# JuliaMolSim/DFTK.jl

Measured on AMD Instinct MI355X. Metric: SCF iterations/sec (Hψ applies/sec) at fixed Ecut·atoms, higher is better.
Workload: dtype f64

## Files before the change

dftk.jl_amd/_lib.py:

```python
from __future__ import annotations

import ctypes as C
import os

from . import _build

c_cplx_p = C.c_void_p
_i64 = C.c_int64


class dftk_mi_cplx(C.Structure):
    _fields_ = [("re", C.c_double), ("im", C.c_double)]


class DftkMiError(RuntimeError):
    def __init__(self, status, msg):
        super().__init__(f"dftk_mi355x status {status}: {msg}")
        self.status = status


_SIGNATURES = {
    "dftk_mi_last_error": (C.c_char_p, []),
    "dftk_mi_version": (C.c_char_p, []),
    "dftk_mi_basis_create": (C.c_int, [C.c_int, C.c_int, C.c_int, C.c_double, C.c_int, C.POINTER(C.c_void_p)]),
    "dftk_mi_basis_destroy": (C.c_int, [C.c_void_p]),
    "dftk_mi_basis_sync": (C.c_int, [C.c_void_p]),
    "dftk_mi_basis_set_fft_batch": (C.c_int, [C.c_void_p, C.c_int]),
    "dftk_mi_basis_stream": (C.c_void_p, [C.c_void_p]),
    "dftk_mi_kblock_create": (C.c_int, [C.c_void_p, _i64, C.c_void_p, C.c_void_p, C.POINTER(C.c_void_p)]),
    "dftk_mi_kblock_destroy": (C.c_int, [C.c_void_p]),
    "dftk_mi_kblock_set_projectors": (C.c_int, [C.c_void_p, C.c_int, C.c_void_p, _i64, C.c_void_p]),
    "dftk_mi_kblock_set_potential": (C.c_int, [C.c_void_p, C.c_void_p]),
    "dftk_mi_apply_H": (C.c_int, [C.c_void_p, C.c_int, C.c_void_p, _i64, C.c_void_p, _i64]),
    "dftk_mi_apply_H_parts": (C.c_int, [C.c_void_p, C.c_int, C.c_int, C.c_void_p, _i64, C.c_void_p, _i64]),
    "dftk_mi_local_potential": (C.c_int, [C.c_void_p, C.c_void_p, C.c_void_p, C.c_void_p, C.c_int, C.c_void_p,
                                          C.c_void_p]),
    "dftk_mi_local_potential_collinear": (C.c_int, [C.c_void_p, C.c_void_p, C.c_void_p, C.c_void_p, C.c_int, C.c_void_p,
                                                    C.c_void_p]),
    "dftk_mi_density_accumulate_spin": (C.c_int, [C.c_void_p, C.c_int, C.c_void_p, _i64, C.c_void_p, C.c_void_p, C.c_int,
                                                  C.c_int]),
    "dftk_mi_kpoint_sphere_host": (C.c_int, [C.c_int, C.c_int, C.c_int, C.c_void_p, C.c_void_p, C.c_double, _i64,
                                             C.POINTER(_i64), C.c_void_p, C.c_void_p, C.c_void_p]),
    "dftk_mi_build_projectors_hgh": (C.c_int, [C.c_void_p, _i64, C.c_void_p, C.c_void_p, C.c_void_p, C.c_double, C.c_int,
                                               C.c_void_p, C.c_void_p, C.c_int, C.c_void_p, C.c_void_p, C.c_void_p, _i64,
                                               C.POINTER(C.c_int)]),
    "dftk_mi_atomic_superposition": (C.c_int, [C.c_void_p, C.c_int, C.c_void_p, C.c_int, C.c_void_p, C.c_int, C.c_void_p,
                                               C.c_void_p, C.c_void_p]),
    "dftk_mi_forces_local": (C.c_int, [C.c_void_p, C.c_void_p, C.c_int, C.c_void_p, C.c_int, C.c_void_p, C.c_void_p,
                                       C.c_void_p, C.c_void_p]),
    "dftk_mi_forces_nonlocal": (C.c_int, [C.c_void_p, C.c_void_p, C.c_int, C.c_void_p, _i64, C.c_void_p, C.c_int,
                                          C.c_void_p, C.c_void_p]),
    "dftk_mi_xc_gga": (C.c_int, [C.c_void_p, _i64, C.c_void_p, C.c_void_p, C.c_int, C.c_double, C.c_void_p, C.c_void_p,
                                 C.c_void_p]),
    "dftk_mi_ifft_sphere": (C.c_int, [C.c_void_p, C.c_void_p, C.c_void_p]),
    "dftk_mi_fft_sphere": (C.c_int, [C.c_void_p, C.c_void_p, C.c_void_p]),
    "dftk_mi_density_accumulate": (C.c_int, [C.c_void_p, C.c_int, C.c_void_p, _i64, C.c_void_p, C.c_void_p]),
    "dftk_mi_lobpcg": (C.c_int, [C.c_void_p, C.c_int, C.c_void_p, _i64, C.c_double, C.c_int, C.c_int, C.c_int,
                                 C.c_int, C.c_uint64, C.c_void_p, C.c_void_p, C.POINTER(C.c_int),
                                 C.POINTER(C.c_int), C.POINTER(_i64)]),
    "dftk_mi_local_potential_gga": (C.c_int, [C.c_void_p, C.c_void_p, C.c_void_p, C.c_void_p, C.c_void_p, C.c_int,
                                              C.c_double, C.c_void_p, C.c_void_p]),
    "dftk_mi_symmetrize_rho": (C.c_int, [C.c_void_p, C.c_int, C.c_void_p, C.c_void_p, C.c_int, C.c_void_p, C.c_void_p]),
    "dftk_mi_mix_kerker": (C.c_int, [C.c_void_p, C.c_void_p, C.c_double, C.c_void_p, C.c_void_p]),
    "dftk_mi_mix_dielectric": (C.c_int, [C.c_void_p, C.c_void_p, C.c_double, C.c_double, C.c_void_p, C.c_void_p]),
    "dftk_mi_chi0_dielectric_apply": (C.c_int, [C.c_void_p, C.c_void_p, C.c_double, C.c_double, C.c_void_p, C.c_void_p]),
    "dftk_mi_cube_fourier_filter": (C.c_int, [C.c_void_p, C.c_void_p, C.c_void_p, C.c_void_p]),
    "dftk_mi_kblocks_set_potential": (C.c_int, [C.c_int, C.c_void_p, C.c_void_p]),
    "dftk_mi_lobpcg_multi": (C.c_int, [C.c_int, C.c_void_p, C.c_int, C.c_void_p, C.c_void_p, C.c_double, C.c_int, C.c_int,
                                       C.c_int, C.c_int, C.c_void_p, C.c_void_p, C.c_void_p, C.c_void_p, C.c_void_p,
                                       C.c_void_p, C.c_void_p]),
    "dftk_mi_density_accumulate_multi": (C.c_int, [C.c_int, C.c_void_p, C.c_void_p, C.c_void_p, C.c_void_p, C.c_void_p,
                                                   C.c_void_p]),
    "dftk_mi_density_accumulate_multi2": (C.c_int, [C.c_int, C.c_void_p, C.c_void_p, C.c_void_p, C.c_void_p, C.c_void_p,
                                                    C.c_void_p, C.c_void_p, C.c_void_p]),
    "dftk_mi_band_kinetic_multi": (C.c_int, [C.c_int, C.c_void_p, C.c_void_p, C.c_void_p, C.c_void_p, C.c_void_p]),
    "dftk_mi_batch_stats": (C.c_int, [C.POINTER(_i64), C.POINTER(_i64), C.POINTER(_i64), C.POINTER(_i64)]),
    "dftk_mi_lobpcg_small_stats": (C.c_int, [C.POINTER(_i64), C.POINTER(_i64)]),
    "dftk_mi_ortho_small": (C.c_int, [C.c_void_p, _i64, C.c_int, C.c_void_p, _i64, C.c_int, C.c_void_p, _i64, C.c_void_p,
                                      C.c_double, C.c_void_p]),
    "dftk_mi_lobpcg_last_AX": (C.c_void_p, [C.c_void_p]),
    "dftk_mi_lobpcg_history": (C.c_int, [C.c_void_p, C.POINTER(C.c_int), C.POINTER(C.c_int), C.c_void_p, C.c_size_t,
                                         C.POINTER(C.c_int)]),
    "dftk_mi_columnwise_norms": (C.c_int, [C.c_void_p, _i64, C.c_int, C.c_void_p, _i64, C.c_void_p]),
    "dftk_mi_columnwise_dots": (C.c_int, [C.c_void_p, _i64, C.c_int, C.c_void_p, _i64, C.c_void_p, _i64, C.c_void_p]),
    "dftk_mi_ortho_qr": (C.c_int, [C.c_void_p, _i64, C.c_int, C.c_void_p, _i64, C.c_int, C.POINTER(C.c_int),
                                   C.POINTER(C.c_int)]),
    "dftk_mi_tpa_precondprep": (C.c_int, [C.c_void_p, C.c_int, C.c_void_p, _i64, C.c_void_p]),
    "dftk_mi_tpa_ldiv": (C.c_int, [C.c_void_p, C.c_int, C.c_void_p, _i64, C.c_void_p, C.c_double, C.c_void_p, _i64]),
    "dftk_mi_block_residual": (C.c_int, [C.c_void_p, C.c_int, C.c_void_p, _i64, C.c_void_p, _i64, C.c_void_p,
                                         C.c_void_p, _i64, C.c_void_p, C.c_void_p, C.c_void_p]),
    "dftk_mi_kblock_set_gamma_real": (C.c_int, [C.c_void_p, C.c_int]),
    "dftk_mi_gamma_half_size": (C.c_int, [C.c_void_p, C.POINTER(_i64)]),
    "dftk_mi_gamma_tables_host": (C.c_int, [C.c_int, C.c_int, C.c_int, _i64, C.c_void_p, C.POINTER(_i64), C.c_void_p,
                                            C.c_void_p]),
    "dftk_mi_gamma_compress": (C.c_int, [C.c_void_p, C.c_int, C.c_void_p, _i64, C.c_void_p, _i64]),
    "dftk_mi_gamma_compress_aligned": (C.c_int, [C.c_void_p, C.c_int, C.c_void_p, _i64, C.c_void_p, _i64]),
    "dftk_mi_gamma_expand": (C.c_int, [C.c_void_p, C.c_int, C.c_void_p, _i64, C.c_void_p, _i64]),
    "dftk_mi_gamma_apply_H": (C.c_int, [C.c_void_p, C.c_int, C.c_int, C.c_void_p, _i64, C.c_void_p, _i64]),
    "dftk_mi_density_accumulate_real": (C.c_int, [C.c_void_p, C.c_int, C.c_void_p, _i64, C.c_void_p, C.c_void_p]),
    "dftk_mi_shard_plan_host": (C.c_int, [C.c_int, C.c_int, C.c_int, C.c_void_p, C.c_void_p, C.c_void_p, C.c_void_p,
                                          C.c_void_p, C.c_void_p]),
    "dftk_mi_kblock_set_shard": (C.c_int, [C.c_void_p, C.c_void_p, C.c_void_p]),
    "dftk_mi_zgemm": (C.c_int, [C.c_void_p, C.c_char, _i64, _i64, _i64, dftk_mi_cplx, C.c_void_p, _i64,
                                C.c_void_p, _i64, dftk_mi_cplx, C.c_void_p, _i64]),
    "dftk_mi_zgemm_ex": (C.c_int, [C.c_void_p, C.c_char, _i64, _i64, _i64, dftk_mi_cplx, C.c_void_p, _i64,
                                   C.c_void_p, _i64, dftk_mi_cplx, C.c_void_p, _i64, C.c_int]),
    "dftk_mi_zgemm_plan_host": (C.c_int, [C.c_char, _i64, _i64, _i64, C.c_int, C.POINTER(C.c_int)]),
    "dftk_mi_heev": (C.c_int, [C.c_void_p, C.c_int, C.c_void_p, _i64, C.c_void_p, C.c_void_p, _i64]),
    "dftk_mi_prof_zgemm_shapes": (C.c_int, [C.c_void_p, C.c_int, C.c_void_p, C.c_void_p, C.POINTER(C.c_int)]),
    "dftk_mi_heev_lowest": (C.c_int, [C.c_void_p, C.c_int, C.c_int, C.c_void_p, _i64, C.c_void_p, C.c_void_p, _i64]),
    "dftk_mi_heev_sigma_host": (C.c_int, [C.c_int, C.c_void_p, C.c_int, C.POINTER(C.c_double), C.POINTER(C.c_double),
                                          C.POINTER(C.c_int), C.c_double]),
    "dftk_mi_potrf_trtri": (C.c_int, [C.c_void_p, C.c_int, C.c_void_p, _i64, C.c_void_p, _i64]),
    "dftk_mi_potrf_trtri_real": (C.c_int, [C.c_void_p, C.c_int, C.c_void_p, _i64, C.c_void_p, _i64]),
    "dftk_mi_comm_get_unique_id": (C.c_int, [C.c_char_p]),
    "dftk_mi_comm_init_rank": (C.c_int, [C.c_char_p, C.c_int, C.c_int, C.c_int, C.POINTER(C.c_void_p)]),
    "dftk_mi_comm_create_host": (C.c_int, [C.c_int, C.c_int, C.c_int, C.c_void_p, C.c_void_p, C.c_void_p,
                                           C.POINTER(C.c_void_p)]),
    "dftk_mi_comm_destroy": (C.c_int, [C.c_void_p]),
    "dftk_mi_comm_describe": (C.c_int, [C.c_void_p, C.POINTER(C.c_int), C.POINTER(C.c_int), C.POINTER(C.c_int)]),
    "dftk_mi_comm_rank": (C.c_int, [C.c_void_p]),
    "dftk_mi_comm_size": (C.c_int, [C.c_void_p]),
    "dftk_mi_allreduce_sum_f64": (C.c_int, [C.c_void_p, C.c_void_p, C.c_size_t, C.c_void_p]),
    "dftk_mi_prof_enable": (C.c_int, [C.c_void_p, C.c_int]),
    "dftk_mi_prof_get": (C.c_int, [C.c_void_p, C.c_int, C.POINTER(C.c_double), C.POINTER(C.c_double),
                                   C.POINTER(_i64)]),
    "dftk_mi_anderson_create": (C.c_int, [C.c_void_p, _i64, C.c_int, C.c_double, C.c_double, C.POINTER(C.c_void_p)]),
    "dftk_mi_anderson_destroy": (C.c_int, [C.c_void_p]),
    "dftk_mi_anderson_reset": (C.c_int, [C.c_void_p]),
    "dftk_mi_anderson_history": (C.c_int, [C.c_void_p]),
    "dftk_mi_anderson_step": (C.c_int, [C.c_void_p, C.c_void_p, C.c_double, C.c_void_p, C.c_void_p, C.POINTER(C.c_int)]),
    "dftk_mi_chi0_mix": (C.c_int, [C.c_void_p, C.c_int, C.c_void_p, C.c_void_p, C.c_void_p, C.c_double, C.c_int, C.c_double,
                                   C.c_double, C.c_void_p, C.c_double, C.c_int, C.c_int, C.c_void_p, C.POINTER(C.c_int),
                                   C.POINTER(C.c_int)]),
    "dftk_mi_launch_count": (C.c_int, [C.POINTER(_i64), C.POINTER(_i64)]),
    "dftk_mi_kblock_reuse_AX": (C.c_int, [C.c_void_p, C.c_int]),
    "dftk_mi_ax_reuse_count": (C.c_int, [C.POINTER(_i64)]),
    "dftk_mi_step_sums": (C.c_int, [C.c_void_p, _i64, C.c_void_p, C.c_void_p, C.c_void_p, C.c_void_p]),
    "dftk_mi_fermi_bisection": (C.c_int, [C.c_int, C.c_void_p, C.c_void_p, C.c_void_p, C.c_int, C.c_double, C.c_double,
                                          C.c_double, C.c_double, C.c_double, C.POINTER(C.c_double)]),
    "dftk_mi_diag_mfma_peak": (C.c_int, [C.c_void_p, C.c_int, C.c_int, C.POINTER(C.c_double)]),
    "dftk_mi_jacobi_schedule_host": (C.c_int, [C.c_int, C.c_int, C.POINTER(C.c_int), C.POINTER(C.c_int),
                                               C.POINTER(C.c_int)]),
    "dftk_mi_fft_plan_host": (C.c_int, [C.c_int, C.POINTER(C.c_int), C.POINTER(C.c_int), C.POINTER(C.c_int)]),
    "dftk_mi_sphere_tables_host": (C.c_int, [C.c_int, C.c_int, C.c_int, _i64, C.c_void_p, C.POINTER(_i64),
                                             C.POINTER(C.c_int), C.c_void_p, C.c_void_p]),
}

ALLREDUCE_FN = C.CFUNCTYPE(C.c_int, C.c_void_p, C.POINTER(C.c_double), C.c_size_t)
ALLTOALLV_FN = C.CFUNCTYPE(C.c_int, C.c_void_p, C.POINTER(C.c_double), C.POINTER(C.c_size_t), C.POINTER(C.c_size_t),
                           C.POINTER(C.c_double), C.POINTER(C.c_size_t), C.POINTER(C.c_size_t))

EXPORTED_SYMBOLS = tuple(_SIGNATURES)
_lib = None


def load(build_if_missing: bool = True):
    global _lib
    if _lib is not None:
        return _lib
    path = _build.LIBPATH
    if build_if_missing and _build.needs_build():
        _build.build()
    if not os.path.exists(path):
        raise RuntimeError(f"{path} is missing and could not be built; the MI355X hot path has no fallback")
    lib = C.CDLL(path, mode=C.RTLD_GLOBAL)
    for name, (res, args) in _SIGNATURES.items():
        fn = getattr(lib, name)
        fn.restype = res
        fn.argtypes = args
    version = lib.dftk_mi_version().decode()
    if not version.endswith("src=" + _build.source_hash()):
        raise RuntimeError(f"{path} was built from other sources ({version!r}, expected src={_build.source_hash()}): "
                           "stale binary, rebuild with python -m dftk_jl_amd._build")
    _lib = lib
    return lib


def check(status: int):
    if status != 0:
        msg = load().dftk_mi_last_error().decode(errors="replace")
# ... 7 lines not shown
```

dftk.jl_amd/csrc/api.cpp:

```cpp
#include "common.h"
#include <chrono>
#include "batch.h"
#include <algorithm>
#include <cmath>
#include <cstdarg>
#include <cstdio>
#include <cstdlib>
#include <cstring>
#include <vector>

static thread_local char g_err[1024] = "";

void dftk_set_error(const char* fmt, ...) {
    va_list ap;
    va_start(ap, fmt);
    vsnprintf(g_err, sizeof(g_err), fmt, ap);
    va_end(ap);
}

extern "C" const char* dftk_mi_last_error(void) { return g_err; }

hipError_t dftk_scratch_malloc(void** p, size_t bytes) {
    static const bool poison = getenv("DFTK_MI_POISON") != nullptr;
    hipError_t e = hipMalloc(p, bytes);
// ... 1047 lines not shown
    }
    cd *R1, *F, *Gf;
    CHK(shard_buffers(kb, n_bands, &R1, &F, &Gf));
    Transposer t(kb, n_bands);
    CHK(t.to_bands(reinterpret_cast<const cd*>(psi_d), R1, F));
    if (t.mine == 0) return 0;
    return launch_density(kb, t.mine, F, kb->n_G, weight_h + t.c0[t.me], rho_d);
}

extern "C" int dftk_mi_density_accumulate_spin(dftk_mi_kblock* kb, int n_bands, const dftk_mi_cplx* psi_d, int64_t ld_psi,
                                               const double* weight_h, double* rho_d, int spin, int n_spin) {
    if (!kb || !rho_d || n_spin < 1 || n_spin > 2 || spin < 0 || spin >= n_spin) return DFTK_MI_EINVAL;
    const int64_t N = (int64_t)kb->basis->nx * kb->basis->ny * kb->basis->nz;
    return dftk_mi_density_accumulate(kb, n_bands, psi_d, ld_psi, weight_h, rho_d + (int64_t)spin * N);
}

extern "C" int dftk_mi_kblock_set_gamma_real(dftk_mi_kblock* kb, int on) {
    if (!kb) return DFTK_MI_EINVAL;
    HIPCHK(hipSetDevice(kb->basis->device));
    return gamma_enable(kb, on);
}

extern "C" int dftk_mi_gamma_tables_host(int nx, int ny, int nz, int64_t n_G, const int64_t* mapping0_h,
                                         int64_t* n_half, int32_t* row_h, int32_t* partner_row_h) {
    if (nx < 1 || ny < 1 || nz < 1 || n_G < 1 || !mapping0_h || !n_half) return DFTK_MI_EINVAL;
    if ((row_h == nullptr) != (partner_row_h == nullptr)) return DFTK_MI_EINVAL;
    return gamma_tables_host(nx, ny, nz, n_G, mapping0_h, n_half, row_h, partner_row_h);
}

static int gamma_ready(dftk_mi_kblock* kb) {
    if (!kb || !kb->gr || !kb->gr->d_g) {
        dftk_set_error("gamma_real: call dftk_mi_kblock_set_gamma_real(kb, 1) first");
        return DFTK_MI_EINVAL;
    }
    return 0;
}

extern "C" int dftk_mi_gamma_half_size(dftk_mi_kblock* kb, int64_t* n_half) {
    if (!n_half) return DFTK_MI_EINVAL;
    CHK(gamma_ready(kb));
    *n_half = gamma_local_rows(kb);
    return 0;
}

extern "C" int dftk_mi_gamma_compress(dftk_mi_kblock* kb, int m, const dftk_mi_cplx* X_d, int64_t ldx,
                                      dftk_mi_cplx* Xh_d, int64_t ldh) {
    CHK(gamma_ready(kb));
    if (m < 0 || !X_d || !Xh_d || ldx < local_rows(kb) || ldh < gamma_local_rows(kb)) return DFTK_MI_EINVAL;
    HIPCHK(hipSetDevice(kb->basis->device));
    if (kb->sh_comm)
        return gamma_lobpcg_load(kb, m, reinterpret_cast<const cd*>(X_d), ldx, reinterpret_cast<cd*>(Xh_d), ldh);
    return gamma_compress(kb, m, reinterpret_cast<const cd*>(X_d), ldx, reinterpret_cast<cd*>(Xh_d), ldh);
}

extern "C" int dftk_mi_gamma_compress_aligned(dftk_mi_kblock* kb, int m, const dftk_mi_cplx* X_d, int64_t ldx,
                                              dftk_mi_cplx* Xh_d, int64_t ldh) {
    CHK(gamma_ready(kb));
    if (m < 0 || !X_d || !Xh_d || ldx < local_rows(kb) || ldh < gamma_local_rows(kb)) return DFTK_MI_EINVAL;
    HIPCHK(hipSetDevice(kb->basis->device));
    return gamma_lobpcg_load(kb, m, reinterpret_cast<const cd*>(X_d), ldx, reinterpret_cast<cd*>(Xh_d), ldh, true);
}

extern "C" int dftk_mi_gamma_expand(dftk_mi_kblock* kb, int m, const dftk_mi_cplx* Xh_d, int64_t ldh,
                                    dftk_mi_cplx* X_d, int64_t ldx) {
    CHK(gamma_ready(kb));
    if (m < 0 || !X_d || !Xh_d || ldx < local_rows(kb) || ldh < gamma_local_rows(kb)) return DFTK_MI_EINVAL;
    HIPCHK(hipSetDevice(kb->basis->device));
    if (kb->sh_comm)
        return gamma_lobpcg_store(kb, m, reinterpret_cast<const cd*>(Xh_d), ldh, reinterpret_cast<cd*>(X_d), ldx);
    return gamma_expand(kb, m, reinterpret_cast<const cd*>(Xh_d), ldh, reinterpret_cast<cd*>(X_d), ldx);
}

extern "C" int dftk_mi_gamma_apply_H(dftk_mi_kblock* kb, int which, int n_bands, const dftk_mi_cplx* psih_d,
                                     int64_t ld_psi, dftk_mi_cplx* Hpsih_d, int64_t ld_Hpsi) {
    CHK(gamma_ready(kb));
    if (!psih_d || !Hpsih_d || n_bands < 0 || (which & ~7) || ld_psi < gamma_local_rows(kb) ||
        ld_Hpsi < gamma_local_rows(kb))
        return DFTK_MI_EINVAL;
    HIPCHK(hipSetDevice(kb->basis->device));
    return gamma_apply_H(kb, which, n_bands, reinterpret_cast<const cd*>(psih_d), ld_psi,
                         reinterpret_cast<cd*>(Hpsih_d), ld_Hpsi);
}

extern "C" int dftk_mi_density_accumulate_real(dftk_mi_kblock* kb, int n_bands, const dftk_mi_cplx* psi_d,
                                               int64_t ld_psi, const double* weight_h, double* rho_d) {
    if (!kb || !psi_d || !weight_h || !rho_d || n_bands < 0 || ld_psi < local_rows(kb)) return DFTK_MI_EINVAL;
    if (n_bands == 0) return 0;
    HIPCHK(hipSetDevice(kb->basis->device));
    if (!kb->sh_comm) prof_count(kb->basis, PROF_A2A_MODEL, 8.0 * (double)kb->n_G * n_bands);
    return gamma_density(kb, n_bands, reinterpret_cast<const cd*>(psi_d), ld_psi, weight_h, rho_d);
}

extern "C" int dftk_mi_lobpcg(dftk_mi_kblock* kb, int M, dftk_mi_cplx* X_d, int64_t ldX, double tol, int miniter,
                              int maxiter, int n_conv_check, int use_tpa, uint64_t seed, double* lambda_h,
                              double* resid_h, int* n_iter, int* converged, int64_t* n_matvec) {
    if (!kb || !X_d || M < 1 || ldX < local_rows(kb) || !lambda_h || !resid_h || !n_iter || !converged || !n_matvec ||
        maxiter < 0)
        return DFTK_MI_EINVAL;
    HIPCHK(hipSetDevice(kb->basis->device));
    return lobpcg_run(kb, M, reinterpret_cast<cd*>(X_d), ldX, tol, miniter, maxiter, n_conv_check, use_tpa, seed,
                      lambda_h, resid_h, n_iter, converged, n_matvec);
}

extern "C" int dftk_mi_lobpcg_multi(int n_kblocks, dftk_mi_kblock* const* kbs, int M, dftk_mi_cplx* const* X_d,
                                    const int64_t* ldX, double tol, int miniter, int maxiter, int n_conv_check, int use_tpa,
                                    const uint64_t* seeds, double* lambda_h, double* resid_h, int* n_iter, int* converged,
                                    int64_t* n_matvec, int* status) {
    if (n_kblocks < 0 || (n_kblocks > 0 && (!kbs || !X_d || !ldX || !lambda_h || !resid_h || !n_iter || !converged ||
                                            !n_matvec || !status)) || M < 1 || maxiter < 0)
        return DFTK_MI_EINVAL;
    if (n_kblocks == 0) return 0;
    for (int i = 0; i < n_kblocks; ++i)
        if (!kbs[i] || !X_d[i] || ldX[i] < local_rows(kbs[i])) return DFTK_MI_EINVAL;
    HIPCHK(hipSetDevice(kbs[0]->basis->device));
    return lobpcg_run_multi(n_kblocks, kbs, M, reinterpret_cast<cd* const*>(X_d), ldX, tol, miniter, maxiter, n_conv_check,
                            use_tpa, seeds, lambda_h, resid_h, n_iter, converged, n_matvec, status);
}

extern "C" int dftk_mi_band_kinetic_multi(int n_kblocks, dftk_mi_kblock* const* kbs, const int* n_bands,
                                          const dftk_mi_cplx* const* psi_d, const int64_t* ld_psi, double* out_h) {
    if (n_kblocks < 0 || (n_kblocks > 0 && (!kbs || !n_bands || !psi_d || !ld_psi || !out_h))) return DFTK_MI_EINVAL;
    if (n_kblocks == 0) return 0;
    dftk_mi_basis* b = kbs[0] ? kbs[0]->basis : nullptr;
    if (!b) return DFTK_MI_EINVAL;
    size_t total = 0;
    for (int i = 0; i < n_kblocks; ++i) {
        if (!kbs[i] || kbs[i]->basis != b || kbs[i]->sh_comm || !psi_d[i] || n_bands[i] < 0 || ld_psi[i] < kbs[i]->n_G)
            return DFTK_MI_EINVAL;
        total += (size_t)n_bands[i];
    }
    HIPCHK(hipSetDevice(b->device));
    CHK(ensure_ws(b, total * sizeof(double)));
    double* d = reinterpret_cast<double*>(b->ws);
    std::vector<std::function<int()>> bodies;
    size_t off = 0;
    for (int i = 0; i < n_kblocks; ++i) {
        const size_t o = off;
        off += (size_t)n_bands[i];
        bodies.push_back([=]() {
            if (n_bands[i] == 0) return 0;
            CHK(ew_weighted_colsums(b, kbs[i]->n_G, n_bands[i], reinterpret_cast<const cd*>(psi_d[i]), ld_psi[i], kbs[i]->d_kin,
                                    d + o));
            return dev_d2h_sync(b, out_h + o, d + o, (size_t)n_bands[i] * sizeof(double));
        });
    }
    std::vector<int> rets;
    CHK(batch_run(b, bodies, rets));
    for (int r : rets)
        if (r != 0) return r;
    return 0;
}

extern "C" int dftk_mi_density_accumulate_multi(int n_kblocks, dftk_mi_kblock* const* kbs, const int* n_bands,
                                                const dftk_mi_cplx* const* psi_d, const int64_t* ld_psi,
                                                const double* weights_h, double* rho_d) {
    return dftk_mi_density_accumulate_multi2(n_kblocks, kbs, n_bands, psi_d, ld_psi, weights_h, rho_d, nullptr, nullptr);
}

extern "C" int dftk_mi_density_accumulate_multi2(int n_kblocks, dftk_mi_kblock* const* kbs, const int* n_bands,
                                                 const dftk_mi_cplx* const* psi_d, const int64_t* ld_psi,
                                                 const double* weights_h, double* rho_d, const double* weights2_h,
                                                 double* rho2_d) {
    if (n_kblocks < 0 || (n_kblocks > 0 && (!kbs || !n_bands || !psi_d || !ld_psi || !weights_h)) || !rho_d ||
        ((weights2_h == nullptr) != (rho2_d == nullptr)) || (rho2_d && rho2_d == rho_d))
        return DFTK_MI_EINVAL;
    if (n_kblocks == 0) return 0;
// ... 244 lines not shown
```

dftk.jl_amd/csrc/common.h:

```cpp
#pragma once
#include <hip/hip_runtime.h>
#include <stdint.h>
#include <stddef.h>
#include <string>
#include <map>
#include <vector>
#include "../../include/dftk_mi355x.h"

typedef double2 cd;

#include <atomic>
extern std::atomic<int64_t> g_dftk_launches, g_dftk_host_syncs;
inline hipError_t dftk_counted_stream_sync(hipStream_t s) {
    g_dftk_host_syncs.fetch_add(1, std::memory_order_relaxed);
    return (hipStreamSynchronize)(s);
}
#define hipStreamSynchronize(s) dftk_counted_stream_sync(s)
#undef hipLaunchKernelGGL
#define hipLaunchKernelGGL(kernelName, ...)                               \
    do {                                                                  \
        g_dftk_launches.fetch_add(1, std::memory_order_relaxed);          \
        hipLaunchKernelGGLInternal((kernelName), __VA_ARGS__);            \
    } while (0)

// ... 25 lines not shown
};

int  plan_radices(int n, int* nrad, int* rad);
void plan_positions(int n, int nrad, const int* rad, int* pos);

struct dftk_mi_basis {
    int nx, ny, nz, nxp;
    double volume;
    int device;
    hipStream_t stream;
    FftAxis ax[3];
    void* d_tables[6];
    int fft_batch;
    cd* T1; size_t T1_bytes;
    cd* T2; size_t T2_bytes;
    void* ws; size_t ws_bytes;
    double* d_scalars;
    double* h_scalars;
    char* h_fetch;
    int use_mfma;
    struct Prof* prof;
    void* dense_ws; size_t dense_ws_bytes;
    void* eig_ws; size_t eig_ws_bytes;
    struct dftk_mi_comm* comm;
    void* symm_tab; uint64_t symm_key; int symm_n;
};

enum ProfFamily {
    PROF_ZGEMM = 0,
    PROF_FFT_A = 1,
    PROF_FFT_B = 2,
    PROF_FFT_C = 3,
    PROF_FFT_D = 4,
    PROF_FFT_E = 5,
    PROF_DENS_Z = 6,
    PROF_HEEV = 7,
    PROF_CHOL = 8,
    PROF_APPLY_H = 9,
    PROF_ZGEMM_BYTES = 10,
    PROF_ZGEMM_STRUCT = 11,
    PROF_ZGEMM_EXEC = 12,
    PROF_COMM = 13,
    PROF_ZGEMM_CPLX = 14,
    PROF_EW = 15,
    PROF_HOST_WAIT = 16,
    PROF_AR_MODEL = 17,
    PROF_A2A_MODEL = 18,
    PROF_NFAM = 24
};
struct Prof {
    bool on = false;
    struct Pair { hipEvent_t a, b; int fam; uint64_t tag; double work; };
    struct Shape { double ms = 0, work = 0; int64_t n = 0; };
    std::map<uint64_t, Shape> shapes;
    std::vector<Pair> pending;
    std::vector<Pair> pool;
    int open = 0;
    int mute = 0;
    bool shape_tags = false;
    double ms[PROF_NFAM] = {0};
    double work[PROF_NFAM] = {0};
    int64_t launches[PROF_NFAM] = {0};
};
int prof_begin(dftk_mi_basis* b, int fam, double work, uint64_t tag = 0);
void prof_end(dftk_mi_basis* b, int slot);
int prof_resolve(dftk_mi_basis* b);
struct ProfScope {
    dftk_mi_basis* b;
    int slot;
    ProfScope(dftk_mi_basis* basis, int fam, double work) : b(basis), slot(prof_begin(basis, fam, work)) {}
    ~ProfScope() { prof_end(b, slot); }
    ProfScope(const ProfScope&) = delete;
    ProfScope& operator=(const ProfScope&) = delete;
};
void prof_count(dftk_mi_basis* b, int fam, double work);
const size_t HOST_FETCH_BYTES = 256 * 1024;
int host_wait(dftk_mi_basis* b);
int host_fetch(dftk_mi_basis* b, void* dst_h, const void* src_d, size_t bytes);

struct GammaReal {
    bool on = false;
    int64_t n_half = 0;
    int *d_g = nullptr, *d_mg = nullptr;
    double* d_kin_half = nullptr;
    cd* P_half = nullptr;
    const cd* P_src = nullptr;
    int P_n_p = 0;
    cd* buf = nullptr;
    size_t buf_bytes = 0;
    std::vector<int64_t> half_rows;
};

struct dftk_mi_kblock {
    dftk_mi_basis* basis;
    int device;
    int64_t n_G;
    int64_t n_lines;
    int nzx;
    int z_lo;
    int*   d_cpos;
    int*   d_line_start;
    int*   d_line_ypos;
    int*   d_zls;
    int*   d_zpos;
    int*   d_zval;
    int*   d_line_yval;
    int*   d_cx;
    double* d_kin;
    double* d_Vs;
    struct SharedVs* Vs_share;
    int n_p;
    const cd* P;
    int64_t ldP;
    double* d_D;
    int D_bw;
    cd* lob_buf; size_t lob_bytes;
    cd* last_AX;
    cd* ax_keep; int ax_M; int64_t ax_rows; int64_t ax_ld;
    double* d_Vs_ax;
    double* d_dVs;
    bool ax_reuse_next;
    dftk_mi_comm* sh_comm;
    std::vector<int64_t>* sh_rows;
    cd* sh_buf; size_t sh_bytes;
    std::vector<double>* lob_hist; int lob_hist_M, lob_hist_iters, lob_n_svd;
    std::vector<int64_t>* h_mapping;
    std::vector<double>* h_kin;
    GammaReal* gr;
    int32_t* d_G3;
};

int fft_ensure_scratch(dftk_mi_basis* b, dftk_mi_kblock* kb, int nb);
int launch_local_apply(dftk_mi_kblock* kb, int nb, const cd* psi, int64_t ldpsi, cd* out,
                       int64_t ldout, bool add_kinetic, bool have_local);
int launch_ifft_to_cube(dftk_mi_kblock* kb, const cd* c, cd* cube, int nb = 1);
int launch_fft_from_cube(dftk_mi_kblock* kb, const cd* cube, cd* c, int nb = 1);
int launch_density(dftk_mi_kblock* kb, int nb, const cd* psi, int64_t ldpsi, const double* w_h, double* rho,
                   const double* w_im_h = nullptr, const double* w2_h = nullptr, double* rho2 = nullptr);
int launch_pad_potential(dftk_mi_kblock* kb, const double* V);
int launch_kinetic_only(dftk_mi_kblock* kb, int nb, const cd* psi, int64_t ldpsi, cd* out,
                        int64_t ldout, bool accumulate, bool use_kin);

int zgemm(dftk_mi_basis* b, char transA, int64_t m, int64_t n, int64_t k, cd alpha, const cd* A,
          int64_t lda, const cd* B, int64_t ldb, cd beta, cd* C, int64_t ldc, int upper = 0);
int ensure_ws(dftk_mi_basis* b, size_t bytes);

int dense_potrf_trtri(dftk_mi_basis* b, int n, cd* A, int64_t lda, cd* invR, int64_t ldi,
                      double* normest_R, double* normest_invR, bool real_input = false);
int dense_heev(dftk_mi_basis* b, int n, cd* A, int64_t lda, double* W_h, cd* V, int64_t ldv);
int dense_heev_full(dftk_mi_basis* b, int n, cd* A, int64_t lda, double* W_h, cd* V, int64_t ldv);
int dense_input_norms(dftk_mi_basis* b, int n, const cd* A, int64_t lda, double* off2, double* dg2, double* im2);
int dense_heev_lowest(dftk_mi_basis* b, int n, int nev, cd* A, int64_t lda, double* W_h, cd* V, int64_t ldv);
int eig_choose_sigma_host(int n, const double* diag, int nev, double* sigma, double* gap_guess);
int eig_hold_iterations_host(double gap_over_norm);
struct ProfMute {
    dftk_mi_basis* b;
    explicit ProfMute(dftk_mi_basis* basis) : b(basis) { if (b->prof) b->prof->mute += 1; }
    ~ProfMute() { if (b->prof) b->prof->mute -= 1; }
    ProfMute(const ProfMute&) = delete;
    ProfMute& operator=(const ProfMute&) = delete;
};
int jacobi_schedule_host(int n, int round, int* nb_out, int* pairs, int* where);
int apply_D(dftk_mi_kblock* kb, int n_bands, const cd* X , cd* Y);
int ew_colnorms(dftk_mi_basis* b, int64_t n, int m, const cd* X, int64_t ldx, double* out_d);
int ew_coldots(dftk_mi_basis* b, int64_t n, int m, const cd* X, int64_t ldx, const cd* Y, int64_t ldy,
               double* out_re_d);
int ew_residual(dftk_mi_basis* b, int64_t n, int m, const cd* AX, int64_t lda, const cd* X, int64_t ldx,
                const double* lam_d, cd* R, int64_t ldr, double* norms_d, const double* kin, double* mean_kin_d,
                double* xx_d);
int ew_tpa(dftk_mi_basis* b, int64_t n, int m, const cd* src, int64_t lds, cd* dst, int64_t ldd, const double* kin,
           const double* mean_kin_d, double* norms_d, double default_shift = 1.0);
int ew_scale_cols(dftk_mi_basis* b, int64_t n, int m, cd* X, int64_t ldx, const double* s_d, bool invert);
int ew_copy(dftk_mi_basis* b, int64_t n, int m, const cd* X, int64_t ldx, cd* Y, int64_t ldy);
int ew_add(dftk_mi_basis* b, int64_t n, int m, const cd* X, int64_t ldx, cd* Y, int64_t ldy);
int ew_sub_real(dftk_mi_basis* b, int64_t n, const double* a, const double* c, double* out);
int ew_fill_zero(dftk_mi_basis* b, cd* X, size_t count);
int ew_sub_identity_shifted(dftk_mi_basis* b, int rows, int cols, cd* C, int64_t ldc, int row0);
int ew_gather_cols(dftk_mi_basis* b, int64_t n, int m, const cd* X, int64_t ldx, const int* perm_d,
                   cd* Y, int64_t ldy);
int ew_add_diag(dftk_mi_basis* b, int n, cd* A, int64_t lda, double shift);
int ew_frob2(dftk_mi_basis* b, int64_t n, int m, const cd* X, int64_t ldx, double* out_d);
int ew_hermitize_upper(dftk_mi_basis* b, int n, cd* A, int64_t lda);
int ew_conj_transpose(dftk_mi_basis* b, int n, const cd* A, int64_t lda, cd* B, int64_t ldb);
int ew_square(dftk_mi_basis* b, double* d, size_t n);
int ew_sqrt(dftk_mi_basis* b, double* d, size_t n);
int ew_coldots_im(dftk_mi_basis* b, int64_t n, int m, const cd* X, int64_t ldx, const cd* Y, int64_t ldy,
                  double* out_im_d);
int ew_weighted_colsums(dftk_mi_basis* b, int64_t n, int m, const cd* X, int64_t ldx, const double* w_d,
                        double* out_d);

int comm_size(const dftk_mi_comm* c);
int comm_rank(const dftk_mi_comm* c);
int comm_allreduce(dftk_mi_comm* c, dftk_mi_basis* b, double* d, size_t n);
int comm_allreduce_norms(dftk_mi_comm* c, dftk_mi_basis* b, double* d, size_t n);
int comm_alltoallv(dftk_mi_comm* c, dftk_mi_basis* b, const cd* send, const size_t* soff, const size_t* scnt,
                   cd* recv, const size_t* roff, const size_t* rcnt);

int local_potential_collinear(dftk_mi_kblock* cube_kb, const double* rho, const double* vloc, const double* green,
                              int fun_mask, double* V_out, double* energies_h);
int local_potential_lda(dftk_mi_kblock* cube_kb, const double* recip_h, const double* rho, const double* vloc,
                        const double* green, int fun_mask, double threshold, double* V_out, double* energies_h);

int cube_symmetrize(dftk_mi_kblock* cube_kb, int n_sym, const int32_t* S_h, const double* tau_h, int do_lowpass,
                    const double* rho_in, double* rho_out);
int cube_fourier_filter(dftk_mi_kblock* cube_kb, int kind, const double* recip_h, double p0, double p1,
                        const double* mult_d, const double* f, double* out);
int xc_gga_pointwise(dftk_mi_basis* b, int64_t n, const double* rho, const double* sigma, int fun_mask,
                     double threshold, double* e, double* vrho, double* vsigma);

int sphere_enumerate_host(int nx, int ny, int nz, const double* B, const double* k, double Ecut, int64_t cap,
                          int64_t* n_G_out, int64_t* mapping0, double* kinetic, int32_t* G_out);
int build_projectors_hgh(dftk_mi_basis* b, int64_t n_rows, const int32_t* G_d, const double* recip_h, const double* k_h,
                         double volume, int n_species, const double* rp_h, const int* nproj_h, int n_atoms,
                         const int* species_of_atom_h, const double* positions_h, cd* P_d, int64_t ldP, int* n_p_out);

int atomic_superposition(dftk_mi_kblock* cube_kb, int kind, const double* recip_h, int n_species, const double* par_h,
                         int n_atoms, const int* species_of_atom_h, const double* positions_h, double* out_d);

int gamma_tables_host(int nx, int ny, int nz, int64_t n_G, const int64_t* mapping, int64_t* n_half_out, int32_t* g,
                      int32_t* mg);
int gamma_enable(dftk_mi_kblock* kb, int on);
void gamma_destroy(GammaReal* gr);
int gamma_compress(dftk_mi_kblock* kb, int m, const cd* X, int64_t ldx, cd* H, int64_t ldh);
int gamma_compress_aligned(dftk_mi_kblock* kb, int m, const cd* X, int64_t ldx, cd* H, int64_t ldh);
int gamma_expand(dftk_mi_kblock* kb, int m, const cd* H, int64_t ldh, cd* X, int64_t ldx);
int gamma_apply_H(dftk_mi_kblock* kb, int which, int nb, const cd* psi, int64_t ldpsi, cd* Hpsi, int64_t ldH);
int gamma_density(dftk_mi_kblock* kb, int nb, const cd* psi, int64_t ldpsi, const double* w_h, double* rho);
int gamma_ensure_buf(dftk_mi_kblock* kb, size_t elems);
int gamma_pack_pairs(dftk_mi_kblock* kb, int nb, const cd* H, int64_t ldh, cd* Z, int64_t ldz);
int gamma_unpack_pairs(dftk_mi_kblock* kb, int nb, const cd* W, int64_t ldw, cd* H, int64_t ldh);
int gamma_pack_full(dftk_mi_kblock* kb, int nb, const cd* X, int64_t ldx, cd* Z, int64_t ldz);
int gamma_gather_P(dftk_mi_kblock* kb, int ncols, const cd* P, int64_t ldP, cd* Ph, int64_t ldh, double* asym_mag_h);
int gamma_density_bands(dftk_mi_kblock* kb, int nb, const cd* psi, int64_t ldpsi, const double* w_h, double* rho);
int64_t gamma_local_rows(const dftk_mi_kblock* kb);
int64_t gamma_row0(const dftk_mi_kblock* kb);
int gamma_projectors(dftk_mi_kblock* kb);
int gamma_apply_H_sharded(dftk_mi_kblock* kb, int which, int nb, const cd* psi, int64_t ldpsi, cd* Hpsi, int64_t ldH);
int gamma_projectors_sharded(dftk_mi_kblock* kb);
int gamma_density_sharded(dftk_mi_kblock* kb, int nb, const cd* psi, int64_t ldpsi, const double* w_h, double* rho);
int gamma_lobpcg_load(dftk_mi_kblock* kb, int M, const cd* Xuser, int64_t ldX, cd* Xh, int64_t ldh, bool align = false);
int gamma_lobpcg_store(dftk_mi_kblock* kb, int M, const cd* Xh, int64_t ldh, cd* Xuser, int64_t ldX);
int apply_nonlocal_rows(dftk_mi_kblock* kb, int nb, const cd* P, int64_t ldP, int64_t rows, const cd* psi,
                        int64_t ldpsi, cd* Hpsi, int64_t ldH, bool accumulate, int gemm_flags, dftk_mi_comm* comm);

int forces_local(dftk_mi_kblock* cube_kb, const double* recip_h, int n_species, const double* par_h, int n_atoms,
                 const int* species_of_atom_h, const double* positions_h, const double* rho_d, double* forces_h);
int forces_nonlocal(dftk_mi_kblock* kb, const double* kcoord_h, int nb, const cd* psi, int64_t ld_psi,
                    const double* weight_h, int n_atoms, const int* col_start_h, double* forces_h);

int lobpcg_ortho(dftk_mi_basis* b, int64_t n, int m, cd* X, int64_t ldx, int force_svd, int* n_chol, int* used_svd);
int lobpcg_run_multi(int n_kb, dftk_mi_kblock* const* kbs, int M, cd* const* X, const int64_t* ldX, double tol, int miniter,
                     int maxiter, int n_conv_check, int use_tpa, const uint64_t* seeds, double* lambda_h, double* resid_h,
                     int* n_iter, int* converged, int64_t* n_matvec, int* status);
int lobpcg_run(dftk_mi_kblock* kb, int M, cd* X, int64_t ldX, double tol, int miniter, int maxiter,
               int n_conv_check, int use_tpa, uint64_t seed, double* lambda_h, double* resid_h,
               int* n_iter, int* converged, int64_t* n_matvec);
```

dftk.jl_amd/csrc/fft_kernels.hip:

```cpp
#include "common.h"
#include "batch.h"
#include <algorithm>
#include <cstring>
#include <type_traits>

#define FFT_L 8
#ifndef ZPASS_MIN_BLOCKS
#define ZPASS_MIN_BLOCKS 6
#endif
#ifndef DENS_MIN_BLOCKS
#define DENS_MIN_BLOCKS 1
#endif
#ifndef YFWD_MIN_BLOCKS
#define YFWD_MIN_BLOCKS 1
#endif
#define FFT_LS_X 9
#define FFT_LS_YZ 8
#define FFT_THREADS 256
#define FFT_TPL (FFT_THREADS / FFT_L)
#define DENS_MAXACC 12

__device__ __forceinline__ cd cmul(cd a, cd w) {
    return make_double2(fma(a.x, w.x, -a.y * w.y), fma(a.x, w.y, a.y * w.x));
}
// ... 192 lines not shown
        case 4: fft_stage<FFT_LS, 4, false, true>(buf, tw, n, m, sgn, l, j, vcol, vstride); return true;
        case 5: fft_stage<FFT_LS, 5, false, true>(buf, tw, n, m, sgn, l, j, vcol, vstride); return true;
        case 6: fft_stage<FFT_LS, 6, false, true>(buf, tw, n, m, sgn, l, j, vcol, vstride); return true;
        case 8: fft_stage<FFT_LS, 8, false, true>(buf, tw, n, m, sgn, l, j, vcol, vstride); return true;
        default: return false;
    }
}

template <int FFT_LS, bool DIF, bool GEN>
__device__ __forceinline__ void fft_stage_dispatch(int R, cd* buf, const cd* tw, int n, int m, double sgn,
                                                   int l, int j) {
    switch (R) {
        case 2: fft_stage<FFT_LS, 2, DIF>(buf, tw, n, m, sgn, l, j); break;
        case 3: fft_stage<FFT_LS, 3, DIF>(buf, tw, n, m, sgn, l, j); break;
        case 4: fft_stage<FFT_LS, 4, DIF>(buf, tw, n, m, sgn, l, j); break;
        case 5: fft_stage<FFT_LS, 5, DIF>(buf, tw, n, m, sgn, l, j); break;
        case 6: fft_stage<FFT_LS, 6, DIF>(buf, tw, n, m, sgn, l, j); break;
        case 8: fft_stage<FFT_LS, 8, DIF>(buf, tw, n, m, sgn, l, j); break;
        default:
            if constexpr (GEN) {
                if (R == 7)
                    fft_stage<FFT_LS, 7, DIF>(buf, tw, n, m, sgn, l, j);
                else
                    fft_stage_generic<FFT_LS, DIF>(buf, tw, n, m, R, sgn, l, j);
            }
            break;
    }
}

template <int FFT_LS, bool DIF, bool GEN>
__device__ __forceinline__ bool fft_tile(cd* buf, const cd* tw, const FftAxis& ax, double sgn, int l, int j,
                                         const double* vcol = nullptr, int64_t vstride = 0,
                                         bool skip_first = false) {
    const int n = ax.n;
    bool fused = false;
    if (!DIF) {
        int m = 1;
        for (int s = 0; s < ax.nrad; ++s) {
            const int R = ax.rad[s];
            if (vcol != nullptr && s == ax.nrad - 1)
                fused = fft_stage_vmul<FFT_LS>(R, buf, tw, n, m, sgn, l, j, vcol, vstride);
            if (!fused) fft_stage_dispatch<FFT_LS, false, GEN>(R, buf, tw, n, m, sgn, l, j);
            __syncthreads();
            m *= R;
        }
    } else {
        int m = n;
        for (int s = ax.nrad - 1; s >= 0; --s) {
            const int R = ax.rad[s];
            m /= R;
            if (skip_first && s == ax.nrad - 1) continue;
            fft_stage_dispatch<FFT_LS, true, GEN>(R, buf, tw, n, m, sgn, l, j);
            __syncthreads();
        }
    }
    return fused;
}

template <int FFT_LS>
__device__ __forceinline__ void tile_prologue(cd* buf, cd* tw, const FftAxis& ax, bool zero, bool copy_tw = true) {
    const int n = ax.n;
    if (copy_tw)
        for (int t = threadIdx.x; t < n; t += FFT_THREADS) tw[t] = ax.tw[t];
    if (zero) {
        const cd z = make_double2(0.0, 0.0);
        for (int t = threadIdx.x; t < n * FFT_LS; t += FFT_THREADS) buf[t] = z;
    }
}

extern __shared__ __attribute__((aligned(16))) char dftk_smem[];

struct FftJob {
    const int *line_start, *cpos, *line_ypos, *zls, *zpos;
    int z_lo;
    const double* kin;
    const double* Vs;
    const cd* psi;
    cd* out;
    int n_lines, nzx;
    double w, wim;
    double w2;
};

template <bool GEN>
__global__ __launch_bounds__(FFT_THREADS) void k_xbwd_scatter(FftAxis ax, int nxp, int n_lines,
                                                              const int* __restrict__ line_start,
                                                              const int* __restrict__ cpos,
                                                              const cd* __restrict__ psi, int64_t ldpsi,
                                                              cd* __restrict__ T1, int64_t T1_stride,
                                                              const FftJob* __restrict__ jobs) {
    constexpr int FFT_LS = FFT_LS_X;
    cd* buf = reinterpret_cast<cd*>(dftk_smem);
    cd* tw = buf + ax.n * FFT_LS;
    const int tid = threadIdx.x, l = tid & (FFT_L - 1), j = tid >> 3;
    const int band = blockIdx.y;
    const int l0 = blockIdx.x * FFT_L;
    const cd* p = psi + (int64_t)band * ldpsi;
    if (jobs) {
        const FftJob jb = jobs[band];
        n_lines = jb.n_lines;
        line_start = jb.line_start;
        cpos = jb.cpos;
        p = jb.psi;
        if (l0 >= n_lines) return;
    }
    tile_prologue<FFT_LS>(buf, tw, ax, true);
    __syncthreads();
    const int line = l0 + l;
    if (line < n_lines) {
        const int c0 = line_start[line], c1 = line_start[line + 1];
        for (int c = c0 + j; c < c1; c += FFT_TPL) buf[cpos[c] * FFT_LS + l] = p[c];
    }
    __syncthreads();
    fft_tile<FFT_LS, false, GEN>(buf, tw, ax, +1.0, l, j);
    cd* out = T1 + (int64_t)band * T1_stride + (int64_t)l0 * nxp;
    const int nlv = min(FFT_L, n_lines - l0);
    const int n = ax.n;
    for (int idx = tid; idx < nlv * nxp; idx += FFT_THREADS) {
        const int ll = idx / nxp;
        const int x = idx - ll * nxp;
        out[idx] = (x < n) ? buf[x * FFT_LS + ll] : make_double2(0.0, 0.0);
    }
}

template <bool GEN>
__global__ __launch_bounds__(FFT_THREADS) void k_ybwd(FftAxis ay, int nxp, int ny,
                                                      const int* __restrict__ zls,
                                                      const int* __restrict__ line_ypos,
                                                      const cd* __restrict__ T1, int64_t T1_stride,
                                                      cd* __restrict__ T2, int64_t T2_stride,
                                                      const FftJob* __restrict__ jobs) {
    constexpr int FFT_LS = FFT_LS_YZ;
    cd* buf = reinterpret_cast<cd*>(dftk_smem);
    cd* tw = buf + ay.n * FFT_LS;
    const int tid = threadIdx.x, l = tid & (FFT_L - 1), j = tid >> 3;
    const int x = blockIdx.x * FFT_L + l;
    const int zi = blockIdx.y, band = blockIdx.z;
    if (jobs) {
        const FftJob jb = jobs[band];
        if (zi >= jb.nzx) return;
        zls = jb.zls;
        line_ypos = jb.line_ypos;
    }
    const cd* t1 = T1 + (int64_t)band * T1_stride;
    const int ln0 = zls[zi] + j, ln1 = zls[zi + 1];
    const bool early = ln1 - zls[zi] <= 3 * FFT_TPL;
    cd e0, e1, e2;
    if (early) {
        if (ln0 < ln1) e0 = t1[(int64_t)ln0 * nxp + x];
        if (ln0 + FFT_TPL < ln1) e1 = t1[(int64_t)(ln0 + FFT_TPL) * nxp + x];
        if (ln0 + 2 * FFT_TPL < ln1) e2 = t1[(int64_t)(ln0 + 2 * FFT_TPL) * nxp + x];
    }
    tile_prologue<FFT_LS>(buf, tw, ay, true);
    __syncthreads();
    if (early) {
        if (ln0 < ln1) buf[line_ypos[ln0] * FFT_LS + l] = e0;
        if (ln0 + FFT_TPL < ln1) buf[line_ypos[ln0 + FFT_TPL] * FFT_LS + l] = e1;
        if (ln0 + 2 * FFT_TPL < ln1) buf[line_ypos[ln0 + 2 * FFT_TPL] * FFT_LS + l] = e2;
    } else {
        for (int ln = ln0; ln < ln1; ln += FFT_TPL) buf[line_ypos[ln] * FFT_LS + l] = t1[(int64_t)ln * nxp + x];
    }
    __syncthreads();
    fft_tile<FFT_LS, false, GEN>(buf, tw, ay, +1.0, l, j);
    cd* t2 = T2 + (int64_t)band * T2_stride + (int64_t)zi * ny * nxp + x;
    for (int y = j; y < ny; y += FFT_TPL) t2[(int64_t)y * nxp] = buf[y * FFT_LS + l];
}

template <int MODE, bool GEN>
__global__ __launch_bounds__(FFT_THREADS, ZPASS_MIN_BLOCKS) void k_zpass(FftAxis az, int nx, int nxp, int ny, int nzx,
                                                       int nbands, const int* __restrict__ zpos,
                                                       const double* __restrict__ Vs,
                                                       cd* __restrict__ T2, int64_t T2_stride,
                                                       cd* __restrict__ cube, const FftJob* __restrict__ jobs = nullptr) {
    constexpr int FFT_LS = FFT_LS_YZ;
    cd* buf = reinterpret_cast<cd*>(dftk_smem);
    cd* tw = buf + az.n * FFT_LS;
    const int tid = threadIdx.x, l = tid & (FFT_L - 1), j = tid >> 3;
    const int xcd = blockIdx.x & 7, slot = blockIdx.x >> 3;
    const int band = slot % nbands;
    const int grp = (slot / nbands) * 8 + xcd;
    const int nxt = nxp / FFT_L;
    if (grp >= nxt * ny) return;
    if (jobs) {
        const FftJob jb = jobs[band];
        zpos = jb.zpos;
        nzx = jb.nzx;
        Vs = jb.Vs;
    }
    const int y = grp / nxt;
    const int x = (grp - y * nxt) * FFT_L + l;
    const int nz = az.n;
    const int64_t plane = (int64_t)ny * nxp;
    cd* t2 = T2 + (int64_t)band * T2_stride + (int64_t)y * nxp + x;
    const bool early = MODE != 2 && nzx <= 3 * FFT_TPL;
// ... 293 lines not shown
            wi = jb.wim;
            wb2 = jb.w2;
            nzx = jb.nzx;
            z_lo = jb.z_lo;
        } else {
            wb = w[ib];
            wi = wim ? wim[ib] : wb;
        }
        if (wb == 0.0 && wi == 0.0 && wb2 == 0.0) continue;
        const cd* __restrict__ t2 = T2 + (int64_t)ib * T2_stride + (int64_t)y * nxp + (x - l);
        const unsigned planeB = plane * (unsigned)sizeof(cd), stepB = (unsigned)FS::R2 * planeB;
        const unsigned off_lo = (unsigned)j * planeB + (unsigned)l * (unsigned)sizeof(cd);
        const unsigned off_hi = off_lo - (unsigned)(FS::N - nzx) * planeB;
        const int zneg0 = FS::N - (nzx - z_lo);
        auto in = [&](auto ni) -> cd {
            constexpr int n1 = decltype(ni)::value;
            const int e = FS::R2 * n1 + j;
            const bool lo = e < z_lo, hi = e >= zneg0;
            cd v = make_double2(0.0, 0.0);
            if (lo || hi) v = ld_off(t2, (lo ? off_lo : off_hi) + (unsigned)n1 * stepB);
            return v;
        };
        cd psi[FS::R2];
        FS::backward(buf, az.tw, l, j, in, psi);
        if (j < FS::R1) {
#pragma unroll
            for (int p = 0; p < FS::R2; ++p) {
                acc[p] = fma(wb, psi[p].x * psi[p].x, fma(wi, psi[p].y * psi[p].y, acc[p]));
                if (rho2) acc2[p] = fma(wb2, psi[p].x * psi[p].x + psi[p].y * psi[p].y, acc2[p]);
            }
        }
        __syncthreads();
    }
    if (j < FS::R1 && x < nx) {
        double* __restrict__ r0 = (part ? part + (int64_t)blockIdx.z * az.n * ny * nx : rho) + (int64_t)y * nx + (x - l);
        const unsigned zB = (unsigned)ny * (unsigned)nx * 8u;
        const unsigned ob = (unsigned)j * zB + (unsigned)l * 8u;
        static_for<0, FS::R2>([&](auto pi) {
            constexpr int p = decltype(pi)::value;
            const unsigned off = ob + (unsigned)(FS::R1 * FS::k2_of(p)) * zB;
            st_off(r0, off, part ? acc[p] : ld_off((const double*)r0, off) + acc[p]);
        });
        if (rho2) {
            double* __restrict__ q0 = (part ? part + ((int64_t)gridDim.z + blockIdx.z) * az.n * ny * nx : rho2) + (int64_t)y * nx + (x - l);
            static_for<0, FS::R2>([&](auto pi) {
                constexpr int p = decltype(pi)::value;
                const unsigned off = ob + (unsigned)(FS::R1 * FS::k2_of(p)) * zB;
                st_off(q0, off, part ? acc2[p] : ld_off((const double*)q0, off) + acc2[p]);
            });
        }
    }
}

template <bool GEN>
__global__ __launch_bounds__(FFT_THREADS, YFWD_MIN_BLOCKS) void k_yfwd(FftAxis ay, int nxp, int ny,
                                                      const int* __restrict__ zls,
                                                      const int* __restrict__ line_ypos,
                                                      const cd* __restrict__ T2, int64_t T2_stride,
                                                      cd* __restrict__ T1, int64_t T1_stride,
                                                      const FftJob* __restrict__ jobs) {
    constexpr int FFT_LS = FFT_LS_YZ;
    cd* buf = reinterpret_cast<cd*>(dftk_smem);
    cd* tw = buf + ay.n * FFT_LS;
    const int tid = threadIdx.x, l = tid & (FFT_L - 1), j = tid >> 3;
    const int x = blockIdx.x * FFT_L + l;
    const int zi = blockIdx.y, band = blockIdx.z;
    if (jobs) {
        const FftJob jb = jobs[band];
        if (zi >= jb.nzx) return;
        zls = jb.zls;
        line_ypos = jb.line_ypos;
    }
    tile_prologue<FFT_LS>(buf, tw, ay, false);
    const cd* t2 = T2 + (int64_t)band * T2_stride + (int64_t)zi * ny * nxp + x;
    for (int y = j; y < ny; y += FFT_TPL) buf[y * FFT_LS + l] = t2[(int64_t)y * nxp];
    __syncthreads();
    fft_tile<FFT_LS, true, GEN>(buf, tw, ay, -1.0, l, j);
    cd* t1 = T1 + (int64_t)band * T1_stride;
    const int ln1 = zls[zi + 1];
    for (int ln = zls[zi] + j; ln < ln1; ln += FFT_TPL)
        t1[(int64_t)ln * nxp + x] = buf[line_ypos[ln] * FFT_LS + l];
}

template <bool GEN>
__global__ __launch_bounds__(FFT_THREADS, YFWD_MIN_BLOCKS) void k_xfwd_gather(FftAxis ax, int nxp, int n_lines,
                                                             const int* __restrict__ line_start,
                                                             const int* __restrict__ cpos,
                                                             const cd* __restrict__ T1, int64_t T1_stride,
                                                             const double* __restrict__ kin,
                                                             const cd* __restrict__ psi, int64_t ldpsi,
                                                             cd* __restrict__ out, int64_t ldout,
                                                             const FftJob* __restrict__ jobs) {
    constexpr int FFT_LS = FFT_LS_X;
    cd* buf = reinterpret_cast<cd*>(dftk_smem);
    cd* tw = buf + ax.n * FFT_LS;
    const int tid = threadIdx.x, l = tid & (FFT_L - 1), j = tid >> 3;
    const int band = blockIdx.y;
    const int l0 = blockIdx.x * FFT_L;
    const int n = ax.n;
    cd* o = out + (int64_t)band * ldout;
    const cd* p = psi + (int64_t)band * ldpsi;
    if (jobs) {
        const FftJob jb = jobs[band];
        n_lines = jb.n_lines;
        line_start = jb.line_start;
        cpos = jb.cpos;
        kin = jb.kin;
        p = jb.psi;
        o = jb.out;
        if (l0 >= n_lines) return;
    }
    tile_prologue<FFT_LS>(buf, tw, ax, false);
    const cd* in = T1 + (int64_t)band * T1_stride + (int64_t)l0 * nxp;
    const int nlv = min(FFT_L, n_lines - l0);
    for (int idx = tid; idx < FFT_L * nxp; idx += FFT_THREADS) {
        const int ll = idx / nxp;
        const int x = idx - ll * nxp;
        if (x < n) buf[x * FFT_LS + ll] = (ll < nlv) ? in[idx] : make_double2(0.0, 0.0);
    }
    __syncthreads();
    fft_tile<FFT_LS, true, GEN>(buf, tw, ax, -1.0, l, j);
    const int line = l0 + l;
    if (line < n_lines) {
        const int c0 = line_start[line], c1 = line_start[line + 1];
        for (int c = c0 + j; c < c1; c += FFT_TPL) {
            cd v = buf[cpos[c] * FFT_LS + l];
            if (kin != nullptr) {
                const double k = kin[c];
                const cd q = p[c];
                v.x = fma(k, q.x, v.x);
                v.y = fma(k, q.y, v.y);
            }
            o[c] = v;
        }
    }
}

template <bool GEN>
__global__ __launch_bounds__(FFT_THREADS, DENS_MIN_BLOCKS) void k_zdensity(FftAxis az, int nx, int nxp, int ny, int nzx,
                                                          const int* __restrict__ zpos, int nb,
                                                          const double* __restrict__ w,
                                                          const double* __restrict__ wim,
                                                          const cd* __restrict__ T2, int64_t T2_stride,
                                                          double* __restrict__ rho, const FftJob* __restrict__ jobs,
                                                          double* __restrict__ part, double* __restrict__ rho2 = nullptr) {
    constexpr int FFT_LS = FFT_LS_YZ;
    cd* buf = reinterpret_cast<cd*>(dftk_smem);
    cd* tw = buf + az.n * FFT_LS;
    const int tid = threadIdx.x, l = tid & (FFT_L - 1), j = tid >> 3;
    const int x = blockIdx.x * FFT_L + l;
    const int y = blockIdx.y;
    const int nz = az.n;
    const int64_t plane = (int64_t)ny * nxp;
    double acc[DENS_MAXACC], acc2[DENS_MAXACC];
#pragma unroll
    for (int k = 0; k < DENS_MAXACC; ++k) acc[k] = acc2[k] = 0.0;
    for (int t = tid; t < nz; t += FFT_THREADS) tw[t] = az.tw[t];
    for (int ib = blockIdx.z; ib < nb; ib += gridDim.z) {
        double wb, wi, wb2 = 0.0;
        if (jobs) {
            const FftJob jb = jobs[ib];
            wb = jb.w;
            wi = jb.wim;
            wb2 = jb.w2;
            zpos = jb.zpos;
            nzx = jb.nzx;
        } else {
            wb = w[ib];
            wi = wim ? wim[ib] : wb;
        }
        if (wb == 0.0 && wi == 0.0 && wb2 == 0.0) continue;
        const cd z0 = make_double2(0.0, 0.0);
        for (int t = tid; t < nz * FFT_LS; t += FFT_THREADS) buf[t] = z0;
        __syncthreads();
        const cd* t2 = T2 + (int64_t)ib * T2_stride + (int64_t)y * nxp + x;
        for (int zi = j; zi < nzx; zi += FFT_TPL) buf[zpos[zi] * FFT_LS + l] = t2[(int64_t)zi * plane];
        __syncthreads();
        fft_tile<FFT_LS, false, GEN>(buf, tw, az, +1.0, l, j);
#pragma unroll
        for (int k = 0; k < DENS_MAXACC; ++k) {
            const int z = j + k * FFT_TPL;
            if (z < nz) {
                const cd v = buf[z * FFT_LS + l];
                acc[k] = fma(wb, v.x * v.x, fma(wi, v.y * v.y, acc[k]));
                if (rho2) acc2[k] = fma(wb2, v.x * v.x + v.y * v.y, acc2[k]);
            }
        }
        __syncthreads();
    }
    if (x < nx) {
        double* __restrict__ dst = part ? part + (int64_t)blockIdx.z * nz * ny * nx : rho;
#pragma unroll
        for (int k = 0; k < DENS_MAXACC; ++k) {
            const int z = j + k * FFT_TPL;
            if (z < nz) {
                const int64_t at = ((int64_t)z * ny + y) * nx + x;
                dst[at] = part ? acc[k] : dst[at] + acc[k];
            }
        }
        if (rho2) {
            double* __restrict__ dst2 = part ? part + ((int64_t)gridDim.z + blockIdx.z) * nz * ny * nx : rho2;
#pragma unroll
            for (int k = 0; k < DENS_MAXACC; ++k) {
                const int z = j + k * FFT_TPL;
                if (z < nz) {
                    const int64_t at = ((int64_t)z * ny + y) * nx + x;
                    dst2[at] = part ? acc2[k] : dst2[at] + acc2[k];
                }
            }
        }
    }
}
// ... 5 lines not shown
    for (int g = 0; g < ngroups; ++g) s += part[(int64_t)g * n + i];
    rho[i] += s;
}

__global__ void k_pad_potential(int nx, int nxp, int64_t rows, double scale, const double* __restrict__ V,
                                double* __restrict__ Vs) {
    const int64_t i = (int64_t)blockIdx.x * blockDim.x + threadIdx.x;
    if (i >= rows * nxp) return;
    const int64_t r = i / nxp;
    const int x = (int)(i - r * nxp);
    Vs[i] = (x < nx) ? V[r * nx + x] * scale : 0.0;
}

__global__ void k_kinetic(int64_t n, int nb, const double* __restrict__ kin, const cd* __restrict__ psi,
                          int64_t ldpsi, cd* __restrict__ out, int64_t ldout, int accumulate) {
    const int64_t i = (int64_t)blockIdx.x * blockDim.x + threadIdx.x;
    if (i >= n) return;
    const double k = kin ? kin[i] : 0.0;
    for (int b = 0; b < nb; ++b) {
        cd q = psi[(int64_t)b * ldpsi + i];
        cd v = make_double2(k * q.x, k * q.y);
        if (accumulate) {
            cd o = out[(int64_t)b * ldout + i];
            v.x += o.x;
            v.y += o.y;
        }
        out[(int64_t)b * ldout + i] = v;
    }
}

static size_t lds_bytes(int n, int ls = FFT_LS_YZ) { return (size_t)n * (ls + 1) * sizeof(cd); }

int fft_ensure_scratch(dftk_mi_basis* b, dftk_mi_kblock* kb, int nb) {
    const size_t t1 = (size_t)nb * kb->n_lines * b->nxp * sizeof(cd);
    const size_t t2 = (size_t)nb * kb->nzx * b->ny * b->nxp * sizeof(cd);
    if (t1 > b->T1_bytes) {
        if (b->T1) HIPCHK(hipFree(b->T1));
        b->T1 = nullptr;
        HIPCHK(dftk_scratch_malloc((void**)&b->T1, t1));
        b->T1_bytes = t1;
    }
    if (t2 > b->T2_bytes) {
        if (b->T2) HIPCHK(hipFree(b->T2));
        b->T2 = nullptr;
        HIPCHK(dftk_scratch_malloc((void**)&b->T2, t2));
        b->T2_bytes = t2;
    }
    return 0;
}

static int check_lds(dftk_mi_basis* b) {
    const int nmax = b->nx > b->ny ? (b->nx > b->nz ? b->nx : b->nz) : (b->ny > b->nz ? b->ny : b->nz);
    if (lds_bytes(nmax, FFT_LS_X) > 160 * 1024) {
        dftk_set_error("FFT axis length %d needs %zu B of LDS (> 160 KiB)", nmax, lds_bytes(nmax, FFT_LS_X));
        return DFTK_MI_EINVAL;
    }
    return 0;
}

template <typename K>
static int set_lds_attr(K kernel, size_t bytes) {
    if (bytes > 64 * 1024) {
        HIPCHK(hipFuncSetAttribute(reinterpret_cast<const void*>(kernel),
                                   hipFuncAttributeMaxDynamicSharedMemorySize, (int)bytes));
    }
    return 0;
}

static bool axis_generic(const FftAxis& ax) {
    for (int s = 0; s < ax.nrad; ++s)
        if (ax.rad[s] > 5 && ax.rad[s] != 6 && ax.rad[s] != 8) return true;
    return false;
}

#define LAUNCH_FFT(KERNEL, AX, GRID, LDS, STREAM, ...)                                               \
    do {                                                                                             \
        if (axis_generic(AX)) {                                                                      \
            CHK(set_lds_attr(KERNEL<true>, LDS));                                                    \
            hipLaunchKernelGGL((KERNEL<true>), GRID, dim3(FFT_THREADS), LDS, STREAM, __VA_ARGS__);   \
        } else {                                                                                     \
            CHK(set_lds_attr(KERNEL<false>, LDS));                                                   \
            hipLaunchKernelGGL((KERNEL<false>), GRID, dim3(FFT_THREADS), LDS, STREAM, __VA_ARGS__);  \
        }                                                                                            \
    } while (0)
#define LAUNCH_ZPASS(MODE, AX, GRID, LDS, STREAM, ...)                                                      \
    do {                                                                                                    \
        if (axis_generic(AX)) {                                                                             \
            CHK(set_lds_attr(k_zpass<MODE, true>, LDS));                                                    \
            hipLaunchKernelGGL((k_zpass<MODE, true>), GRID, dim3(FFT_THREADS), LDS, STREAM, __VA_ARGS__);   \
        } else {                                                                                            \
            CHK(set_lds_attr(k_zpass<MODE, false>, LDS));                                                   \
            hipLaunchKernelGGL((k_zpass<MODE, false>), GRID, dim3(FFT_THREADS), LDS, STREAM, __VA_ARGS__);  \
        }                                                                                                   \
    } while (0)

#define REG_SIZES(X)                                                                                                      \
    X(24, 2, 2, 3, 2) X(27, 3, 3, 3, 1) X(30, 5, 1, 3, 2) X(32, 2, 2, 4, 2) X(36, 3, 2, 3, 2) X(40, 2, 2, 5, 2) X(48, 3, 2, 4, 2) X(54, 3, 2, 3, 3)           \
    X(45, 3, 3, 5, 1) X(50, 5, 2, 5, 1) X(60, 3, 2, 5, 2)                                                                 \
    X(64, 4, 2, 4, 2) X(72, 3, 3, 4, 2) X(80, 5, 2, 4, 2) X(90, 5, 2, 3, 3) X(96, 4, 3, 4, 2) X(100, 5, 2, 5, 2)          \
    X(108, 4, 3, 3, 3) X(120, 4, 3, 5, 2) X(128, 4, 4, 4, 2) X(144, 4, 3, 4, 3) X(150, 5, 3, 5, 2) X(160, 4, 4, 5, 2)     \
    X(180, 5, 3, 4, 3) X(192, 4, 4, 4, 3) X(200, 5, 4, 5, 2) X(216, 6, 3, 4, 3) X(240, 4, 4, 5, 3) X(256, 4, 4, 4, 4)
static bool fft_reg_on(int n) {
    static const bool off = getenv("DFTK_MI_FFT_REG") != nullptr && atoi(getenv("DFTK_MI_FFT_REG")) == 0;
    static const int nmin = getenv("DFTK_MI_FFT_REG_MIN") ? atoi(getenv("DFTK_MI_FFT_REG_MIN")) : 24;
    return !off && n >= nmin;
}
static bool fft_reg_fits(const dftk_mi_basis* b) {
    return (uint64_t)b->nz * (uint64_t)b->ny * (uint64_t)b->nxp * sizeof(cd) < (1ull << 32);
}
struct RegZ {
    dftk_mi_basis* b;
    hipStream_t stream;
    dim3 grid;
    int nzx, z_lo, nbands;
    const double* Vs;
    cd* T2;
    int64_t s2;
    const double *w, *wim;
    double* rho;
    const FftJob* jobs;
    double* part = nullptr;
    double* rho2 = nullptr;
};
template <int A, int B, int C, int D>
static int reg_zpass_t(const RegZ& r) {
    typedef FourStep<A, B, C, D> FS;
    const size_t lds = (size_t)FS::LDS_ELEMS * sizeof(cd);
    CHK(set_lds_attr(k_zpass_reg<A, B, C, D>, lds));
    hipLaunchKernelGGL((k_zpass_reg<A, B, C, D>), r.grid, dim3(FS::THREADS), lds, r.stream, r.b->ax[2], r.b->nx, r.b->nxp, r.b->ny,
                       r.nzx, r.z_lo, r.nbands, r.Vs, r.T2, r.s2, r.jobs);
    return 0;
}
template <int A, int B, int C, int D>
static int reg_zdens_t(const RegZ& r) {
    typedef FourStep<A, B, C, D> FS;
    const size_t lds = (size_t)FS::LDS_ELEMS * sizeof(cd);
    CHK(set_lds_attr(k_zdensity_reg<A, B, C, D>, lds));
    hipLaunchKernelGGL((k_zdensity_reg<A, B, C, D>), r.grid, dim3(FS::THREADS), lds, r.stream, r.b->ax[2], r.b->nx, r.b->nxp,
                       r.b->ny, r.nzx, r.z_lo, r.nbands, r.w, r.wim, (const cd*)r.T2, r.s2, r.rho, r.jobs, r.part, r.rho2);
    return 0;
}
static int reg_zpass(const RegZ& r, bool tables_ok) {
    if (!tables_ok || !fft_reg_on(r.b->nz) || !fft_reg_fits(r.b)) return 1;
    switch (r.b->nz) {
#define X(NN, A, B, C, D) case NN: return reg_zpass_t<A, B, C, D>(r);
        REG_SIZES(X)
#undef X
        default: return 1;
    }
}
static int reg_zdens(const RegZ& r, bool tables_ok) {
    if (!tables_ok || !fft_reg_on(r.b->nz) || !fft_reg_fits(r.b)) return 1;
    switch (r.b->nz) {
#define X(NN, A, B, C, D) case NN: return reg_zdens_t<A, B, C, D>(r);
        REG_SIZES(X)
#undef X
        default: return 1;
    }
}

static dim3 zpass_grid(const dftk_mi_basis* b, int nbands) {
    const int64_t groups = (int64_t)(b->nxp / FFT_L) * b->ny;
    return dim3((unsigned)(((groups + 7) / 8) * 8 * nbands));
}

struct Strides {
    int64_t s1, s2;
};
static Strides strides(dftk_mi_kblock* kb) {
    dftk_mi_basis* b = kb->basis;
    return Strides{(int64_t)kb->n_lines * b->nxp, (int64_t)kb->nzx * b->ny * b->nxp};
}

static int run_AB(dftk_mi_kblock* kb, int nbb, const cd* psi, int64_t ldpsi) {
    dftk_mi_basis* b = kb->basis;
    const Strides st = strides(kb);
    const int gl = (int)((kb->n_lines + FFT_L - 1) / FFT_L);
    const int nxt = b->nxp / FFT_L;
    const double Ncube = (double)b->nx * b->ny * b->nz;
    const double t1b = 16.0 * (double)kb->n_lines * b->nxp, t2b = 16.0 * (double)kb->nzx * b->ny * b->nxp;
    (void)Ncube;
    int ps = prof_begin(b, PROF_FFT_A, (16.0 * kb->n_G + t1b) * nbb);
    LAUNCH_FFT(k_xbwd_scatter, b->ax[0], dim3(gl, nbb), lds_bytes(b->nx, FFT_LS_X), b->stream, b->ax[0],
                       b->nxp, (int)kb->n_lines, kb->d_line_start, kb->d_cpos, psi, ldpsi, b->T1, st.s1, (const FftJob*)nullptr);
    prof_end(b, ps);
    ps = prof_begin(b, PROF_FFT_B, (t1b + t2b) * nbb);
    LAUNCH_FFT(k_ybwd, b->ax[1], dim3(nxt, kb->nzx, nbb), lds_bytes(b->ny), b->stream, b->ax[1],
                       b->nxp, b->ny, kb->d_zls, kb->d_line_ypos, b->T1, st.s1, b->T2, st.s2, (const FftJob*)nullptr);
    prof_end(b, ps);
    return 0;
}

static int run_DE(dftk_mi_kblock* kb, int nbb, const double* kin, const cd* psi, int64_t ldpsi, cd* out,
                  int64_t ldout) {
    dftk_mi_basis* b = kb->basis;
    const Strides st = strides(kb);
    const int gl = (int)((kb->n_lines + FFT_L - 1) / FFT_L);
    const int nxt = b->nxp / FFT_L;
    const double Ncube = (double)b->nx * b->ny * b->nz;
    const double t1b = 16.0 * (double)kb->n_lines * b->nxp, t2b = 16.0 * (double)kb->nzx * b->ny * b->nxp;
    (void)Ncube;
    int ps = prof_begin(b, PROF_FFT_D, (t1b + t2b) * nbb);
    LAUNCH_FFT(k_yfwd, b->ax[1], dim3(nxt, kb->nzx, nbb), lds_bytes(b->ny), b->stream, b->ax[1],
                       b->nxp, b->ny, kb->d_zls, kb->d_line_ypos, b->T2, st.s2, b->T1, st.s1, (const FftJob*)nullptr);
    prof_end(b, ps);
    ps = prof_begin(b, PROF_FFT_E, (t1b + (kin ? 40.0 : 16.0) * kb->n_G) * nbb);
    LAUNCH_FFT(k_xfwd_gather, b->ax[0], dim3(gl, nbb), lds_bytes(b->nx, FFT_LS_X), b->stream, b->ax[0],
                       b->nxp, (int)kb->n_lines, kb->d_line_start, kb->d_cpos, b->T1, st.s1, kin, psi, ldpsi, out,
                       ldout, (const FftJob*)nullptr);
    prof_end(b, ps);
    return 0;
}

int launch_local_apply(dftk_mi_kblock* kb, int nb, const cd* psi, int64_t ldpsi, cd* out, int64_t ldout,
                       bool add_kinetic, bool have_local) {
    dftk_mi_basis* b = kb->basis;
    if (!have_local || kb->d_Vs == nullptr) {
        return launch_kinetic_only(kb, nb, psi, ldpsi, out, ldout, false, add_kinetic);
    }
    CHK(check_lds(b));
    const int batch = b->fft_batch;
    CHK(fft_ensure_scratch(b, kb, nb < batch ? nb : batch));
    const Strides st = strides(kb);
    const int nxt = b->nxp / FFT_L;
    for (int b0 = 0; b0 < nb; b0 += batch) {
        const int nbb = (nb - b0) < batch ? (nb - b0) : batch;
        const cd* p = psi + (int64_t)b0 * ldpsi;
        CHK(run_AB(kb, nbb, p, ldpsi));
        const int pc = prof_begin(b, PROF_FFT_C, 2.0 * 16.0 * (double)kb->nzx * b->ny * b->nxp * nbb +
                                                     8.0 * (double)b->nz * b->ny * b->nxp);
        const RegZ rz{b, b->stream, zpass_grid(b, nbb), kb->nzx, kb->z_lo, nbb, kb->d_Vs, b->T2, st.s2, nullptr, nullptr, nullptr,
                      nullptr};
        const int reg_st = reg_zpass(rz, kb->z_lo >= 0);
        if (reg_st < 0) return reg_st;
        if (reg_st != 0)
        LAUNCH_ZPASS(0, b->ax[2], zpass_grid(b, nbb), lds_bytes(b->nz), b->stream, b->ax[2], b->nx, b->nxp, b->ny, kb->nzx, nbb, kb->d_zpos, kb->d_Vs, b->T2, st.s2,
                           (cd*)nullptr, (const FftJob*)nullptr);
        prof_end(b, pc);
        CHK(run_DE(kb, nbb, add_kinetic ? kb->d_kin : nullptr, p, ldpsi, out + (int64_t)b0 * ldout, ldout));
    }
    HIPCHK(hipGetLastError());
    return 0;
}

int launch_kinetic_only(dftk_mi_kblock* kb, int nb, const cd* psi, int64_t ldpsi, cd* out, int64_t ldout,
                        bool accumulate, bool use_kin) {
    dftk_mi_basis* b = kb->basis;
    const int threads = 256;
    const int blocks = (int)((kb->n_G + threads - 1) / threads);
    hipLaunchKernelGGL(k_kinetic, dim3(blocks), dim3(threads), 0, b->stream, kb->n_G, nb,
                       use_kin ? kb->d_kin : (const double*)nullptr, psi, ldpsi, out, ldout, accumulate ? 1 : 0);
    HIPCHK(hipGetLastError());
    return 0;
}

int launch_ifft_to_cube(dftk_mi_kblock* kb, const cd* c, cd* cube, int nb) {
    dftk_mi_basis* b = kb->basis;
    CHK(check_lds(b));
    CHK(fft_ensure_scratch(b, kb, nb));
    const Strides st = strides(kb);
    CHK(run_AB(kb, nb, c, kb->n_G));
    LAUNCH_ZPASS(1, b->ax[2], zpass_grid(b, nb), lds_bytes(b->nz), b->stream, b->ax[2], b->nx, b->nxp, b->ny, kb->nzx, nb, kb->d_zpos, (const double*)nullptr, b->T2, st.s2,
                       cube, (const FftJob*)nullptr);
    HIPCHK(hipGetLastError());
    return 0;
}

int launch_fft_from_cube(dftk_mi_kblock* kb, const cd* cube, cd* c, int nb) {
    dftk_mi_basis* b = kb->basis;
    CHK(check_lds(b));
    CHK(fft_ensure_scratch(b, kb, nb));
    const Strides st = strides(kb);
    LAUNCH_ZPASS(2, b->ax[2], zpass_grid(b, nb), lds_bytes(b->nz), b->stream, b->ax[2], b->nx, b->nxp, b->ny, kb->nzx, nb, kb->d_zpos, (const double*)nullptr, b->T2, st.s2,
                       const_cast<cd*>(cube), (const FftJob*)nullptr);
    CHK(run_DE(kb, nb, nullptr, c, kb->n_G, c, kb->n_G));
    HIPCHK(hipGetLastError());
    return 0;
}

int launch_density(dftk_mi_kblock* kb, int nb, const cd* psi, int64_t ldpsi, const double* w_h, double* rho,
                   const double* w_im_h, const double* w2_h, double* rho2) {
    dftk_mi_basis* b = kb->basis;
    if (batching() && nb > 0) {
        BOp o;
        o.b = b;
        o.kb = kb;
        o.type = BOP_DENSITY; o.m = nb; o.A = psi; o.lda = ldpsi; o.C = rho; o.D = w2_h ? rho2 : nullptr;
        o.flags = (w_im_h ? 1 : 0) | (w2_h ? 2 : 0);
        o.payload.resize((size_t)(1 + (w_im_h ? 1 : 0) + (w2_h ? 1 : 0)) * nb * sizeof(double));
        memcpy(o.payload.data(), w_h, (size_t)nb * sizeof(double));
        size_t at = (size_t)nb * sizeof(double);
        if (w_im_h) {
            memcpy(o.payload.data() + at, w_im_h, (size_t)nb * sizeof(double));
            at += (size_t)nb * sizeof(double);
        }
        if (w2_h) memcpy(o.payload.data() + at, w2_h, (size_t)nb * sizeof(double));
        return batch_record(std::move(o));
    }
    if (w2_h) {
        CHK(launch_density(kb, nb, psi, ldpsi, w_h, rho, w_im_h, nullptr, nullptr));
        return launch_density(kb, nb, psi, ldpsi, w2_h, rho2, nullptr, nullptr, nullptr);
    }
    CHK(check_lds(b));
    if (b->nz > DENS_MAXACC * FFT_TPL) {
        dftk_set_error("density kernel supports nz <= %d", DENS_MAXACC * FFT_TPL);
        return DFTK_MI_EINVAL;
    }
    const int batch = b->fft_batch;
    CHK(fft_ensure_scratch(b, kb, nb < batch ? nb : batch));
    const Strides st = strides(kb);
    CHK(ensure_ws(b, 2 * (size_t)nb * sizeof(double)));
    double* w_d = reinterpret_cast<double*>(b->ws);
    double* wim_d = w_im_h ? w_d + nb : nullptr;
    HIPCHK(hipMemcpyAsync(w_d, w_h, (size_t)nb * sizeof(double), hipMemcpyHostToDevice, b->stream));
    if (w_im_h) HIPCHK(hipMemcpyAsync(wim_d, w_im_h, (size_t)nb * sizeof(double), hipMemcpyHostToDevice, b->stream));
    for (int b0 = 0; b0 < nb; b0 += batch) {
        const int nbb = (nb - b0) < batch ? (nb - b0) : batch;
        bool any = false;
        for (int i = 0; i < nbb; ++i) any = any || (w_h[b0 + i] != 0.0) || (w_im_h && w_im_h[b0 + i] != 0.0);
        if (!any) continue;
        CHK(run_AB(kb, nbb, psi + (int64_t)b0 * ldpsi, ldpsi));
        const int pz = prof_begin(b, PROF_DENS_Z, 16.0 * (double)kb->nzx * b->ny * b->nxp * nbb +
// ... 224 lines not shown
```

dftk.jl_amd/csrc/gamma_kernels.hip:

```cpp
#include "common.h"
#include <algorithm>
#include <cmath>
#include <cstdio>
#include <unordered_map>
#include <vector>

int gamma_tables_host(int nx, int ny, int nz, int64_t n_G, const int64_t* mapping, int64_t* n_half_out, int32_t* g,
                      int32_t* mg) {
    if (n_G < 1 || mapping[0] != 0) {
        dftk_set_error("gamma_real: the sphere must contain G = 0 as its first entry");
        return DFTK_MI_EINVAL;
    }
    std::unordered_map<int64_t, int32_t> row;
    row.reserve((size_t)n_G * 2);
    for (int64_t c = 0; c < n_G; ++c) row[mapping[c]] = (int32_t)c;
    int64_t nh = 0;
    for (int64_t c = 0; c < n_G; ++c) {
        const int64_t lin = mapping[c];
        const int ix = (int)(lin % nx), iy = (int)((lin / nx) % ny), iz = (int)(lin / ((int64_t)nx * ny));
        const int64_t mlin = (int64_t)((nx - ix) % nx) + (int64_t)nx * (((ny - iy) % ny) + (int64_t)ny * ((nz - iz) % nz));
        auto it = row.find(mlin);
        if (it == row.end()) {
            dftk_set_error("gamma_real: the sphere is not inversion symmetric (row %lld has no -G partner)", (long long)c);
            return DFTK_MI_EINVAL;
// ... 119 lines not shown
            im[u] = j < nh ? mg[j] : 0;
        }
#pragma unroll
        for (int u = 0; u < GR_UNR; ++u) {
            a[u] = x[ig[u]];
            b[u] = x[im[u]];
        }
#pragma unroll
        for (int u = 0; u < GR_UNR; ++u) {
            const int64_t j = j0 + u * GRA_NT;
            cd aa = a[u], bb = b[u];
            if (rot) {
                aa = make_double2(aa.x * c + aa.y * sn, aa.y * c - aa.x * sn);
                bb = make_double2(bb.x * c + bb.y * sn, bb.y * c - bb.x * sn);
            }
            const double s = j ? GR_ISQRT2 : 0.5;
            if (j < nh) h[j] = make_double2(s * (aa.x + bb.x), s * (aa.y - bb.y));
        }
    }
}

__global__ __launch_bounds__(256) void k_gr_expand(int64_t nh, const int* __restrict__ g, const int* __restrict__ mg,
                                                   const cd* __restrict__ H, int64_t ldh, cd* __restrict__ X, int64_t ldx) {
    const int64_t j0 = (int64_t)blockIdx.x * GR_ROWS + threadIdx.x;
    cd* x = X + (int64_t)blockIdx.y * ldx;
    const cd* hc = H + (int64_t)blockIdx.y * ldh;
    int ig[GR_UNR], im[GR_UNR];
    cd h[GR_UNR];
#pragma unroll
    for (int u = 0; u < GR_UNR; ++u) {
        const int64_t j = j0 + u * 256;
        const bool in = j < nh;
        ig[u] = in ? g[j] : 0;
        im[u] = in ? mg[j] : 0;
        h[u] = in ? hc[j] : make_double2(0.0, 0.0);
    }
#pragma unroll
    for (int u = 0; u < GR_UNR; ++u) {
        const int64_t j = j0 + u * 256;
        if (j >= nh) continue;
        if (j == 0) {
            x[ig[u]] = make_double2(h[u].x, 0.0);
            continue;
        }
        x[ig[u]] = make_double2(GR_ISQRT2 * h[u].x, GR_ISQRT2 * h[u].y);
        x[im[u]] = make_double2(GR_ISQRT2 * h[u].x, -GR_ISQRT2 * h[u].y);
    }
}

__global__ __launch_bounds__(256) void k_gr_pack(int64_t nh, int nb, const int* __restrict__ g, const int* __restrict__ mg,
                                                 const cd* __restrict__ H, int64_t ldh, cd* __restrict__ Z, int64_t ldz) {
    const int64_t j0 = (int64_t)blockIdx.x * GR_ROWS + threadIdx.x;
    const int p = blockIdx.y;
    const bool has_b = 2 * p + 1 < nb;
    const cd* ha = H + (int64_t)(2 * p) * ldh;
    const cd* hb = H + (int64_t)(has_b ? 2 * p + 1 : 2 * p) * ldh;
    cd* z = Z + (int64_t)p * ldz;
    int ig[GR_UNR], im[GR_UNR];
    cd a[GR_UNR], b[GR_UNR];
#pragma unroll
    for (int u = 0; u < GR_UNR; ++u) {
        const int64_t j = j0 + u * 256;
        const bool in = j < nh;
        ig[u] = in ? g[j] : 0;
        im[u] = in ? mg[j] : 0;
        a[u] = in ? ha[j] : make_double2(0.0, 0.0);
        b[u] = (in && has_b) ? hb[j] : make_double2(0.0, 0.0);
    }
    const double s = GR_ISQRT2;
#pragma unroll
    for (int u = 0; u < GR_UNR; ++u) {
        const int64_t j = j0 + u * 256;
        if (j >= nh) continue;
        if (j == 0) {
            z[ig[u]] = make_double2(a[u].x, b[u].x);
            continue;
        }
        z[ig[u]] = make_double2(s * (a[u].x - b[u].y), s * (a[u].y + b[u].x));
        z[im[u]] = make_double2(s * (a[u].x + b[u].y), s * (b[u].x - a[u].y));
    }
}

__global__ __launch_bounds__(256) void k_gr_unpack(int64_t nh, int nb, const int* __restrict__ g, const int* __restrict__ mg,
                                                   const cd* __restrict__ W, int64_t ldw, cd* __restrict__ H, int64_t ldh) {
    const int64_t j0 = (int64_t)blockIdx.x * GR_ROWS + threadIdx.x;
    const int p = blockIdx.y;
    const cd* w = W + (int64_t)p * ldw;
    int ig[GR_UNR], im[GR_UNR];
    cd wg[GR_UNR], wm[GR_UNR];
#pragma unroll
    for (int u = 0; u < GR_UNR; ++u) {
        const int64_t j = j0 + u * 256;
        ig[u] = j < nh ? g[j] : 0;
        im[u] = j < nh ? mg[j] : 0;
    }
#pragma unroll
    for (int u = 0; u < GR_UNR; ++u) {
        wg[u] = w[ig[u]];
        wm[u] = w[im[u]];
    }
#pragma unroll
    for (int u = 0; u < GR_UNR; ++u) {
        const int64_t j = j0 + u * 256;
        if (j >= nh) continue;
        const double s = j ? GR_ISQRT2 : 0.5;
        H[j + (int64_t)(2 * p) * ldh] = make_double2(s * (wg[u].x + wm[u].x), s * (wg[u].y - wm[u].y));
        if (2 * p + 1 < nb) H[j + (int64_t)(2 * p + 1) * ldh] = make_double2(s * (wg[u].y + wm[u].y), s * (wm[u].x - wg[u].x));
    }
}

__global__ __launch_bounds__(256) void k_gr_pack_full(int64_t n, int nb, const cd* __restrict__ X, int64_t ldx,
                                                      cd* __restrict__ Z, int64_t ldz) {
    const int64_t i0 = (int64_t)blockIdx.x * GR_ROWS + threadIdx.x;
    const int p = blockIdx.y;
    const bool has_b = 2 * p + 1 < nb;
    const cd* xa = X + (int64_t)(2 * p) * ldx;
    const cd* xb = X + (int64_t)(has_b ? 2 * p + 1 : 2 * p) * ldx;
    cd a[GR_UNR], b[GR_UNR];
#pragma unroll
    for (int u = 0; u < GR_UNR; ++u) {
        const int64_t i = i0 + u * 256;
        a[u] = i < n ? xa[i] : make_double2(0.0, 0.0);
        b[u] = (i < n && has_b) ? xb[i] : make_double2(0.0, 0.0);
    }
#pragma unroll
    for (int u = 0; u < GR_UNR; ++u) {
        const int64_t i = i0 + u * 256;
        if (i < n) Z[i + (int64_t)p * ldz] = make_double2(a[u].x - b[u].y, a[u].y + b[u].x);
    }
}

__global__ __launch_bounds__(256) void k_gr_gather_P(int64_t nh, const int* __restrict__ g, const int* __restrict__ mg,
                                                     const cd* __restrict__ P, int64_t ldP, cd* __restrict__ Ph, int64_t ldh,
                                                     unsigned long long* __restrict__ out) {
    __shared__ double sh[2][256];
    const int64_t j = (int64_t)blockIdx.x * blockDim.x + threadIdx.x;
    double asym = 0.0, mag = 0.0;
    if (j < nh) {
        const cd* pc = P + (int64_t)blockIdx.y * ldP;
        const cd a = pc[g[j]], b = pc[mg[j]];
        asym = hypot(b.x - a.x, b.y + a.y);
        mag = hypot(a.x, a.y);
        Ph[j + (int64_t)blockIdx.y * ldh] = j ? make_double2(GR_SQRT2 * a.x, GR_SQRT2 * a.y) : make_double2(a.x, 0.0);
    }
    sh[0][threadIdx.x] = asym == asym ? asym : INFINITY;
    sh[1][threadIdx.x] = mag == mag ? mag : INFINITY;
    __syncthreads();
    for (int s = 128; s > 0; s >>= 1) {
        if ((int)threadIdx.x < s) {
            sh[0][threadIdx.x] = fmax(sh[0][threadIdx.x], sh[0][threadIdx.x + s]);
            sh[1][threadIdx.x] = fmax(sh[1][threadIdx.x], sh[1][threadIdx.x + s]);
        }
        __syncthreads();
    }
    if (threadIdx.x == 0) {
        atomicMax(out, (unsigned long long)__double_as_longlong(sh[0][0]));
        atomicMax(out + 1, (unsigned long long)__double_as_longlong(sh[1][0]));
    }
}

static dim3 gr_grid(int64_t rows, int cols) { return dim3((unsigned)((rows + 255) / 256), (unsigned)cols); }
static dim3 gr_grid_unr(int64_t rows, int cols) { return dim3((unsigned)((rows + GR_ROWS - 1) / GR_ROWS), (unsigned)cols); }

int gamma_enable(dftk_mi_kblock* kb, int on) {
    dftk_mi_basis* b = kb->basis;
    if (!on) {
        if (kb->gr) kb->gr->on = false;
        return 0;
    }
    if (kb->gr && kb->gr->d_g) {
        kb->gr->on = true;
        return 0;
    }
    if (!kb->h_mapping || !kb->h_kin) return DFTK_MI_EINVAL;
    std::vector<int32_t> g((size_t)(kb->n_G + 1) / 2 + 1), mg(g.size());
    int64_t nh = 0;
    CHK(gamma_tables_host(b->nx, b->ny, b->nz, kb->n_G, kb->h_mapping->data(), &nh, g.data(), mg.data()));
    std::vector<double> kin((size_t)nh);
    for (int64_t j = 0; j < nh; ++j) {
        const double a = (*kb->h_kin)[g[j]], c = (*kb->h_kin)[mg[j]];
        if (std::fabs(a - c) > 1e-12 * (1.0 + std::fabs(a))) {
            dftk_set_error("gamma_real: kinetic energies of G and -G differ (k != 0?)");
            return DFTK_MI_EINVAL;
        }
        kin[j] = a;
    }
    GammaReal* gr = kb->gr ? kb->gr : new GammaReal();
    gr->n_half = nh;
    HIPCHK(hipMalloc((void**)&gr->d_g, nh * sizeof(int)));
    HIPCHK(hipMalloc((void**)&gr->d_mg, nh * sizeof(int)));
    HIPCHK(hipMalloc((void**)&gr->d_kin_half, nh * sizeof(double)));
    HIPCHK(hipMemcpy(gr->d_g, g.data(), nh * sizeof(int), hipMemcpyHostToDevice));
    HIPCHK(hipMemcpy(gr->d_mg, mg.data(), nh * sizeof(int), hipMemcpyHostToDevice));
    HIPCHK(hipMemcpy(gr->d_kin_half, kin.data(), nh * sizeof(double), hipMemcpyHostToDevice));
    gr->half_rows.clear();
    if (kb->sh_comm) {
        const int p = comm_size(kb->sh_comm);
        if (nh < p) {
            dftk_set_error("gamma_real: more ranks than half-sphere rows");
            if (!kb->gr) delete gr;
            return DFTK_MI_EINVAL;
        }
        gr->half_rows.assign(p + 1, 0);
        const int64_t base = nh / p, rem = nh % p;
        for (int r = 0; r < p; ++r) gr->half_rows[r + 1] = gr->half_rows[r] + base + (r < rem ? 1 : 0);
    }
    gr->on = true;
    kb->gr = gr;
    return 0;
}

int64_t gamma_local_rows(const dftk_mi_kblock* kb) {
    const GammaReal* gr = kb->gr;
    if (!kb->sh_comm) return gr->n_half;
    const int r = comm_rank(kb->sh_comm);
    return gr->half_rows[r + 1] - gr->half_rows[r];
}
int64_t gamma_row0(const dftk_mi_kblock* kb) { return kb->sh_comm ? kb->gr->half_rows[comm_rank(kb->sh_comm)] : 0; }

void gamma_destroy(GammaReal* gr) {
    if (!gr) return;
    void* ptrs[] = {gr->d_g, gr->d_mg, gr->d_kin_half, gr->P_half, gr->buf};
    for (void* p : ptrs)
        if (p) hipFree(p);
    delete gr;
}

int gamma_ensure_buf(dftk_mi_kblock* kb, size_t elems) {
    GammaReal* gr = kb->gr;
    const size_t need = elems * sizeof(cd);
    if (need <= gr->buf_bytes) return 0;
    HIPCHK(hipStreamSynchronize(kb->basis->stream));
    if (gr->buf) HIPCHK(hipFree(gr->buf));
    gr->buf = nullptr;
    gr->buf_bytes = 0;
    HIPCHK(dftk_scratch_malloc((void**)&gr->buf, need));
    gr->buf_bytes = need;
    return 0;
}

int gamma_compress(dftk_mi_kblock* kb, int m, const cd* X, int64_t ldx, cd* H, int64_t ldh) {
    if (m <= 0) return 0;
    GammaReal* gr = kb->gr;
    ProfScope prof_scope(kb->basis, PROF_EW, 48.0 * (double)gr->n_half * m);
    hipLaunchKernelGGL(k_gr_compress, gr_grid_unr(gr->n_half, m), dim3(256), 0, kb->basis->stream, gr->n_half, gr->d_g,
                       gr->d_mg, X, ldx, H, ldh);
    HIPCHK(hipGetLastError());
    return 0;
}

int gamma_compress_aligned(dftk_mi_kblock* kb, int m, const cd* X, int64_t ldx, cd* H, int64_t ldh) {
    if (m <= 0) return 0;
    GammaReal* gr = kb->gr;
    ProfScope prof_scope(kb->basis, PROF_EW, 64.0 * (double)gr->n_half * m);
    hipLaunchKernelGGL(k_gr_compress_aligned, dim3(m), dim3(GRA_NT), 0, kb->basis->stream, gr->n_half, gr->d_g, gr->d_mg, X, ldx,
                       H, ldh);
    HIPCHK(hipGetLastError());
    return 0;
}

int gamma_expand(dftk_mi_kblock* kb, int m, const cd* H, int64_t ldh, cd* X, int64_t ldx) {
    if (m <= 0) return 0;
    GammaReal* gr = kb->gr;
    ProfScope prof_scope(kb->basis, PROF_EW, 48.0 * (double)gr->n_half * m);
    hipLaunchKernelGGL(k_gr_expand, gr_grid_unr(gr->n_half, m), dim3(256), 0, kb->basis->stream, gr->n_half, gr->d_g,
                       gr->d_mg, H, ldh, X, ldx);
    HIPCHK(hipGetLastError());
    return 0;
}

int gamma_gather_P(dftk_mi_kblock* kb, int ncols, const cd* P, int64_t ldP, cd* Ph, int64_t ldh, double* asym_mag_h) {
    GammaReal* gr = kb->gr;
    dftk_mi_basis* b = kb->basis;
    unsigned long long* d_out = reinterpret_cast<unsigned long long*>(b->d_scalars);
    HIPCHK(hipMemsetAsync(d_out, 0, 2 * sizeof(unsigned long long), b->stream));
    if (ncols > 0) {
        hipLaunchKernelGGL(k_gr_gather_P, gr_grid(gr->n_half, ncols), dim3(256), 0, b->stream, gr->n_half, gr->d_g,
                           gr->d_mg, P, ldP, Ph, ldh, d_out);
        HIPCHK(hipGetLastError());
    }
    HIPCHK(hipMemcpyAsync(asym_mag_h, d_out, 2 * sizeof(double), hipMemcpyDeviceToHost, b->stream));
    HIPCHK(hipStreamSynchronize(b->stream));
    return 0;
}

static int gr_projectors(dftk_mi_kblock* kb) {
    GammaReal* gr = kb->gr;
    if (gr->P_src == kb->P && gr->P_n_p == kb->n_p && gr->P_half) return 0;
    if (kb->sh_comm) return gamma_projectors_sharded(kb);
    dftk_mi_basis* b = kb->basis;
    HIPCHK(hipStreamSynchronize(b->stream));
    if (gr->P_half) HIPCHK(hipFree(gr->P_half));
    gr->P_half = nullptr;
    HIPCHK(hipMalloc((void**)&gr->P_half, (size_t)gr->n_half * kb->n_p * sizeof(cd)));
    double h[2];
    CHK(gamma_gather_P(kb, kb->n_p, kb->P, kb->ldP, gr->P_half, gr->n_half, h));
    if (!(std::isfinite(h[1]) && h[0] <= 1e-10 * (h[1] > 0 ? h[1] : 1.0))) {
        dftk_set_error("gamma_real: the projectors are not real-symmetric (max |P(-G) - conj P(G)| = %.3e, max |P| = %.3e)",
                       h[0], h[1]);
        HIPCHK(hipFree(gr->P_half));
        gr->P_half = nullptr;
        return DFTK_MI_EINVAL;
    }
    gr->P_src = kb->P;
    gr->P_n_p = kb->n_p;
    return 0;
}

int gamma_projectors(dftk_mi_kblock* kb) { return gr_projectors(kb); }

int gamma_pack_pairs(dftk_mi_kblock* kb, int nb, const cd* H, int64_t ldh, cd* Z, int64_t ldz) {
    if (nb <= 0) return 0;
    GammaReal* gr = kb->gr;
    ProfScope prof_scope(kb->basis, PROF_EW, 32.0 * (double)gr->n_half * nb);
    hipLaunchKernelGGL(k_gr_pack, gr_grid_unr(gr->n_half, (nb + 1) / 2), dim3(256), 0, kb->basis->stream, gr->n_half, nb,
                       gr->d_g, gr->d_mg, H, ldh, Z, ldz);
    HIPCHK(hipGetLastError());
    return 0;
}
int gamma_unpack_pairs(dftk_mi_kblock* kb, int nb, const cd* W, int64_t ldw, cd* H, int64_t ldh) {
    if (nb <= 0) return 0;
    GammaReal* gr = kb->gr;
    ProfScope prof_scope(kb->basis, PROF_EW, 32.0 * (double)gr->n_half * nb);
    hipLaunchKernelGGL(k_gr_unpack, gr_grid_unr(gr->n_half, (nb + 1) / 2), dim3(256), 0, kb->basis->stream, gr->n_half, nb,
                       gr->d_g, gr->d_mg, W, ldw, H, ldh);
    HIPCHK(hipGetLastError());
    return 0;
}
int gamma_pack_full(dftk_mi_kblock* kb, int nb, const cd* X, int64_t ldx, cd* Z, int64_t ldz) {
    if (nb <= 0) return 0;
    ProfScope prof_scope(kb->basis, PROF_EW, 32.0 * (double)kb->n_G * nb);
    hipLaunchKernelGGL(k_gr_pack_full, gr_grid_unr(kb->n_G, (nb + 1) / 2), dim3(256), 0, kb->basis->stream, kb->n_G, nb, X,
                       ldx, Z, ldz);
    HIPCHK(hipGetLastError());
    return 0;
}

int gamma_apply_H(dftk_mi_kblock* kb, int which, int nb, const cd* psi, int64_t ldpsi, cd* Hpsi, int64_t ldH) {
    if (nb <= 0) return 0;
    if (kb->sh_comm) return gamma_apply_H_sharded(kb, which, nb, psi, ldpsi, Hpsi, ldH);
    GammaReal* gr = kb->gr;
    dftk_mi_basis* b = kb->basis;
    const int nb2 = (nb + 1) / 2;
    const bool local = (which & 1) && kb->d_Vs != nullptr;
    const bool kinetic = which & 2;
    const int slot = prof_begin(b, PROF_APPLY_H, (double)nb);
    struct G {
        dftk_mi_basis* b;
        int s;
        ~G() { prof_end(b, s); }
    } guard{b, slot};
    CHK(gamma_ensure_buf(kb, 2 * (size_t)kb->n_G * nb2));
    cd* Z = gr->buf;
    cd* W = gr->buf + (size_t)kb->n_G * nb2;
    prof_count(b, PROF_A2A_MODEL, 16.0 * (double)gr->n_half * nb);
    prof_count(b, PROF_A2A_MODEL, 16.0 * (double)gr->n_half * nb);
    if ((which & 4) && kb->n_p > 0) prof_count(b, PROF_AR_MODEL, 16.0 * (double)kb->n_p * nb);
    CHK(gamma_pack_pairs(kb, nb, psi, ldpsi, Z, kb->n_G));
    CHK(launch_local_apply(kb, nb2, Z, kb->n_G, W, kb->n_G, kinetic, local));
    CHK(gamma_unpack_pairs(kb, nb, W, kb->n_G, Hpsi, ldH));
    if ((which & 4) && kb->n_p > 0) {
        CHK(gr_projectors(kb));
        CHK(apply_nonlocal_rows(kb, nb, gr->P_half, gr->n_half, gr->n_half, psi, ldpsi, Hpsi, ldH, true,
                                DFTK_MI_GEMM_REAL, nullptr));
    }
    return 0;
}

int gamma_density(dftk_mi_kblock* kb, int nb, const cd* psi, int64_t ldpsi, const double* w_h, double* rho) {
    if (nb <= 0) return 0;
    if (!kb->gr) {
        kb->gr = new GammaReal();
        kb->gr->on = false;
    }
    if (kb->sh_comm) return gamma_density_sharded(kb, nb, psi, ldpsi, w_h, rho);
    return gamma_density_bands(kb, nb, psi, ldpsi, w_h, rho);
}

int gamma_density_bands(dftk_mi_kblock* kb, int nb, const cd* psi, int64_t ldpsi, const double* w_h, double* rho) {
    if (nb <= 0) return 0;
    const int nb2 = (nb + 1) / 2;
    CHK(gamma_ensure_buf(kb, (size_t)kb->n_G * nb2));
    CHK(gamma_pack_full(kb, nb, psi, ldpsi, kb->gr->buf, kb->n_G));
    std::vector<double> wre(nb2), wim(nb2);
    for (int p = 0; p < nb2; ++p) {
        wre[p] = w_h[2 * p];
        wim[p] = (2 * p + 1 < nb) ? w_h[2 * p + 1] : 0.0;
    }
    return launch_density(kb, nb2, kb->gr->buf, kb->n_G, wre.data(), rho, wim.data());
}
```

dftk.jl_amd/csrc/lobpcg.cpp:

```cpp
#include "common.h"
#include "batch.h"
#include <cstdio>
#include <cstdlib>
#include <algorithm>
#include <atomic>
#include <cmath>
#include <complex>
#include <cstring>
#include <functional>
#include <numeric>
#include <random>
#include <utility>
#include <vector>

namespace {

const double EPS = 2.220446049250313e-16;
const int64_t DEFER_FETCH_MAX_ELEMS = 1 << 16;
const cd ONE = {1.0, 0.0}, ZERO = {0.0, 0.0}, MONE = {-1.0, 0.0};

struct Mat {
    cd* p;
    int64_t ld;
    int64_t rows;
// ... 6 lines not shown

struct Ctx {
    dftk_mi_kblock* kb;
    dftk_mi_basis* b;
    cd *O, *Rw, *invR, *BYX, *tmpS;
    cd* Vh;
    double *d_a, *d_b;
    int dstride = 0;
    std::vector<double> h;
    std::mt19937_64 rng;
    std::mt19937_64 rng_rep;
    bool replicated = false;
    bool small = false;
    int n_svd = 0;
    bool real_mode = false;
    bool holds_g0 = false;
    int rf = 0;
    int mm(char transA, int64_t m, int64_t n, int64_t k, cd alpha, const cd* A, int64_t lda, const cd* B, int64_t ldb,
           cd beta, cd* C, int64_t ldc, int upper = 0) {
        return zgemm(b, transA, m, n, k, alpha, A, lda, B, ldb, beta, C, ldc, upper | rf);
    }
    dftk_mi_comm* comm = nullptr;
    int reduce_c(cd* d, size_t n) {
        if (!small) prof_count(b, PROF_AR_MODEL, 16.0 * (double)n);
        return comm ? comm_allreduce(comm, c_b(), reinterpret_cast<double*>(d), 2 * n) : 0;
    }
    int reduce_d(double* d, size_t n) {
        if (!small) prof_count(b, PROF_AR_MODEL, 8.0 * (double)n);
        return comm ? comm_allreduce(comm, c_b(), d, n) : 0;
    }
    int reduce_norms(double* d, size_t n) {
        if (!small) prof_count(b, PROF_AR_MODEL, 8.0 * (double)n);
        return comm ? comm_allreduce_norms(comm, c_b(), d, n) : 0;
    }
    dftk_mi_basis* c_b() { return b; }
};

int h2d(dftk_mi_basis* b, void* dst_d, const void* src_h, size_t bytes) { return dev_h2d(b, dst_d, src_h, bytes); }
int stream_sync(dftk_mi_basis* b) { return dev_stream_sync(b); }
int d2h_sync(dftk_mi_basis* b, void* dst_h, const void* src_d, size_t bytes) { return dev_d2h_sync(b, dst_h, src_d, bytes); }

int d2h(Ctx& c, const double* d, int n) {
    if ((int)c.h.size() < n) c.h.resize(n);
    return d2h_sync(c.b, c.h.data(), d, n * sizeof(double));
}

int frob2(Ctx& c, const Mat& A, double* out) {
    CHK(ew_frob2(c.b, A.rows, A.cols, A.p, A.ld, c.d_a));
    CHK(d2h(c, c.d_a, A.cols));
    double s = 0.0;
    for (int i = 0; i < A.cols; ++i) s += c.h[i];
    *out = s;
    return 0;
}

int safe_cholesky(Ctx& c, int m, int* nchol_out, double* nR, double* nI) {
    int nchol = 0;
    double alpha = 100.0;
    for (;;) {
        if (nchol >= 5) {
            *nchol_out = 10000;
            return 0;
        }
        nchol += 1;
        CHK(ew_copy(c.b, m, m, c.O, m, c.Rw, m));
        int st = dense_potrf_trtri(c.b, m, c.Rw, m, c.invR, m, nR, nI, c.real_mode);
        if (st == 0) break;
        if (st != DFTK_MI_NUM_CHOLESKY) return st;
        double f2;
        CHK(frob2(c, Mat{c.O, m, m, m}, &f2));
        if (!std::isfinite(f2)) return DFTK_MI_NUM_NONFINITE;
        CHK(ew_add_diag(c.b, m, c.O, m, alpha * EPS * std::sqrt(f2)));
        alpha *= 10.0;
    }
    *nchol_out = nchol;
    return 0;
}

int randomize_column(Ctx& c, Mat X, int col);

int svd_polar(Ctx& c, Mat X, cd* scratch, int64_t scratch_ld);

int ortho_X(Ctx& c, Mat X, cd* tmp, double tol, int* nchol_total_out, double* growth_out, bool allow_svd = true,
            int64_t tmp_ld = 0, bool force_svd = false, const std::function<int()>* hook = nullptr, int* hook_out = nullptr) {
    double growth = 1.0;
    int nchol_total = 0;
    const int m = X.cols;
    if (m == 0) {
        *growth_out = 1.0;
        *nchol_total_out = 0;
        return 0;
    }
    if (tmp_ld <= 0) tmp_ld = X.rows;
    Mat src = X, dst{tmp, tmp_ld, X.rows, m};
    for (int pass = 0;; ++pass) {
        if (pass >= 30) {
            dftk_set_error("ortho!(X) did not reach the orthogonality tolerance in 30 Cholesky-QR passes");
            return DFTK_MI_NUM_CHOLESKY;
        }
        CHK(c.mm('C', m, m, src.rows, ONE, src.p, src.ld, src.p, src.ld, ZERO, c.O, m, 1));
        CHK(c.reduce_c(c.O, (size_t)m * m));
        CHK(ew_hermitize_upper(c.b, m, c.O, m));
        int nchol = 10000;
        double nR = 0, nI = 0;
        int st_chol = 0;
        if (!force_svd) st_chol = safe_cholesky(c, m, &nchol, &nR, &nI);
        if (st_chol != 0 && pass == 0 && hook) CHK(stream_sync(c.b));
        if (pass == 0 && hook) {
            const int hr = (*hook)();
            if (hr != 0) {
                *hook_out = hr;
                *growth_out = 1.0;
                *nchol_total_out = 0;
                return 0;
            }
        }
        if (st_chol != 0) return st_chol;
        nchol_total += nchol;
        if (nchol > 10) {
            if (!allow_svd) {
                dftk_set_error("ortho!(X): Cholesky keeps failing inside the SVD fallback");
                return DFTK_MI_NUM_CHOLESKY;
            }
            CHK(svd_polar(c, src, dst.p, dst.ld));
            if (src.p != X.p) CHK(ew_copy(c.b, X.rows, m, src.p, src.ld, X.p, X.ld));
            *growth_out = 1.0;
            *nchol_total_out = 100;
            c.n_svd += 1;
            return 0;
        }
        CHK(c.mm('N', src.rows, m, m, ONE, src.p, src.ld, c.invR, m, ZERO, dst.p, dst.ld,
                  2));
        std::swap(src, dst);
        growth *= nI;
        const double condR = nR * nI;
        const double est = EPS * condR * condR;
        if (nchol == 1 && est < tol) break;
    }
    if (src.p != X.p) CHK(ew_copy(c.b, X.rows, m, src.p, src.ld, X.p, X.ld));
    *growth_out = growth;
    *nchol_total_out = nchol_total;
    return 0;
}

int svd_polar(Ctx& c, Mat X, cd* scratch, int64_t scratch_ld) {
    const int m = X.cols;
    CHK(c.mm('C', m, m, X.rows, ONE, X.p, X.ld, X.p, X.ld, ZERO, c.O, m, 1));
    CHK(c.reduce_c(c.O, (size_t)m * m));
    CHK(ew_hermitize_upper(c.b, m, c.O, m));
    std::vector<double> w(m);
    CHK(dense_heev(c.b, m, c.O, m, w.data(), c.Rw, m));
    Mat W{scratch, scratch_ld, X.rows, m};
    CHK(c.mm('N', X.rows, m, m, ONE, X.p, X.ld, c.Rw, m, ZERO, W.p, W.ld));
    CHK(ew_colnorms(c.b, W.rows, m, W.p, W.ld, c.d_a));
    CHK(c.reduce_norms(c.d_a, m));
    CHK(d2h(c, c.d_a, m));
    double smax = 0.0;
    for (int i = 0; i < m; ++i) {
        if (!std::isfinite(c.h[i])) return DFTK_MI_NUM_NONFINITE;
        smax = std::max(smax, c.h[i]);
    }
    std::vector<double> sig(c.h.begin(), c.h.begin() + m);
    bool any_null = false;
    for (int i = 0; i < m; ++i)
        if (!(sig[i] > 1e-7 * smax) || smax == 0.0) {
            CHK(randomize_column(c, W, i));
            any_null = true;
        }
    if (any_null) {
        CHK(ew_colnorms(c.b, W.rows, m, W.p, W.ld, c.d_a));
        CHK(c.reduce_norms(c.d_a, m));
    }
    CHK(ew_scale_cols(c.b, W.rows, m, W.p, W.ld, c.d_a, true));
    CHK(ew_conj_transpose(c.b, m, c.Rw, m, c.Vh, m));
    int nch;
    double gr;
    CHK(ortho_X(c, W, X.p, 2 * EPS, &nch, &gr, false, X.ld));
    CHK(c.mm('N', X.rows, m, m, ONE, W.p, W.ld, c.Vh, m, ZERO, X.p, X.ld));
    return 0;
}

int randomize_column(Ctx& c, Mat X, int col) {
    std::normal_distribution<double> nd(0.0, 1.0);
    std::vector<double> v(2 * X.rows);
    std::mt19937_64& gen = c.replicated ? c.rng_rep : c.rng;
    for (auto& x : v) x = nd(gen);
    if (c.real_mode) {
        if (c.small)
            for (size_t i = 1; i < v.size(); i += 2) v[i] = 0.0;
        else if (c.holds_g0)
            v[1] = 0.0;
    }
    CHK(h2d(c.b, X.p + (int64_t)col * X.ld, v.data(), v.size() * sizeof(double)));
    return stream_sync(c.b);
}

bool contiguous(const std::vector<Mat>& Ys) {
    for (size_t i = 0; i + 1 < Ys.size(); ++i)
        if (Ys[i].ld != Ys[i + 1].ld || Ys[i].rows != Ys[i + 1].rows ||
            Ys[i].p + (int64_t)Ys[i].cols * Ys[i].ld != Ys[i + 1].p)
            return false;
    return !Ys.empty();
}
int total_cols(const std::vector<Mat>& Ys) {
    int n = 0;
    for (auto& Y : Ys) n += Y.cols;
    return n;
}

int ortho_XY(Ctx& c, Mat X, const std::vector<Mat>& Ys, cd* tmp, double tol, const double* norms_d = nullptr) {
    if (X.cols == 0) return 0;
    if (!norms_d) {
        CHK(ew_colnorms(c.b, X.rows, X.cols, X.p, X.ld, c.d_a));
        CHK(c.reduce_norms(c.d_a, X.cols));
        norms_d = c.d_a;
    }
    CHK(ew_scale_cols(c.b, X.rows, X.cols, X.p, X.ld, norms_d, true));
    int ny = 0;
    for (auto& Y : Ys) ny += Y.cols;
    std::vector<Mat> merged;
    if (Ys.size() > 1 && contiguous(Ys)) merged = {Mat{Ys[0].p, Ys[0].ld, Ys[0].rows, ny}};
    const std::vector<Mat>& Yl = merged.empty() ? Ys : merged;
    int niter = 1;
    std::vector<double> hb;
    for (;;) {
        int off = 0;
        for (auto& Y : Yl) {
            if (Y.cols == 0) continue;
            CHK(c.mm('C', Y.cols, X.cols, X.rows, ONE, Y.p, Y.ld, X.p, X.ld, ZERO, c.BYX + off, ny));
            off += Y.cols;
        }
        CHK(c.reduce_c(c.BYX, (size_t)ny * X.cols));
        off = 0;
        for (auto& Y : Yl) {
            if (Y.cols == 0) continue;
            CHK(c.mm('N', X.rows, X.cols, Y.cols, MONE, Y.p, Y.ld, c.BYX + off, ny, ONE, X.p, X.ld));
            off += Y.cols;
        }
        CHK(ew_colnorms(c.b, X.rows, X.cols, X.p, X.ld, c.d_a));
        CHK(c.reduce_norms(c.d_a, X.cols));
        const bool one_fetch = c.dstride > 0 && c.d_b == c.d_a + c.dstride && X.cols <= c.dstride;
        const bool defer = one_fetch && (int64_t)X.rows * X.cols <= DEFER_FETCH_MAX_ELEMS;
        if (one_fetch) {
            CHK(ew_frob2(c.b, ny, X.cols, c.BYX, ny, c.d_b));
            hb.resize(c.dstride + X.cols);
            if (defer)
                CHK(dev_d2h_async(c.b, hb.data(), c.d_a, hb.size() * sizeof(double)));
            else
                CHK(d2h_sync(c.b, hb.data(), c.d_a, hb.size() * sizeof(double)));
        } else {
            hb.resize(X.cols);
            CHK(d2h_sync(c.b, hb.data(), c.d_a, hb.size() * sizeof(double)));
        }
        double byx2 = 0.0;
        std::vector<int> dropped;
        bool nonfinite = false;
        auto evaluate = [&]() {
            byx2 = 0.0;
            dropped.clear();
            if (one_fetch)
                for (int j = 0; j < X.cols; ++j) byx2 += hb[c.dstride + j];
            for (int j = 0; j < X.cols; ++j) {
                if (!std::isfinite(hb[j])) nonfinite = true;
                if (hb[j] <= tol) dropped.push_back(j);
            }
        };
        bool speculated = false;
        int ninner = 0;
        double growth = 1.0;
        if (defer) {
            const std::function<int()> hook = [&]() -> int {
                evaluate();
                if (nonfinite) return 3;
                if (!dropped.empty()) return 2;
                if (std::sqrt(byx2) < tol && niter > 1) return 1;
                return 0;
            };
            int hr = 0;
            CHK(ortho_X(c, X, tmp, tol, &ninner, &growth, true, 0, false, &hook, &hr));
            if (hr == 3) return DFTK_MI_NUM_NONFINITE;
            if (hr == 1) break;
            speculated = hr == 0;
        } else {
            evaluate();
            if (nonfinite) return DFTK_MI_NUM_NONFINITE;
        }
        for (int j : dropped) {
            CHK(randomize_column(c, X, j));
            Mat xj = X.cols_from(j, 1);
            int o2 = 0;
            cd* scr = c.BYX + (int64_t)ny * X.cols;
            for (auto& Y : Yl) {
                if (Y.cols == 0) continue;
                CHK(c.mm('C', Y.cols, 1, X.rows, ONE, Y.p, Y.ld, xj.p, xj.ld, ZERO, scr + o2, ny));
                o2 += Y.cols;
            }
            CHK(c.reduce_c(scr, (size_t)ny));
            o2 = 0;
            for (auto& Y : Yl) {
                if (Y.cols == 0) continue;
                CHK(c.mm('N', X.rows, 1, Y.cols, MONE, Y.p, Y.ld, scr + o2, ny, ONE, xj.p, xj.ld));
                o2 += Y.cols;
            }
        }
        if (!one_fetch) CHK(frob2(c, Mat{c.BYX, ny, ny, X.cols}, &byx2));
        if (!speculated) {
            if (std::sqrt(byx2) < tol && niter > 1) break;
            CHK(ortho_X(c, X, tmp, tol, &ninner, &growth));
        }
        if (growth * EPS < tol) break;
        if (niter > 10) {
            CHK(svd_polar(c, X, tmp, X.rows));
            c.n_svd += 1;
            return 0;
        }
        niter += 1;
    }
    return 0;
}

typedef std::complex<double> zd;
static int host_ortho_small_impl(std::vector<zd>& Xio, int n, int m, const zd* Y, int ny, double tol, int* why, std::mt19937_64* gen,
                                 bool real);
int host_ortho_small(std::vector<zd>& Xio, int n, int m, const zd* Y, int ny, double tol, std::mt19937_64* gen = nullptr,
                     bool real = false) {
    int why = 0;
    const int ok = host_ortho_small_impl(Xio, n, m, Y, ny, tol, &why, gen, real);
    static const bool trace = getenv("DFTK_MI_KBATCH_TRACE") != nullptr;
    if (!ok && trace) fprintf(stderr, "[host cP ortho] %d x %d against %d columns: device path (reason %d)\n", n, m, ny, why);
    return ok;
}
static int host_ortho_small_impl(std::vector<zd>& Xio, int n, int m, const zd* Y, int ny, double tol, int* why, std::mt19937_64* gen,
                                 bool real) {
    std::vector<zd> X = Xio, T((size_t)n * m), BYX((size_t)ny * m), O((size_t)m * m), R((size_t)m * m), Ri((size_t)m * m);
    auto colnorm = [&](int j) {
        double s = 0.0;
        for (int i = 0; i < n; ++i) s += std::norm(X[i + (size_t)j * n]);
        return std::sqrt(s);
    };
    for (int j = 0; j < m; ++j) {
        const double f = 1.0 / colnorm(j);
        for (int i = 0; i < n; ++i) X[i + (size_t)j * n] *= f;
    }
    auto normest = [&](const std::vector<zd>& U) {
        double dmax = 0.0, off = 0.0;
        for (int j = 0; j < m; ++j)
            for (int i = 0; i <= j; ++i) {
                if (i == j)
                    dmax = std::max(dmax, std::abs(U[i + (size_t)j * m]));
                else
                    off += std::norm(U[i + (size_t)j * m]);
            }
        return dmax + std::sqrt(off);
    };
    for (int niter = 1;; ++niter) {
        double byx2 = 0.0;
        for (int j = 0; j < m; ++j)
            for (int a = 0; a < ny; ++a) {
                zd s = 0.0;
                for (int i = 0; i < n; ++i) s += std::conj(Y[i + (size_t)a * n]) * X[i + (size_t)j * n];
                BYX[a + (size_t)j * ny] = s;
                byx2 += std::norm(s);
            }
        for (int j = 0; j < m; ++j)
            for (int a = 0; a < ny; ++a) {
                const zd s = BYX[a + (size_t)j * ny];
                for (int i = 0; i < n; ++i) X[i + (size_t)j * n] -= Y[i + (size_t)a * n] * s;
            }
        for (int j = 0; j < m; ++j) {
            const double nj = colnorm(j);
            if (!std::isfinite(nj) || (nj <= tol && !gen)) {
                *why = 1;
                return 0;
            }
            if (nj <= tol) {
                std::normal_distribution<double> nd(0.0, 1.0);
                for (int i = 0; i < n; ++i) {
                    const double re = nd(*gen), im = nd(*gen);
                    X[i + (size_t)j * n] = zd(re, real ? 0.0 : im);
                }
                for (int a = 0; a < ny; ++a) {
                    zd s = 0.0;
                    for (int i = 0; i < n; ++i) s += std::conj(Y[i + (size_t)a * n]) * X[i + (size_t)j * n];
                    BYX[a + (size_t)j * ny] = s;
                }
                for (int a = 0; a < ny; ++a) {
                    const zd s = BYX[a + (size_t)j * ny];
                    for (int i = 0; i < n; ++i) X[i + (size_t)j * n] -= Y[i + (size_t)a * n] * s;
                }
            }
        }
        if (std::sqrt(byx2) < tol && niter > 1) break;
        double growth = 1.0;
        for (int pass = 0;; ++pass) {
            if (pass >= 30) {
                *why = 2;
                return 0;
            }
            for (int j = 0; j < m; ++j)
                for (int i = 0; i <= j; ++i) {
// ... 95 lines not shown
    Ctx c;
    c.kb = nullptr;
    c.b = b;
    cd* w = reinterpret_cast<cd*>(buf);
    cd* tmp = w;
    c.O = w + (size_t)n * m;
    c.Rw = c.O + (size_t)m * m;
    c.invR = c.Rw + (size_t)m * m;
    c.Vh = c.invR + (size_t)m * m;
    c.BYX = c.tmpS = nullptr;
    c.d_a = reinterpret_cast<double*>(c.Vh + (size_t)m * m);
    c.d_b = c.d_a + (m + 8);
    c.dstride = m + 8;
    c.rng.seed(0x9E3779B97F4A7C15ull);
    int nch = 0;
    double gr = 1.0;
    int st = ortho_X(c, Mat{X, ldx, n, m}, tmp, 2 * EPS, &nch, &gr, true, n, force_svd != 0);
    if (st == 0 && hipStreamSynchronize(b->stream) != hipSuccess) st = DFTK_MI_EHIP;
    hipFree(buf);
    if (n_chol) *n_chol = nch;
    if (used_svd) *used_svd = c.n_svd;
    return st;
}

std::atomic<int64_t> g_ax_reuse_count{0};
static int lobpcg_run_general(dftk_mi_kblock* kb, int M, cd* Xp, int64_t ldX, double tol, int miniter, int maxiter,
                              int n_conv_check, int use_tpa, uint64_t seed, double* lambda_h, double* resid_h, int* n_iter_out,
                              int* converged_out, int64_t* n_matvec_out) {
    dftk_mi_basis* b = kb->basis;
    if (!(kb->n_G > 3 * (int64_t)M)) {
        dftk_set_error("The eigenproblem is too small (n_G=%lld, M=%d): N > 3M required", (long long)kb->n_G, M);
        return DFTK_MI_NUM_TOO_SMALL;
    }
    dftk_mi_comm* comm = (kb->sh_comm && comm_size(kb->sh_comm) > 1) ? kb->sh_comm : nullptr;
    const int64_t row0 = comm ? (*kb->sh_rows)[comm_rank(comm)] : 0;
    const bool real_mode = kb->gr && kb->gr->on;
    const int64_t N = real_mode ? gamma_local_rows(kb) : comm ? (*kb->sh_rows)[comm_rank(comm) + 1] - row0 : kb->n_G;
    const double* kin = !use_tpa ? nullptr : real_mode ? kb->gr->d_kin_half + gamma_row0(kb) : kb->d_kin + row0;
    auto apply_H = [&](int nb, const cd* in, int64_t ldin, cd* out, int64_t ldout) -> int {
        if (real_mode) return gamma_apply_H(kb, 7, nb, in, ldin, out, ldout);
        return dftk_mi_apply_H(kb, nb, reinterpret_cast<const dftk_mi_cplx*>(in), ldin,
                               reinterpret_cast<dftk_mi_cplx*>(out), ldout);
    };
    if (N < 1) {
        dftk_set_error("sharded k-block: empty row slab on rank %d", comm_rank(comm));
        return DFTK_MI_EINVAL;
    }
    if (n_conv_check <= 0 || n_conv_check > M) n_conv_check = M;
    const double ortho_tol = 2 * EPS;

    const size_t blk = (size_t)N * M;
    const size_t nbig = 14;
    const size_t m3 = 3 * (size_t)M;
    const size_t small_elems = m3 * m3 * 2
                               + m3 * M * 2
                               + (size_t)M * M * 4
                               + (2 * (size_t)M + m3) * (M + 1);
    const size_t dbl = 9 * (size_t)(M + 8);
    const size_t need = (nbig * blk + small_elems) * sizeof(cd) + dbl * sizeof(double) + m3 * sizeof(int) + 1024;
    const bool reuse_asked = kb->ax_reuse_next;
    kb->ax_reuse_next = false;
    cd* ax_prev = kb->ax_keep;
    const int64_t ax_prev_ld = kb->ax_ld;
    const bool ax_shape_ok = ax_prev != nullptr && kb->ax_M == M && kb->ax_rows == N;
    kb->ax_keep = nullptr;
    if (need > kb->lob_bytes) {
        CHK(host_wait(b));
        if (kb->lob_buf) HIPCHK(hipFree(kb->lob_buf));
        kb->lob_buf = nullptr;
        kb->lob_bytes = 0;
        ax_prev = nullptr;
        HIPCHK(dftk_scratch_malloc((void**)&kb->lob_buf, need));
        kb->lob_bytes = need;
    }
    bool reuse_ax = reuse_asked && ax_shape_ok && ax_prev != nullptr && kb->d_Vs != nullptr && kb->d_Vs_ax != nullptr;
    cd* w = kb->lob_buf;
    auto take = [&](size_t n) {
        cd* r = w;
        w += n;
        return r;
    };
    Mat Yb[2] = {Mat{take(3 * blk), N, N, 3 * M}, Mat{take(3 * blk), N, N, 3 * M}};
    Mat AYb[2] = {Mat{take(3 * blk), N, N, 3 * M}, Mat{take(3 * blk), N, N, 3 * M}};
    int cur = 0;
    auto Pblk = [&](const Mat& buf, int nact) { return buf.cols_from(M, nact); };
    auto Rblk = [&](const Mat& buf, int nact, bool has_p) { return buf.cols_from(M + (has_p ? nact : 0), nact); };
    Mat newR{take(blk), N, N, M};
    cd* tmp = take(blk);
    cd* G = take(m3 * m3);
    cd* V = take(m3 * m3);
    cd* cP = take(m3 * M);
    Ctx c;
    c.kb = kb;
    c.b = b;
    c.comm = comm;
    c.real_mode = real_mode;
    c.holds_g0 = real_mode && gamma_row0(kb) == 0;
    c.rf = real_mode ? DFTK_MI_GEMM_REAL : 0;
    c.tmpS = take(m3 * M);
    c.O = take((size_t)M * M);
    c.Rw = take((size_t)M * M);
    c.invR = take((size_t)M * M);
    c.Vh = take((size_t)M * M);
    c.BYX = take((2 * (size_t)M + m3) * (M + 1));
    double* dd = reinterpret_cast<double*>(w);
    c.d_a = dd;
    c.d_b = dd + (M + 8);
    c.dstride = M + 8;
    double* d_lam = dd + 2 * (M + 8);
    double* d_norms = dd + 3 * (M + 8);
    double* d_mk = dd + 4 * (M + 8);
    double* d_xx = dd + 5 * (M + 8);
    double* d_rn = dd + 6 * (M + 8);
    c.rng.seed((seed ? seed : 0x9E3779B97F4A7C15ull) + 0x632BE59BD9B4E019ull * (uint64_t)comm_rank(comm));
    c.rng_rep.seed((seed ? seed : 0x9E3779B97F4A7C15ull) ^ 0xD1B54A32D192ED03ull);
    Mat X = Yb[0].cols_from(0, M), AX = AYb[0].cols_from(0, M);
    kb->last_AX = real_mode ? nullptr : AX.p;

    Mat Xuser{Xp, ldX, N, M};
    if (real_mode)
        CHK(gamma_lobpcg_load(kb, M, Xp, ldX, X.p, X.ld, true));
    else
        CHK(ew_copy(b, N, M, Xuser.p, Xuser.ld, X.p, X.ld));
    std::vector<double> resid_history((size_t)M * (maxiter + 1), 0.0);
    auto RH = [&](int i, int it) -> double& { return resid_history[(size_t)i + (size_t)M * it]; };
    std::vector<double> full_lam(M, 0.0);

    {
        int nch;
        double gr;
        CHK(ortho_X(c, X, tmp, ortho_tol, &nch, &gr));
        if (reuse_ax && !(nch == 1)) reuse_ax = false;
    }
    int64_t n_matvec = M;
    if (reuse_ax) {
        g_ax_reuse_count.fetch_add(1);
        dftk_mi_basis* bb = b;
        const size_t cube = (size_t)bb->nz * bb->ny * bb->nxp;
        if (!kb->d_dVs) HIPCHK(hipMalloc((void**)&kb->d_dVs, cube * sizeof(double)));
        CHK(ew_sub_real(bb, (int64_t)cube, kb->d_Vs, kb->d_Vs_ax, kb->d_dVs));
        if (ax_prev != AX.p) {
            CHK(c.mm('N', N, M, M, ONE, ax_prev, ax_prev_ld, c.invR, M, ZERO, AX.p, AX.ld, 2));
        } else {
            CHK(c.mm('N', N, M, M, ONE, ax_prev, ax_prev_ld, c.invR, M, ZERO, newR.p, newR.ld, 2));
            CHK(ew_copy(b, N, M, newR.p, newR.ld, AX.p, AX.ld));
        }
        double* const Vs_bound = kb->d_Vs;
        kb->d_Vs = kb->d_dVs;
        const int st_dv = real_mode ? gamma_apply_H(kb, 1, M, X.p, X.ld, newR.p, newR.ld)
                                    : dftk_mi_apply_H_parts(kb, 1, M, reinterpret_cast<const dftk_mi_cplx*>(X.p), X.ld,
                                                            reinterpret_cast<dftk_mi_cplx*>(newR.p), newR.ld);
        kb->d_Vs = Vs_bound;
        CHK(st_dv);
        CHK(ew_add(b, N, M, newR.p, newR.ld, AX.p, AX.ld));
        static const bool ax_check = getenv("DFTK_MI_AX_REUSE_CHECK") != nullptr;
        if (ax_check) {
            CHK(apply_H(M, X.p, X.ld, newR.p, newR.ld));
            std::vector<cd> h1((size_t)N * M), h2((size_t)N * M);
            CHK(stream_sync(b));
            HIPCHK(hipMemcpy(h1.data(), AX.p, h1.size() * sizeof(cd), hipMemcpyDeviceToHost));
            HIPCHK(hipMemcpy(h2.data(), newR.p, h2.size() * sizeof(cd), hipMemcpyDeviceToHost));
            double worst = 0.0, nrm = 0.0;
            int wc = -1;
            for (int j = 0; j < M; ++j) {
                double d = 0.0, r = 0.0;
                for (int64_t i = 0; i < N; ++i) {
                    const cd a = h1[(size_t)i + (size_t)j * N], f = h2[(size_t)i + (size_t)j * N];
                    d += (a.x - f.x) * (a.x - f.x) + (a.y - f.y) * (a.y - f.y);
                    r += f.x * f.x + f.y * f.y;
                }
                nrm = std::max(nrm, std::sqrt(r));
                if (std::sqrt(d) > worst) {
                    worst = std::sqrt(d);
                    wc = j;
                }
            }
            fprintf(stderr, "[ax reuse check] M=%d N=%lld: max column error %.3e (column %d), max ||H x|| %.3e\n", M, (long long)N, worst,
                    wc, nrm);
        }
    } else {
        CHK(apply_H(M, X.p, X.ld, AX.p, AX.ld));
    }
    CHK(ew_coldots(b, N, M, X.p, X.ld, AX.p, AX.ld, c.d_a));
    CHK(ew_coldots(b, N, M, X.p, X.ld, X.p, X.ld, c.d_b));
    CHK(c.reduce_d(c.d_a, 2 * (size_t)(M + 8)));
    CHK(d2h(c, c.d_a, 2 * (M + 8)));
    for (int i = 0; i < M; ++i) {
        if (!std::isfinite(c.h[i])) {
            dftk_set_error("non-finite values in H*X");
            return DFTK_MI_NUM_NONFINITE;
        }
        full_lam[i] = c.h[i] / c.h[(M + 8) + i];
    }

    int nlocked = 0, niter = 0, lo = 0;
    int status_final = 0;
    bool finished = false;
    int final_iter = maxiter;
    int ncx = 0;

    while (true) {
        const int nact = M - lo;
        Mat &Yc = Yb[cur], &AYc = AYb[cur], &Yn = Yb[cur ^ 1], &AYn = AYb[cur ^ 1];
        X = Yc.cols_from(0, M);
        AX = AYc.cols_from(0, M);
        Mat Xa = X.cols_from(lo), AXa = AX.cols_from(lo);
        Mat Ra = Rblk(Yc, nact, niter > 1), ARa = Rblk(AYc, nact, niter > 1), Pa = Pblk(Yc, nact), APa = Pblk(AYc, nact);
        Mat nX = niter > 0 ? Yn.cols_from(lo, nact) : Xa, nAX = niter > 0 ? AYn.cols_from(lo, nact) : AXa;
        Mat nR = newR.cols_from(0, nact);
        std::vector<Mat> Ys, AYs;
        int nY = 0;
        cd* cX = V;
        bool host_cp = false;
        std::vector<zd> h_cX;
        if (niter > 0) {
            CHK(apply_H(nact, Ra.p, Ra.ld, ARa.p, ARa.ld));
            n_matvec += nact;
            if (niter > 1) {
                Ys = {Xa, Pa, Ra};
                AYs = {AXa, APa, ARa};
            } else {
                Ys = {Xa, Ra};
                AYs = {AXa, ARa};
            }
            nY = (int)Ys.size() * nact;
            if (contiguous(Ys) && contiguous(AYs)) {
                CHK(c.mm('C', nY, nY, N, ONE, Ys[0].p, Ys[0].ld, AYs[0].p, AYs[0].ld, ZERO, G, nY, 1));
                CHK(c.reduce_c(G, (size_t)nY * nY));
            } else {
                for (size_t ib = 0; ib < Ys.size(); ++ib)
                    for (size_t ia = 0; ia <= ib; ++ia)
                        CHK(c.mm('C', nact, nact, N, ONE, Ys[ia].p, Ys[ia].ld, AYs[ib].p, AYs[ib].ld, ZERO,
                                  G + (int64_t)ia * nact + (int64_t)ib * nact * nY, nY));
                CHK(c.reduce_c(G, (size_t)nY * nY));
            }
            CHK(ew_hermitize_upper(b, nY, G, nY));
            std::vector<double> wv(nY);
// ... 34 lines not shown
                    break;
            }
        }
        const int tgt = niter > 0 ? (cur ^ 1) : cur;
        if (nlocked >= n_conv_check) {
            cur = tgt;
            final_iter = niter;
            finished = true;
            break;
        }
        const int newly_locked = nlocked - prev_nlocked;
        const int lenXn = nact - newly_locked;

        Mat nP = Pblk(Yb[tgt], lenXn), nAP = Pblk(AYb[tgt], lenXn);
        if (niter > 0) {
            Mat cPm{cP, nY, nY, lenXn};
            bool cp_done = false;
            if (host_cp) {
                std::vector<zd> h_cP(h_cX.begin() + (size_t)newly_locked * nY, h_cX.begin() + (size_t)(newly_locked + lenXn) * nY);
                for (int a = 0; a < lenXn - newly_locked; ++a)
                    if (2 * newly_locked + a < nY) h_cP[(size_t)(2 * newly_locked + a) + (size_t)a * nY] -= 1.0;
                if (host_ortho_small(h_cP, nY, lenXn, h_cX.data(), ncx, ortho_tol, &c.rng_rep, c.real_mode)) {
                    CHK(h2d(b, cP, h_cP.data(), h_cP.size() * sizeof(cd)));
                    cp_done = true;
                }
            }
            if (!cp_done) {
                CHK(ew_copy(b, nY, lenXn, cX + (int64_t)newly_locked * nY, nY, cP, nY));
                CHK(ew_sub_identity_shifted(b, nY, lenXn - newly_locked, cP, nY, 2 * newly_locked));
                std::vector<Mat> cXs = {Mat{cX, nY, nY, ncx}};
                NoComm replicated(c);
                CHK(ortho_XY(c, cPm, cXs, c.tmpS, ortho_tol));
            }
            CHK(hcat_mul(c, Ys, cP, nY, lenXn, nP));
            CHK(hcat_mul(c, AYs, cP, nY, lenXn, nAP));
        }
        for (int i = 0; i < nact; ++i)
            if (!(std::fabs(h_xx[i] - 1.0) < std::sqrt(EPS))) {
                dftk_set_error("LOBPCG is badly failing to keep the vectors normalized (column %d: %g; iteration %d, "
                               "%d locked, %d active, %d ranks)", lo + i, h_xx[i], niter, nlocked, nact, comm_size(comm));
                return DFTK_MI_NUM_NORMALIZATION;
            }
        if (newly_locked > 0) {
            CHK(ew_copy(b, N, newly_locked, Yb[tgt].p + (int64_t)lo * N, N, Yb[tgt ^ 1].p + (int64_t)lo * N, N));
            CHK(ew_copy(b, N, newly_locked, AYb[tgt].p + (int64_t)lo * N, N, AYb[tgt ^ 1].p + (int64_t)lo * N, N));
        }
        lo = nlocked;
        cur = tgt;
        X = Yb[cur].cols_from(0, M);
        AX = AYb[cur].cols_from(0, M);
        Mat Rn = Rblk(Yb[cur], lenXn, niter > 0);
        CHK(ew_tpa(b, N, lenXn, nR.p + (int64_t)newly_locked * nR.ld, nR.ld, Rn.p, Rn.ld, kin, d_mk + newly_locked,
                   d_rn));
        CHK(c.reduce_norms(d_rn, lenXn));
        std::vector<Mat> Zs = {X};
        if (niter > 0) Zs.push_back(nP);
        CHK(ortho_XY(c, Rn, Zs, tmp, ortho_tol, d_rn));
        static const bool dbg_check = getenv("DFTK_MI_LOBPCG_CHECK") != nullptr;
        if (dbg_check) {
            const int nc = M + (niter > 0 ? 2 : 1) * lenXn;
            CHK(c.mm('C', nc, nc, N, ONE, Yb[cur].p, N, Yb[cur].p, N, ZERO, G, nc));
            CHK(c.reduce_c(G, (size_t)nc * nc));
            std::vector<double> hg(2 * (size_t)nc * nc);
            CHK(d2h_sync(b, hg.data(), G, hg.size() * sizeof(double)));
            double worst[3][3] = {{0}};
            auto blk_of = [&](int j) { return j < M ? 0 : (niter > 0 && j < M + lenXn ? 1 : 2); };
            for (int j = 0; j < nc; ++j)
                for (int i = 0; i < nc; ++i) {
                    const double re = hg[2 * ((size_t)i + (size_t)j * nc)] - (i == j ? 1.0 : 0.0);
                    const double im = hg[2 * ((size_t)i + (size_t)j * nc) + 1];
                    double& w = worst[blk_of(i)][blk_of(j)];
                    w = std::max(w, std::sqrt(re * re + im * im));
                }
            fprintf(stderr, "[lobpcg-check rank %d] it %d locked %d act %d  XX %.1e XP %.1e XR %.1e PP %.1e PR %.1e RR %.1e\n",
                    comm_rank(comm), niter, nlocked, lenXn, worst[0][0], worst[0][1], worst[0][2], worst[1][1],
                    worst[1][2], worst[2][2]);
        }

        if (niter >= maxiter) break;
        niter += 1;
    }
    X = Yb[cur].cols_from(0, M);
    AX = AYb[cur].cols_from(0, M);
    kb->last_AX = real_mode ? nullptr : AX.p;
    if (!finished) final_iter = maxiter;
    (void)status_final;

    std::vector<int> perm(M);
    std::iota(perm.begin(), perm.end(), 0);
    bool sorted = std::is_sorted(full_lam.begin(), full_lam.end());
    if (!sorted) {
        std::stable_sort(perm.begin(), perm.end(), [&](int a, int d) { return full_lam[a] < full_lam[d]; });
        int* d_perm = reinterpret_cast<int*>(dd + 7 * (M + 8));
        CHK(h2d(b, d_perm, perm.data(), M * sizeof(int)));
        CHK(ew_gather_cols(b, N, M, X.p, X.ld, d_perm, tmp, N));
        CHK(ew_copy(b, N, M, tmp, N, X.p, X.ld));
        CHK(ew_gather_cols(b, N, M, AX.p, AX.ld, d_perm, tmp, N));
        CHK(ew_copy(b, N, M, tmp, N, AX.p, AX.ld));
        CHK(stream_sync(b));
    }
    if (real_mode)
        CHK(gamma_lobpcg_store(kb, M, X.p, X.ld, Xp, ldX));
    else
        CHK(ew_copy(b, N, M, X.p, X.ld, Xuser.p, Xuser.ld));
    double maxres = 0.0;
    for (int i = 0; i < M; ++i) {
        lambda_h[i] = full_lam[perm[i]];
        resid_h[i] = RH(perm[i], final_iter);
    }
    for (int i = 0; i < n_conv_check; ++i) maxres = std::max(maxres, resid_h[i]);
    if (!kb->lob_hist) kb->lob_hist = new std::vector<double>();
    kb->lob_hist->assign((size_t)M * (final_iter + 1), 0.0);
    for (int it = 0; it <= final_iter; ++it)
        for (int i = 0; i < M; ++i) (*kb->lob_hist)[(size_t)i + (size_t)M * it] = RH(perm[i], it);
    kb->lob_hist_M = M;
    kb->lob_hist_iters = final_iter;
    kb->lob_n_svd = c.n_svd;
    *converged_out = (maxres < tol) ? 1 : 0;
    *n_iter_out = final_iter;
    *n_matvec_out = n_matvec;
    if (kb->d_Vs != nullptr && !batching()) {
        const size_t cube = (size_t)b->nz * b->ny * b->nxp;
        if (!kb->d_Vs_ax) HIPCHK(hipMalloc((void**)&kb->d_Vs_ax, cube * sizeof(double)));
        HIPCHK(hipMemcpyAsync(kb->d_Vs_ax, kb->d_Vs, cube * sizeof(double), hipMemcpyDeviceToDevice, b->stream));
        kb->ax_keep = AX.p;
        kb->ax_ld = AX.ld;
        kb->ax_M = M;
        kb->ax_rows = N;
    }
    return stream_sync(b);
}


std::atomic<int64_t> g_small_calls{0}, g_small_restarts{0};

bool lobpcg_small_eligible(const dftk_mi_kblock* kb, int M) {
    static const bool off = getenv("DFTK_MI_LOBPCG_SMALL") && atoi(getenv("DFTK_MI_LOBPCG_SMALL")) == 0;
    if (off || getenv("DFTK_MI_KBATCH_SEQUENTIAL") != nullptr || kb->sh_comm || (kb->gr && kb->gr->on)) return false;
    return M >= 1 && M <= 8 && kb->n_G * (int64_t)M <= DEFER_FETCH_MAX_ELEMS && kb->n_G > 3 * (int64_t)M;
}

static int rec_ortho(dftk_mi_basis* b, Mat X, const cd* Y, int64_t ldy, int ny, const double* norms_d, double tol, double* res4) {
    BOp o;
    o.b = b;
    o.type = BOP_ORTHO;
    o.n = X.rows;
    o.m = X.cols;
    o.k = ny;
    o.C = X.p;
    o.ldc = X.ld;
    o.A = Y;
    o.lda = ldy;
    o.W = norms_d;
    o.s0 = tol;
    o.host = res4;
    return batch_record(std::move(o));
}

static int lobpcg_run_small(dftk_mi_kblock* kb, int M, cd* Xp, int64_t ldX, double tol, int miniter, int maxiter,
                            int n_conv_check, int use_tpa, uint64_t seed, double* lambda_h, double* resid_h, int* n_iter_out,
                            int* converged_out, int64_t* n_matvec_out, bool* restart) {
    dftk_mi_basis* b = kb->basis;
    *restart = false;
    const int64_t N = kb->n_G;
    const double* kin = use_tpa ? kb->d_kin : nullptr;
    if (n_conv_check <= 0 || n_conv_check > M) n_conv_check = M;
    const double ortho_tol = 2 * EPS;
    const size_t blk = (size_t)N * M;
    const size_t nbig = 14;
    const size_t m3 = 3 * (size_t)M;
    const size_t small_elems = m3 * m3 * 2 + m3 * M * 2 + (size_t)M * M * 4 + (2 * (size_t)M + m3) * (M + 1);
    const int DS = (int)m3 + 8;
    const size_t dbl = 9 * (size_t)DS;
    const size_t need = (nbig * blk + small_elems) * sizeof(cd) + dbl * sizeof(double) + m3 * sizeof(int) + 1024;
    if (need > kb->lob_bytes) {
        CHK(host_wait(b));
        if (kb->lob_buf) HIPCHK(hipFree(kb->lob_buf));
        kb->lob_buf = nullptr;
        kb->lob_bytes = 0;
        HIPCHK(dftk_scratch_malloc((void**)&kb->lob_buf, need));
        kb->lob_bytes = need;
    }
    cd* w = kb->lob_buf;
// ... 396 lines not shown
```

include/dftk_mi355x.h:

```cpp
#ifndef DFTK_MI355X_H
#define DFTK_MI355X_H

#include <stddef.h>
#include <stdint.h>

#ifdef __cplusplus
extern "C" {
#endif

typedef struct { double re, im; } dftk_mi_cplx;

typedef struct dftk_mi_basis  dftk_mi_basis;
typedef struct dftk_mi_kblock dftk_mi_kblock;
typedef struct dftk_mi_comm   dftk_mi_comm;

#define DFTK_MI_OK                 0
#define DFTK_MI_EINVAL            (-1)
#define DFTK_MI_EHIP              (-2)
#define DFTK_MI_ERCCL             (-3)
#define DFTK_MI_ENOGPU            (-100)
#define DFTK_MI_NUM_NONFINITE       1
#define DFTK_MI_NUM_CHOLESKY        2
#define DFTK_MI_NUM_NORMALIZATION   3
#define DFTK_MI_NUM_EIGEN           4
// ... 90 lines not shown
                         double* lambda_h, double* resid_h, int* n_iter, int* converged, int64_t* n_matvec, int* status);
int dftk_mi_density_accumulate_multi(int n_kblocks, dftk_mi_kblock* const* kbs, const int* n_bands,
                                     const dftk_mi_cplx* const* psi_d, const int64_t* ld_psi, const double* weights_h,
                                     double* rho_d);
int dftk_mi_density_accumulate_multi2(int n_kblocks, dftk_mi_kblock* const* kbs, const int* n_bands,
                                      const dftk_mi_cplx* const* psi_d, const int64_t* ld_psi, const double* weights_h,
                                      double* rho_d, const double* weights2_h, double* rho2_d);
int dftk_mi_band_kinetic_multi(int n_kblocks, dftk_mi_kblock* const* kbs, const int* n_bands,
                               const dftk_mi_cplx* const* psi_d, const int64_t* ld_psi, double* out_h);
int dftk_mi_batch_stats(int64_t* rounds, int64_t* ops, int64_t* merged_launches, int64_t* sequential_ops);
int dftk_mi_lobpcg_small_stats(int64_t* calls, int64_t* restarts);
int dftk_mi_ortho_small(dftk_mi_basis* basis, int64_t n, int m, dftk_mi_cplx* X_d, int64_t ldx, int ny, const dftk_mi_cplx* Y_d,
                        int64_t ldy, const double* norms_d, double tol, double* res4_h);
int dftk_mi_lobpcg_history(dftk_mi_kblock* kb, int* M, int* n_iter, double* hist_h, size_t cap, int* n_svd);
int dftk_mi_kblock_reuse_AX(dftk_mi_kblock* kb, int on);
int dftk_mi_ax_reuse_count(int64_t* calls);

const dftk_mi_cplx* dftk_mi_lobpcg_last_AX(dftk_mi_kblock* kb);

int dftk_mi_columnwise_norms(dftk_mi_basis* basis, int64_t n, int m, const dftk_mi_cplx* X_d, int64_t ldx,
                             double* norms_h );
int dftk_mi_columnwise_dots(dftk_mi_basis* basis, int64_t n, int m, const dftk_mi_cplx* A_d, int64_t lda,
                            const dftk_mi_cplx* B_d, int64_t ldb, dftk_mi_cplx* dots_h );
int dftk_mi_ortho_qr(dftk_mi_basis* basis, int64_t n, int m, dftk_mi_cplx* X_d, int64_t ldx, int force_svd,
                     int* n_chol, int* used_svd);
int dftk_mi_tpa_precondprep(dftk_mi_kblock* kb, int m, const dftk_mi_cplx* X_d, int64_t ldx, double* mean_kin_h);
int dftk_mi_tpa_ldiv(dftk_mi_kblock* kb, int m, const dftk_mi_cplx* R_d, int64_t ldr, const double* mean_kin_h,
                     double default_shift, dftk_mi_cplx* Y_d, int64_t ldy);
int dftk_mi_block_residual(dftk_mi_kblock* kb, int m, const dftk_mi_cplx* AX_d, int64_t lda,
                           const dftk_mi_cplx* X_d, int64_t ldx, const double* lambda_h, dftk_mi_cplx* R_d,
                           int64_t ldr, double* norms_h, double* mean_kin_h, double* xx_h);

int dftk_mi_zgemm(dftk_mi_basis* basis, char transA, int64_t m, int64_t n, int64_t k,
                  dftk_mi_cplx alpha, const dftk_mi_cplx* A_d, int64_t lda,
                  const dftk_mi_cplx* B_d, int64_t ldb, dftk_mi_cplx beta,
                  dftk_mi_cplx* C_d, int64_t ldc);
#define DFTK_MI_GEMM_UPPER 1
#define DFTK_MI_GEMM_B_UPPER 2
#define DFTK_MI_GEMM_REAL 8
int dftk_mi_zgemm_ex(dftk_mi_basis* basis, char transA, int64_t m, int64_t n, int64_t k,
                     dftk_mi_cplx alpha, const dftk_mi_cplx* A_d, int64_t lda,
                     const dftk_mi_cplx* B_d, int64_t ldb, dftk_mi_cplx beta,
                     dftk_mi_cplx* C_d, int64_t ldc, int flags);
int dftk_mi_heev(dftk_mi_basis* basis, int n, dftk_mi_cplx* A_d, int64_t lda, double* W_h,
                 dftk_mi_cplx* V_d, int64_t ldv);
int dftk_mi_heev_lowest(dftk_mi_basis* basis, int n, int nev, dftk_mi_cplx* A_d, int64_t lda, double* W_h,
                        dftk_mi_cplx* V_d, int64_t ldv);
int dftk_mi_heev_sigma_host(int n, const double* diag_h, int nev, double* sigma, double* gap_guess,
                            int* hold_iterations, double norm_bound);
int dftk_mi_potrf_trtri(dftk_mi_basis* basis, int n, dftk_mi_cplx* A_d, int64_t lda,
                        dftk_mi_cplx* invR_d, int64_t ldi);
int dftk_mi_potrf_trtri_real(dftk_mi_basis* basis, int n, dftk_mi_cplx* A_d, int64_t lda,
                             dftk_mi_cplx* invR_d, int64_t ldi);

int dftk_mi_comm_get_unique_id(char id_out[128]);
int dftk_mi_comm_init_rank(const char id[128], int n_ranks, int rank, int device,
                           dftk_mi_comm** comm_out);
typedef int (*dftk_mi_allreduce_fn)(void* user, double* buf_h, size_t n);
typedef int (*dftk_mi_alltoallv_fn)(void* user, const double* send_h, const size_t* send_counts,
                                    const size_t* send_offsets, double* recv_h, const size_t* recv_counts,
                                    const size_t* recv_offsets);
int dftk_mi_comm_create_host(int n_ranks, int rank, int device, dftk_mi_allreduce_fn allreduce,
                             dftk_mi_alltoallv_fn alltoallv, void* user, dftk_mi_comm** comm_out);
int dftk_mi_comm_destroy(dftk_mi_comm* comm);
int dftk_mi_comm_describe(const dftk_mi_comm* comm, int* backend, int* n_ranks, int* version);
int dftk_mi_comm_rank(const dftk_mi_comm* comm);
int dftk_mi_comm_size(const dftk_mi_comm* comm);
int dftk_mi_allreduce_sum_f64(dftk_mi_comm* comm, double* buf_d, size_t n, void* stream);

int dftk_mi_kblock_set_shard(dftk_mi_kblock* kb, dftk_mi_comm* comm, const int64_t* row_starts_h);

int dftk_mi_kblock_set_gamma_real(dftk_mi_kblock* kb, int on);
int dftk_mi_gamma_half_size(dftk_mi_kblock* kb, int64_t* n_half);
int dftk_mi_gamma_tables_host(int nx, int ny, int nz, int64_t n_G, const int64_t* mapping0_h, int64_t* n_half,
                              int32_t* row_h, int32_t* partner_row_h);
int dftk_mi_gamma_compress(dftk_mi_kblock* kb, int m, const dftk_mi_cplx* X_d, int64_t ldx, dftk_mi_cplx* Xh_d,
                           int64_t ldh);
int dftk_mi_gamma_compress_aligned(dftk_mi_kblock* kb, int m, const dftk_mi_cplx* X_d, int64_t ldx, dftk_mi_cplx* Xh_d,
                                   int64_t ldh);
int dftk_mi_gamma_expand(dftk_mi_kblock* kb, int m, const dftk_mi_cplx* Xh_d, int64_t ldh, dftk_mi_cplx* X_d,
                         int64_t ldx);
int dftk_mi_gamma_apply_H(dftk_mi_kblock* kb, int which, int n_bands, const dftk_mi_cplx* psih_d, int64_t ld_psi,
                          dftk_mi_cplx* Hpsih_d, int64_t ld_Hpsi);
int dftk_mi_density_accumulate_real(dftk_mi_kblock* kb, int n_bands, const dftk_mi_cplx* psi_d, int64_t ld_psi,
                                    const double* weight_h, double* rho_d);

int dftk_mi_shard_plan_host(int n_ranks, int rank, int n_bands, const int64_t* row_starts_h, int* band_starts,
                            int64_t* slab_off, int64_t* slab_cnt, int64_t* band_off, int64_t* band_cnt);

int dftk_mi_prof_enable(dftk_mi_basis* basis, int on);
int dftk_mi_prof_get(dftk_mi_basis* basis, int family, double* total_ms, double* work, int64_t* launches);
typedef struct dftk_mi_anderson dftk_mi_anderson;
int dftk_mi_anderson_create(dftk_mi_basis* basis, int64_t n, int m, double maxcond, double errorfactor,
                            dftk_mi_anderson** out);
int dftk_mi_anderson_destroy(dftk_mi_anderson* acc);
int dftk_mi_anderson_reset(dftk_mi_anderson* acc);
int dftk_mi_anderson_history(const dftk_mi_anderson* acc);
int dftk_mi_anderson_step(dftk_mi_anderson* acc, const double* x_d, double alpha, const double* Pf_d, double* x_next_d,
                          int* n_history );
int dftk_mi_chi0_mix(dftk_mi_kblock* cube_kblock, int n_comp, const double* recip_lattice_h, const double* poisson_d,
                     const double* ldos_d, double dvol, int dielectric, double kTF, double eps_r, const double* dF_d,
                     double reltol, int krylovdim, int maxiter, double* drho_d, int* n_applies, int* converged);

int dftk_mi_launch_count(int64_t* launches, int64_t* host_syncs);

int dftk_mi_step_sums(dftk_mi_basis* basis, int64_t n, const double* a_d, const double* b_d, const double* c_d, double* out_h);

int dftk_mi_fermi_bisection(int n_k, const int* n_bands, const double* eig, const double* kweights, int smearing,
                            double temperature, double filled, double n_electrons, double lo, double hi, double* eF_out);
int dftk_mi_prof_zgemm_shapes(dftk_mi_basis* basis, int cap, int64_t* rows6, double* ms, int* count);

int dftk_mi_diag_mfma_peak(dftk_mi_basis* basis, int waves_per_simd, int iters, double* tflops);

int dftk_mi_zgemm_plan_host(char transA, int64_t m, int64_t n, int64_t k, int flags, int* out12);
int dftk_mi_jacobi_schedule_host(int n, int round, int* n_blocks, int* pairs ,
                                 int* where );
int dftk_mi_fft_plan_host(int n, int* n_radices, int* radices , int* pos );
int dftk_mi_sphere_tables_host(int nx, int ny, int nz, int64_t n_G, const int64_t* mapping0_h,
                               int64_t* n_lines, int* n_zplanes, int64_t* line_id ,
                               int64_t* line_start );

#ifdef __cplusplus
}
#endif
#endif
```

Baseline: 5.945.

## Fuse gamma half-format pack into FFT kernels and remove LOBPCG buffer copies

Adds a HALF variant of the x-axis scatter and gather FFT kernels that read the compressed gamma-point half-format pairs directly through an inverse index table, so the separate pack pass is skipped. Adds an accumulate mode to the gamma unpack and apply_H, so the AX-reuse delta potential adds into AX in place instead of going through a temporary and an ew_add. Orthogonalization and the final sort now ping-pong between the double buffers instead of copying back through tmp. This cuts memory traffic and kernel launches, but adds index indirection inside the FFT kernels and more complex buffer-ownership logic.

New measurement: 5.993, median of 6. Within noise of the previous version (+0.8%).

```diff
diff --git a/dftk.jl_amd/_lib.py b/dftk.jl_amd/_lib.py
--- a/dftk.jl_amd/_lib.py
+++ b/dftk.jl_amd/_lib.py
@@ -97,6 +97,7 @@
     "dftk_mi_gamma_compress_aligned": (C.c_int, [C.c_void_p, C.c_int, C.c_void_p, _i64, C.c_void_p, _i64]),
     "dftk_mi_gamma_expand": (C.c_int, [C.c_void_p, C.c_int, C.c_void_p, _i64, C.c_void_p, _i64]),
     "dftk_mi_gamma_apply_H": (C.c_int, [C.c_void_p, C.c_int, C.c_int, C.c_void_p, _i64, C.c_void_p, _i64]),
+    "dftk_mi_gamma_apply_H_add": (C.c_int, [C.c_void_p, C.c_int, C.c_int, C.c_void_p, _i64, C.c_void_p, _i64]),
     "dftk_mi_density_accumulate_real": (C.c_int, [C.c_void_p, C.c_int, C.c_void_p, _i64, C.c_void_p, C.c_void_p]),
     "dftk_mi_shard_plan_host": (C.c_int, [C.c_int, C.c_int, C.c_int, C.c_void_p, C.c_void_p, C.c_void_p, C.c_void_p,
                                           C.c_void_p, C.c_void_p]),
diff --git a/dftk.jl_amd/csrc/api.cpp b/dftk.jl_amd/csrc/api.cpp
--- a/dftk.jl_amd/csrc/api.cpp
+++ b/dftk.jl_amd/csrc/api.cpp
@@ -1153,6 +1153,17 @@
                          reinterpret_cast<cd*>(Hpsih_d), ld_Hpsi);
 }
 
+extern "C" int dftk_mi_gamma_apply_H_add(dftk_mi_kblock* kb, int which, int n_bands, const dftk_mi_cplx* psih_d,
+                                         int64_t ld_psi, dftk_mi_cplx* Hpsih_d, int64_t ld_Hpsi) {
+    CHK(gamma_ready(kb));
+    if (!psih_d || !Hpsih_d || n_bands < 0 || (which & ~7) || ld_psi < gamma_local_rows(kb) ||
+        ld_Hpsi < gamma_local_rows(kb))
+        return DFTK_MI_EINVAL;
+    HIPCHK(hipSetDevice(kb->basis->device));
+    return gamma_apply_H(kb, which, n_bands, reinterpret_cast<const cd*>(psih_d), ld_psi,
+                         reinterpret_cast<cd*>(Hpsih_d), ld_Hpsi, true);
+}
+
 extern "C" int dftk_mi_density_accumulate_real(dftk_mi_kblock* kb, int n_bands, const dftk_mi_cplx* psi_d,
                                                int64_t ld_psi, const double* weight_h, double* rho_d) {
     if (!kb || !psi_d || !weight_h || !rho_d || n_bands < 0 || ld_psi < local_rows(kb)) return DFTK_MI_EINVAL;
diff --git a/dftk.jl_amd/csrc/common.h b/dftk.jl_amd/csrc/common.h
--- a/dftk.jl_amd/csrc/common.h
+++ b/dftk.jl_amd/csrc/common.h
@@ -131,6 +131,7 @@
     bool on = false;
     int64_t n_half = 0;
     int *d_g = nullptr, *d_mg = nullptr;
+    int* d_inv = nullptr;
     double* d_kin_half = nullptr;
     cd* P_half = nullptr;
     const cd* P_src = nullptr;
@@ -180,8 +181,12 @@
 };
 
 int fft_ensure_scratch(dftk_mi_basis* b, dftk_mi_kblock* kb, int nb);
+struct HalfPairs {
+    const int* inv;
+    int n_real;
+};
 int launch_local_apply(dftk_mi_kblock* kb, int nb, const cd* psi, int64_t ldpsi, cd* out,
-                       int64_t ldout, bool add_kinetic, bool have_local);
+                       int64_t ldout, bool add_kinetic, bool have_local, const HalfPairs* half = nullptr);
 int launch_ifft_to_cube(dftk_mi_kblock* kb, const cd* c, cd* cube, int nb = 1);
 int launch_fft_from_cube(dftk_mi_kblock* kb, const cd* cube, cd* c, int nb = 1);
 int launch_density(dftk_mi_kblock* kb, int nb, const cd* psi, int64_t ldpsi, const double* w_h, double* rho,
@@ -273,11 +278,12 @@
 int gamma_compress(dftk_mi_kblock* kb, int m, const cd* X, int64_t ldx, cd* H, int64_t ldh);
 int gamma_compress_aligned(dftk_mi_kblock* kb, int m, const cd* X, int64_t ldx, cd* H, int64_t ldh);
 int gamma_expand(dftk_mi_kblock* kb, int m, const cd* H, int64_t ldh, cd* X, int64_t ldx);
-int gamma_apply_H(dftk_mi_kblock* kb, int which, int nb, const cd* psi, int64_t ldpsi, cd* Hpsi, int64_t ldH);
+int gamma_apply_H(dftk_mi_kblock* kb, int which, int nb, const cd* psi, int64_t ldpsi, cd* Hpsi, int64_t ldH,
+                  bool accumulate = false);
 int gamma_density(dftk_mi_kblock* kb, int nb, const cd* psi, int64_t ldpsi, const double* w_h, double* rho);
 int gamma_ensure_buf(dftk_mi_kblock* kb, size_t elems);
 int gamma_pack_pairs(dftk_mi_kblock* kb, int nb, const cd* H, int64_t ldh, cd* Z, int64_t ldz);
-int gamma_unpack_pairs(dftk_mi_kblock* kb, int nb, const cd* W, int64_t ldw, cd* H, int64_t ldh);
+int gamma_unpack_pairs(dftk_mi_kblock* kb, int nb, const cd* W, int64_t ldw, cd* H, int64_t ldh, bool accumulate = false);
 int gamma_pack_full(dftk_mi_kblock* kb, int nb, const cd* X, int64_t ldx, cd* Z, int64_t ldz);
 int gamma_gather_P(dftk_mi_kblock* kb, int ncols, const cd* P, int64_t ldP, cd* Ph, int64_t ldh, double* asym_mag_h);
 int gamma_density_bands(dftk_mi_kblock* kb, int nb, const cd* psi, int64_t ldpsi, const double* w_h, double* rho);
diff --git a/dftk.jl_amd/csrc/fft_kernels.hip b/dftk.jl_amd/csrc/fft_kernels.hip
--- a/dftk.jl_amd/csrc/fft_kernels.hip
+++ b/dftk.jl_amd/csrc/fft_kernels.hip
@@ -298,13 +298,25 @@
     double w2;
 };
 
-template <bool GEN>
+__device__ __forceinline__ cd half_pair_at(const cd* __restrict__ ha, const cd* __restrict__ hb,
+                                           const int* __restrict__ inv, int c) {
+    const int h = inv[c];
+    const int j = h < 0 ? ~h : h;
+    const cd a = ha[j];
+    const cd b = hb ? hb[j] : make_double2(0.0, 0.0);
+    if (j == 0) return make_double2(a.x, b.x);
+    const double s = 0.70710678118654752;
+    return h < 0 ? make_double2(s * (a.x + b.y), s * (b.x - a.y)) : make_double2(s * (a.x - b.y), s * (a.y + b.x));
+}
+
+template <bool GEN, bool HALF = false>
 __global__ __launch_bounds__(FFT_THREADS) void k_xbwd_scatter(FftAxis ax, int nxp, int n_lines,
                                                               const int* __restrict__ line_start,
                                                               const int* __restrict__ cpos,
                                                               const cd* __restrict__ psi, int64_t ldpsi,
                                                               cd* __restrict__ T1, int64_t T1_stride,
-                                                              const FftJob* __restrict__ jobs) {
+                                                              const FftJob* __restrict__ jobs,
+                                                              const int* __restrict__ inv = nullptr, int n_real = 0) {
     constexpr int FFT_LS = FFT_LS_X;
     cd* buf = reinterpret_cast<cd*>(dftk_smem);
     cd* tw = buf + ax.n * FFT_LS;
@@ -325,7 +337,13 @@
     const int line = l0 + l;
     if (line < n_lines) {
         const int c0 = line_start[line], c1 = line_start[line + 1];
-        for (int c = c0 + j; c < c1; c += FFT_TPL) buf[cpos[c] * FFT_LS + l] = p[c];
+        if constexpr (HALF) {
+            const cd* ha = psi + (int64_t)(2 * band) * ldpsi;
+            const cd* hb = (2 * band + 1 < n_real) ? ha + ldpsi : nullptr;
+            for (int c = c0 + j; c < c1; c += FFT_TPL) buf[cpos[c] * FFT_LS + l] = half_pair_at(ha, hb, inv, c);
+        } else {
+            for (int c = c0 + j; c < c1; c += FFT_TPL) buf[cpos[c] * FFT_LS + l] = p[c];
+        }
     }
     __syncthreads();
     fft_tile<FFT_LS, false, GEN>(buf, tw, ax, +1.0, l, j);
@@ -785,7 +803,7 @@
         t1[(int64_t)ln * nxp + x] = buf[line_ypos[ln] * FFT_LS + l];
 }
 
-template <bool GEN>
+template <bool GEN, bool HALF = false>
 __global__ __launch_bounds__(FFT_THREADS, YFWD_MIN_BLOCKS) void k_xfwd_gather(FftAxis ax, int nxp, int n_lines,
                                                              const int* __restrict__ line_start,
                                                              const int* __restrict__ cpos,
@@ -793,7 +811,8 @@
                                                              const double* __restrict__ kin,
                                                              const cd* __restrict__ psi, int64_t ldpsi,
                                                              cd* __restrict__ out, int64_t ldout,
-                                                             const FftJob* __restrict__ jobs) {
+                                                             const FftJob* __restrict__ jobs,
+                                                             const int* __restrict__ inv = nullptr, int n_real = 0) {
     constexpr int FFT_LS = FFT_LS_X;
     cd* buf = reinterpret_cast<cd*>(dftk_smem);
     cd* tw = buf + ax.n * FFT_LS;
@@ -830,7 +849,13 @@
             cd v = buf[cpos[c] * FFT_LS + l];
             if (kin != nullptr) {
                 const double k = kin[c];
-                const cd q = p[c];
+                cd q;
+                if constexpr (HALF) {
+                    const cd* ha = psi + (int64_t)(2 * band) * ldpsi;
+                    q = half_pair_at(ha, (2 * band + 1 < n_real) ? ha + ldpsi : nullptr, inv, c);
+                } else {
+                    q = p[c];
+                }
                 v.x = fma(k, q.x, v.x);
                 v.y = fma(k, q.y, v.y);
             }
@@ -1002,6 +1027,16 @@
             CHK(set_lds_attr(KERNEL<false>, LDS));                                                   \
             hipLaunchKernelGGL((KERNEL<false>), GRID, dim3(FFT_THREADS), LDS, STREAM, __VA_ARGS__);  \
         }                                                                                            \
+    } while (0)
+#define LAUNCH_FFT_HALF(KERNEL, AX, GRID, LDS, STREAM, ...)                                                \
+    do {                                                                                                   \
+        if (axis_generic(AX)) {                                                                            \
+            CHK(set_lds_attr(KERNEL<true, true>, LDS));                                                    \
+            hipLaunchKernelGGL((KERNEL<true, true>), GRID, dim3(FFT_THREADS), LDS, STREAM, __VA_ARGS__);   \
+        } else {                                                                                           \
+            CHK(set_lds_attr(KERNEL<false, true>, LDS));                                                   \
+            hipLaunchKernelGGL((KERNEL<false, true>), GRID, dim3(FFT_THREADS), LDS, STREAM, __VA_ARGS__);  \
+        }                                                                                                  \
     } while (0)
 #define LAUNCH_ZPASS(MODE, AX, GRID, LDS, STREAM, ...)                                                      \
     do {                                                                                                    \
@@ -1092,7 +1127,7 @@
     return Strides{(int64_t)kb->n_lines * b->nxp, (int64_t)kb->nzx * b->ny * b->nxp};
 }
 
-static int run_AB(dftk_mi_kblock* kb, int nbb, const cd* psi, int64_t ldpsi) {
+static int run_AB(dftk_mi_kblock* kb, int nbb, const cd* psi, int64_t ldpsi, const HalfPairs* half = nullptr) {
     dftk_mi_basis* b = kb->basis;
     const Strides st = strides(kb);
     const int gl = (int)((kb->n_lines + FFT_L - 1) / FFT_L);
@@ -1101,8 +1136,14 @@
     const double t1b = 16.0 * (double)kb->n_lines * b->nxp, t2b = 16.0 * (double)kb->nzx * b->ny * b->nxp;
     (void)Ncube;
     int ps = prof_begin(b, PROF_FFT_A, (16.0 * kb->n_G + t1b) * nbb);
+    if (half)
+        LAUNCH_FFT_HALF(k_xbwd_scatter, b->ax[0], dim3(gl, nbb), lds_bytes(b->nx, FFT_LS_X), b->stream, b->ax[0], b->nxp,
+                        (int)kb->n_lines, kb->d_line_start, kb->d_cpos, psi, ldpsi, b->T1, st.s1, (const FftJob*)nullptr,
+                        half->inv, half->n_real);
+    else
     LAUNCH_FFT(k_xbwd_scatter, b->ax[0], dim3(gl, nbb), lds_bytes(b->nx, FFT_LS_X), b->stream, b->ax[0],
-                       b->nxp, (int)kb->n_lines, kb->d_line_start, kb->d_cpos, psi, ldpsi, b->T1, st.s1, (const FftJob*)nullptr);
+                       b->nxp, (int)kb->n_lines, kb->d_line_start, kb->d_cpos, psi, ldpsi, b->T1, st.s1, (const FftJob*)nullptr,
+                       (const int*)nullptr, 0);
     prof_end(b, ps);
     ps = prof_begin(b, PROF_FFT_B, (t1b + t2b) * nbb);
     LAUNCH_FFT(k_ybwd, b->ax[1], dim3(nxt, kb->nzx, nbb), lds_bytes(b->ny), b->stream, b->ax[1],
@@ -1112,7 +1153,7 @@
 }
 
 static int run_DE(dftk_mi_kblock* kb, int nbb, const double* kin, const cd* psi, int64_t ldpsi, cd* out,
-                  int64_t ldout) {
+                  int64_t ldout, const HalfPairs* half = nullptr) {
     dftk_mi_basis* b = kb->basis;
     const Strides st = strides(kb);
     const int gl = (int)((kb->n_lines + FFT_L - 1) / FFT_L);
@@ -1125,17 +1166,26 @@
                        b->nxp, b->ny, kb->d_zls, kb->d_line_ypos, b->T2, st.s2, b->T1, st.s1, (const FftJob*)nullptr);
     prof_end(b, ps);
     ps = prof_begin(b, PROF_FFT_E, (t1b + (kin ? 40.0 : 16.0) * kb->n_G) * nbb);
+    if (half && kin)
+        LAUNCH_FFT_HALF(k_xfwd_gather, b->ax[0], dim3(gl, nbb), lds_bytes(b->nx, FFT_LS_X), b->stream, b->ax[0], b->nxp,
+                        (int)kb->n_lines, kb->d_line_start, kb->d_cpos, b->T1, st.s1, kin, psi, ldpsi, out, ldout,
+                        (const FftJob*)nullptr, half->inv, half->n_real);
+    else
     LAUNCH_FFT(k_xfwd_gather, b->ax[0], dim3(gl, nbb), lds_bytes(b->nx, FFT_LS_X), b->stream, b->ax[0],
                        b->nxp, (int)kb->n_lines, kb->d_line_start, kb->d_cpos, b->T1, st.s1, kin, psi, ldpsi, out,
-                       ldout, (const FftJob*)nullptr);
+                       ldout, (const FftJob*)nullptr, (const int*)nullptr, 0);
     prof_end(b, ps);
     return 0;
 }
 
 int launch_local_apply(dftk_mi_kblock* kb, int nb, const cd* psi, int64_t ldpsi, cd* out, int64_t ldout,
-                       bool add_kinetic, bool have_local) {
+                       bool add_kinetic, bool have_local, const HalfPairs* half) {
     dftk_mi_basis* b = kb->basis;
     if (!have_local || kb->d_Vs == nullptr) {
+        if (half) {
+            dftk_set_error("launch_local_apply: the half-format source needs the FFT pipeline (a local potential)");
+            return DFTK_MI_EINVAL;
+        }
         return launch_kinetic_only(kb, nb, psi, ldpsi, out, ldout, false, add_kinetic);
     }
     CHK(check_lds(b));
@@ -1145,8 +1195,10 @@
     const int nxt = b->nxp / FFT_L;
     for (int b0 = 0; b0 < nb; b0 += batch) {
         const int nbb = (nb - b0) < batch ? (nb - b0) : batch;
-        const cd* p = psi + (int64_t)b0 * ldpsi;
-        CHK(run_AB(kb, nbb, p, ldpsi));
+        const cd* p = psi + (int64_t)b0 * ldpsi * (half ? 2 : 1);
+        const HalfPairs hb{half ? half->inv : nullptr, half ? half->n_real - 2 * b0 : 0};
+        const HalfPairs* hp = half ? &hb : nullptr;
+        CHK(run_AB(kb, nbb, p, ldpsi, hp));
         const int pc = prof_begin(b, PROF_FFT_C, 2.0 * 16.0 * (double)kb->nzx * b->ny * b->nxp * nbb +
                                                      8.0 * (double)b->nz * b->ny * b->nxp);
         const RegZ rz{b, b->stream, zpass_grid(b, nbb), kb->nzx, kb->z_lo, nbb, kb->d_Vs, b->T2, st.s2, nullptr, nullptr, nullptr,
@@ -1157,7 +1209,7 @@
         LAUNCH_ZPASS(0, b->ax[2], zpass_grid(b, nbb), lds_bytes(b->nz), b->stream, b->ax[2], b->nx, b->nxp, b->ny, kb->nzx, nbb, kb->d_zpos, kb->d_Vs, b->T2, st.s2,
                            (cd*)nullptr, (const FftJob*)nullptr);
         prof_end(b, pc);
-        CHK(run_DE(kb, nbb, add_kinetic ? kb->d_kin : nullptr, p, ldpsi, out + (int64_t)b0 * ldout, ldout));
+        CHK(run_DE(kb, nbb, add_kinetic ? kb->d_kin : nullptr, p, ldpsi, out + (int64_t)b0 * ldout, ldout, hp));
     }
     HIPCHK(hipGetLastError());
     return 0;
diff --git a/dftk.jl_amd/csrc/gamma_kernels.hip b/dftk.jl_amd/csrc/gamma_kernels.hip
--- a/dftk.jl_amd/csrc/gamma_kernels.hip
+++ b/dftk.jl_amd/csrc/gamma_kernels.hip
@@ -225,7 +225,8 @@
 }
 
 __global__ __launch_bounds__(256) void k_gr_unpack(int64_t nh, int nb, const int* __restrict__ g, const int* __restrict__ mg,
-                                                   const cd* __restrict__ W, int64_t ldw, cd* __restrict__ H, int64_t ldh) {
+                                                   const cd* __restrict__ W, int64_t ldw, cd* __restrict__ H, int64_t ldh,
+                                                   int accumulate) {
     const int64_t j0 = (int64_t)blockIdx.x * GR_ROWS + threadIdx.x;
     const int p = blockIdx.y;
     const cd* w = W + (int64_t)p * ldw;
@@ -247,8 +248,23 @@
         const int64_t j = j0 + u * 256;
         if (j >= nh) continue;
         const double s = j ? GR_ISQRT2 : 0.5;
-        H[j + (int64_t)(2 * p) * ldh] = make_double2(s * (wg[u].x + wm[u].x), s * (wg[u].y - wm[u].y));
-        if (2 * p + 1 < nb) H[j + (int64_t)(2 * p + 1) * ldh] = make_double2(s * (wg[u].y + wm[u].y), s * (wm[u].x - wg[u].x));
+        cd va = make_double2(s * (wg[u].x + wm[u].x), s * (wg[u].y - wm[u].y));
+        cd vb = make_double2(s * (wg[u].y + wm[u].y), s * (wm[u].x - wg[u].x));
+        cd* pa = H + j + (int64_t)(2 * p) * ldh;
+        cd* pb = H + j + (int64_t)(2 * p + 1) * ldh;
+        const bool has_b = 2 * p + 1 < nb;
+        if (accumulate) {
+            const cd oa = *pa;
+            va.x += oa.x;
+            va.y += oa.y;
+            if (has_b) {
+                const cd ob = *pb;
+                vb.x += ob.x;
+                vb.y += ob.y;
+            }
+        }
+        *pa = va;
+        if (has_b) *pb = vb;
     }
 }
 
@@ -335,6 +351,13 @@
     HIPCHK(hipMalloc((void**)&gr->d_kin_half, nh * sizeof(double)));
     HIPCHK(hipMemcpy(gr->d_g, g.data(), nh * sizeof(int), hipMemcpyHostToDevice));
     HIPCHK(hipMemcpy(gr->d_mg, mg.data(), nh * sizeof(int), hipMemcpyHostToDevice));
+    std::vector<int32_t> inv((size_t)kb->n_G);
+    for (int64_t j = 0; j < nh; ++j) {
+        inv[mg[j]] = ~(int32_t)j;
+        inv[g[j]] = (int32_t)j;
+    }
+    HIPCHK(hipMalloc((void**)&gr->d_inv, kb->n_G * sizeof(int)));
+    HIPCHK(hipMemcpy(gr->d_inv, inv.data(), kb->n_G * sizeof(int), hipMemcpyHostToDevice));
     HIPCHK(hipMemcpy(gr->d_kin_half, kin.data(), nh * sizeof(double), hipMemcpyHostToDevice));
     gr->half_rows.clear();
     if (kb->sh_comm) {
@@ -363,7 +386,7 @@
 
 void gamma_destroy(GammaReal* gr) {
     if (!gr) return;
-    void* ptrs[] = {gr->d_g, gr->d_mg, gr->d_kin_half, gr->P_half, gr->buf};
+    void* ptrs[] = {gr->d_g, gr->d_mg, gr->d_inv, gr->d_kin_half, gr->P_half, gr->buf};
     for (void* p : ptrs)
         if (p) hipFree(p);
     delete gr;
@@ -461,12 +484,12 @@
     HIPCHK(hipGetLastError());
     return 0;
 }
-int gamma_unpack_pairs(dftk_mi_kblock* kb, int nb, const cd* W, int64_t ldw, cd* H, int64_t ldh) {
+int gamma_unpack_pairs(dftk_mi_kblock* kb, int nb, const cd* W, int64_t ldw, cd* H, int64_t ldh, bool accumulate) {
     if (nb <= 0) return 0;
     GammaReal* gr = kb->gr;
-    ProfScope prof_scope(kb->basis, PROF_EW, 32.0 * (double)gr->n_half * nb);
+    ProfScope prof_scope(kb->basis, PROF_EW, (accumulate ? 48.0 : 32.0) * (double)gr->n_half * nb);
     hipLaunchKernelGGL(k_gr_unpack, gr_grid_unr(gr->n_half, (nb + 1) / 2), dim3(256), 0, kb->basis->stream, gr->n_half, nb,
-                       gr->d_g, gr->d_mg, W, ldw, H, ldh);
+                       gr->d_g, gr->d_mg, W, ldw, H, ldh, accumulate ? 1 : 0);
     HIPCHK(hipGetLastError());
     return 0;
 }
@@ -479,9 +502,15 @@
     return 0;
 }
 
-int gamma_apply_H(dftk_mi_kblock* kb, int which, int nb, const cd* psi, int64_t ldpsi, cd* Hpsi, int64_t ldH) {
+int gamma_apply_H(dftk_mi_kblock* kb, int which, int nb, const cd* psi, int64_t ldpsi, cd* Hpsi, int64_t ldH, bool accumulate) {
     if (nb <= 0) return 0;
-    if (kb->sh_comm) return gamma_apply_H_sharded(kb, which, nb, psi, ldpsi, Hpsi, ldH);
+    if (kb->sh_comm) {
+        if (accumulate) {
+            dftk_set_error("gamma_apply_H: accumulate is not available on a plane-wave sharded block");
+            return DFTK_MI_EINVAL;
+        }
+        return gamma_apply_H_sharded(kb, which, nb, psi, ldpsi, Hpsi, ldH);
+    }
     GammaReal* gr = kb->gr;
     dftk_mi_basis* b = kb->basis;
     const int nb2 = (nb + 1) / 2;
@@ -493,15 +522,20 @@
         int s;
         ~G() { prof_end(b, s); }
     } guard{b, slot};
-    CHK(gamma_ensure_buf(kb, 2 * (size_t)kb->n_G * nb2));
-    cd* Z = gr->buf;
-    cd* W = gr->buf + (size_t)kb->n_G * nb2;
+    CHK(gamma_ensure_buf(kb, (local ? 1 : 2) * (size_t)kb->n_G * nb2));
+    cd* W = gr->buf;
+    cd* Z = local ? nullptr : gr->buf + (size_t)kb->n_G * nb2;
     prof_count(b, PROF_A2A_MODEL, 16.0 * (double)gr->n_half * nb);
     prof_count(b, PROF_A2A_MODEL, 16.0 * (double)gr->n_half * nb);
     if ((which & 4) && kb->n_p > 0) prof_count(b, PROF_AR_MODEL, 16.0 * (double)kb->n_p * nb);
-    CHK(gamma_pack_pairs(kb, nb, psi, ldpsi, Z, kb->n_G));
-    CHK(launch_local_apply(kb, nb2, Z, kb->n_G, W, kb->n_G, kinetic, local));
-    CHK(gamma_unpack_pairs(kb, nb, W, kb->n_G, Hpsi, ldH));
+    if (local) {
+        const HalfPairs hp{gr->d_inv, nb};
+        CHK(launch_local_apply(kb, nb2, psi, ldpsi, W, kb->n_G, kinetic, true, &hp));
+    } else {
+        CHK(gamma_pack_pairs(kb, nb, psi, ldpsi, Z, kb->n_G));
+        CHK(launch_local_apply(kb, nb2, Z, kb->n_G, W, kb->n_G, kinetic, false));
+    }
+    CHK(gamma_unpack_pairs(kb, nb, W, kb->n_G, Hpsi, ldH, accumulate));
     if ((which & 4) && kb->n_p > 0) {
         CHK(gr_projectors(kb));
         CHK(apply_nonlocal_rows(kb, nb, gr->P_half, gr->n_half, gr->n_half, psi, ldpsi, Hpsi, ldH, true,
diff --git a/dftk.jl_amd/csrc/lobpcg.cpp b/dftk.jl_amd/csrc/lobpcg.cpp
--- a/dftk.jl_amd/csrc/lobpcg.cpp
+++ b/dftk.jl_amd/csrc/lobpcg.cpp
@@ -112,10 +112,12 @@
 int svd_polar(Ctx& c, Mat X, cd* scratch, int64_t scratch_ld);
 
 int ortho_X(Ctx& c, Mat X, cd* tmp, double tol, int* nchol_total_out, double* growth_out, bool allow_svd = true,
-            int64_t tmp_ld = 0, bool force_svd = false, const std::function<int()>* hook = nullptr, int* hook_out = nullptr) {
+            int64_t tmp_ld = 0, bool force_svd = false, const std::function<int()>* hook = nullptr, int* hook_out = nullptr,
+            Mat* where = nullptr) {
     double growth = 1.0;
     int nchol_total = 0;
     const int m = X.cols;
+    if (where) *where = X;
     if (m == 0) {
         *growth_out = 1.0;
         *nchol_total_out = 0;
@@ -153,7 +155,10 @@
                 return DFTK_MI_NUM_CHOLESKY;
             }
             CHK(svd_polar(c, src, dst.p, dst.ld));
-            if (src.p != X.p) CHK(ew_copy(c.b, X.rows, m, src.p, src.ld, X.p, X.ld));
+            if (where)
+                *where = src;
+            else if (src.p != X.p)
+                CHK(ew_copy(c.b, X.rows, m, src.p, src.ld, X.p, X.ld));
             *growth_out = 1.0;
             *nchol_total_out = 100;
             c.n_svd += 1;
@@ -167,7 +172,10 @@
         const double est = EPS * condR * condR;
         if (nchol == 1 && est < tol) break;
     }
-    if (src.p != X.p) CHK(ew_copy(c.b, X.rows, m, src.p, src.ld, X.p, X.ld));
+    if (where)
+        *where = src;
+    else if (src.p != X.p)
+        CHK(ew_copy(c.b, X.rows, m, src.p, src.ld, X.p, X.ld));
     *growth_out = growth;
     *nchol_total_out = nchol_total;
     return 0;
@@ -252,22 +260,23 @@
     if (Ys.size() > 1 && contiguous(Ys)) merged = {Mat{Ys[0].p, Ys[0].ld, Ys[0].rows, ny}};
     const std::vector<Mat>& Yl = merged.empty() ? Ys : merged;
     int niter = 1;
+    Mat cur = X, oth{tmp, X.rows, X.rows, X.cols};
     std::vector<double> hb;
     for (;;) {
         int off = 0;
         for (auto& Y : Yl) {
             if (Y.cols == 0) continue;
-            CHK(c.mm('C', Y.cols, X.cols, X.rows, ONE, Y.p, Y.ld, X.p, X.ld, ZERO, c.BYX + off, ny));
+            CHK(c.mm('C', Y.cols, X.cols, X.rows, ONE, Y.p, Y.ld, cur.p, cur.ld, ZERO, c.BYX + off, ny));
             off += Y.cols;
         }
         CHK(c.reduce_c(c.BYX, (size_t)ny * X.cols));
         off = 0;
         for (auto& Y : Yl) {
             if (Y.cols == 0) continue;
-            CHK(c.mm('N', X.rows, X.cols, Y.cols, MONE, Y.p, Y.ld, c.BYX + off, ny, ONE, X.p, X.ld));
+            CHK(c.mm('N', X.rows, X.cols, Y.cols, MONE, Y.p, Y.ld, c.BYX + off, ny, ONE, cur.p, cur.ld));
             off += Y.cols;
         }
-        CHK(ew_colnorms(c.b, X.rows, X.cols, X.p, X.ld, c.d_a));
+        CHK(ew_colnorms(c.b, X.rows, X.cols, cur.p, cur.ld, c.d_a));
         CHK(c.reduce_norms(c.d_a, X.cols));
         const bool one_fetch = c.dstride > 0 && c.d_b == c.d_a + c.dstride && X.cols <= c.dstride;
         const bool defer = one_fetch && (int64_t)X.rows * X.cols <= DEFER_FETCH_MAX_ELEMS;
@@ -298,6 +307,7 @@
         bool speculated = false;
         int ninner = 0;
         double growth = 1.0;
+        Mat res = cur;
         if (defer) {
             const std::function<int()> hook = [&]() -> int {
                 evaluate();
@@ -307,7 +317,7 @@
                 return 0;
             };
             int hr = 0;
-            CHK(ortho_X(c, X, tmp, tol, &ninner, &growth, true, 0, false, &hook, &hr));
+            CHK(ortho_X(c, cur, oth.p, tol, &ninner, &growth, true, oth.ld, false, &hook, &hr, &res));
             if (hr == 3) return DFTK_MI_NUM_NONFINITE;
             if (hr == 1) break;
             speculated = hr == 0;
@@ -316,8 +326,8 @@
             if (nonfinite) return DFTK_MI_NUM_NONFINITE;
         }
         for (int j : dropped) {
-            CHK(randomize_column(c, X, j));
-            Mat xj = X.cols_from(j, 1);
+            CHK(randomize_column(c, cur, j));
+            Mat xj = cur.cols_from(j, 1);
             int o2 = 0;
             cd* scr = c.BYX + (int64_t)ny * X.cols;
             for (auto& Y : Yl) {
@@ -336,16 +346,18 @@
         if (!one_fetch) CHK(frob2(c, Mat{c.BYX, ny, ny, X.cols}, &byx2));
         if (!speculated) {
             if (std::sqrt(byx2) < tol && niter > 1) break;
-            CHK(ortho_X(c, X, tmp, tol, &ninner, &growth));
-        }
+            CHK(ortho_X(c, cur, oth.p, tol, &ninner, &growth, true, oth.ld, false, nullptr, nullptr, &res));
+        }
+        if (res.p != cur.p) std::swap(cur, oth);
         if (growth * EPS < tol) break;
         if (niter > 10) {
-            CHK(svd_polar(c, X, tmp, X.rows));
+            CHK(svd_polar(c, cur, oth.p, oth.ld));
             c.n_svd += 1;
-            return 0;
+            break;
         }
         niter += 1;
     }
+    if (cur.p != X.p) CHK(ew_copy(c.b, X.rows, X.cols, cur.p, cur.ld, X.p, X.ld));
     return 0;
 }
 
@@ -607,7 +619,7 @@
     };
     Mat Yb[2] = {Mat{take(3 * blk), N, N, 3 * M}, Mat{take(3 * blk), N, N, 3 * M}};
     Mat AYb[2] = {Mat{take(3 * blk), N, N, 3 * M}, Mat{take(3 * blk), N, N, 3 * M}};
-    int cur = 0;
+    int cur = (ax_prev != nullptr && ax_prev == AYb[0].p) ? 1 : 0;
     auto Pblk = [&](const Mat& buf, int nact) { return buf.cols_from(M, nact); };
     auto Rblk = [&](const Mat& buf, int nact, bool has_p) { return buf.cols_from(M + (has_p ? nact : 0), nact); };
     Mat newR{take(blk), N, N, M};
@@ -639,14 +651,15 @@
     double* d_rn = dd + 6 * (M + 8);
     c.rng.seed((seed ? seed : 0x9E3779B97F4A7C15ull) + 0x632BE59BD9B4E019ull * (uint64_t)comm_rank(comm));
     c.rng_rep.seed((seed ? seed : 0x9E3779B97F4A7C15ull) ^ 0xD1B54A32D192ED03ull);
-    Mat X = Yb[0].cols_from(0, M), AX = AYb[0].cols_from(0, M);
+    Mat X = Yb[cur].cols_from(0, M), AX = AYb[cur].cols_from(0, M);
     kb->last_AX = real_mode ? nullptr : AX.p;
 
     Mat Xuser{Xp, ldX, N, M};
+    Mat X0{tmp, N, N, M};
     if (real_mode)
-        CHK(gamma_lobpcg_load(kb, M, Xp, ldX, X.p, X.ld, true));
+        CHK(gamma_lobpcg_load(kb, M, Xp, ldX, X0.p, X0.ld, true));
     else
-        CHK(ew_copy(b, N, M, Xuser.p, Xuser.ld, X.p, X.ld));
+        CHK(ew_copy(b, N, M, Xuser.p, Xuser.ld, X0.p, X0.ld));
     std::vector<double> resid_history((size_t)M * (maxiter + 1), 0.0);
     auto RH = [&](int i, int it) -> double& { return resid_history[(size_t)i + (size_t)M * it]; };
     std::vector<double> full_lam(M, 0.0);
@@ -654,7 +667,9 @@
     {
         int nch;
         double gr;
-        CHK(ortho_X(c, X, tmp, ortho_tol, &nch, &gr));
+        Mat res = X0;
+        CHK(ortho_X(c, X0, X.p, ortho_tol, &nch, &gr, true, X.ld, false, nullptr, nullptr, &res));
+        if (res.p != X.p) CHK(ew_copy(b, N, M, res.p, res.ld, X.p, X.ld));
         if (reuse_ax && !(nch == 1)) reuse_ax = false;
     }
     int64_t n_matvec = M;
@@ -664,20 +679,17 @@
         const size_t cube = (size_t)bb->nz * bb->ny * bb->nxp;
         if (!kb->d_dVs) HIPCHK(hipMalloc((void**)&kb->d_dVs, cube * sizeof(double)));
         CHK(ew_sub_real(bb, (int64_t)cube, kb->d_Vs, kb->d_Vs_ax, kb->d_dVs));
-        if (ax_prev != AX.p) {
-            CHK(c.mm('N', N, M, M, ONE, ax_prev, ax_prev_ld, c.invR, M, ZERO, AX.p, AX.ld, 2));
-        } else {
-            CHK(c.mm('N', N, M, M, ONE, ax_prev, ax_prev_ld, c.invR, M, ZERO, newR.p, newR.ld, 2));
-            CHK(ew_copy(b, N, M, newR.p, newR.ld, AX.p, AX.ld));
-        }
+        CHK(c.mm('N', N, M, M, ONE, ax_prev, ax_prev_ld, c.invR, M, ZERO, AX.p, AX.ld, 2));
         double* const Vs_bound = kb->d_Vs;
         kb->d_Vs = kb->d_dVs;
-        const int st_dv = real_mode ? gamma_apply_H(kb, 1, M, X.p, X.ld, newR.p, newR.ld)
-                                    : dftk_mi_apply_H_parts(kb, 1, M, reinterpret_cast<const dftk_mi_cplx*>(X.p), X.ld,
-                                                            reinterpret_cast<dftk_mi_cplx*>(newR.p), newR.ld);
+        const bool acc = real_mode && !kb->sh_comm;
+        const int st_dv = acc         ? gamma_apply_H(kb, 1, M, X.p, X.ld, AX.p, AX.ld, true)
+                          : real_mode ? gamma_apply_H(kb, 1, M, X.p, X.ld, newR.p, newR.ld)
+                                      : dftk_mi_apply_H_parts(kb, 1, M, reinterpret_cast<const dftk_mi_cplx*>(X.p), X.ld,
+                                                              reinterpret_cast<dftk_mi_cplx*>(newR.p), newR.ld);
         kb->d_Vs = Vs_bound;
         CHK(st_dv);
-        CHK(ew_add(b, N, M, newR.p, newR.ld, AX.p, AX.ld));
+        if (!acc) CHK(ew_add(b, N, M, newR.p, newR.ld, AX.p, AX.ld));
         static const bool ax_check = getenv("DFTK_MI_AX_REUSE_CHECK") != nullptr;
         if (ax_check) {
             CHK(apply_H(M, X.p, X.ld, newR.p, newR.ld));
@@ -878,7 +890,6 @@
     }
     X = Yb[cur].cols_from(0, M);
     AX = AYb[cur].cols_from(0, M);
-    kb->last_AX = real_mode ? nullptr : AX.p;
     if (!finished) final_iter = maxiter;
     (void)status_final;
 
@@ -889,12 +900,15 @@
         std::stable_sort(perm.begin(), perm.end(), [&](int a, int d) { return full_lam[a] < full_lam[d]; });
         int* d_perm = reinterpret_cast<int*>(dd + 7 * (M + 8));
         CHK(h2d(b, d_perm, perm.data(), M * sizeof(int)));
-        CHK(ew_gather_cols(b, N, M, X.p, X.ld, d_perm, tmp, N));
-        CHK(ew_copy(b, N, M, tmp, N, X.p, X.ld));
-        CHK(ew_gather_cols(b, N, M, AX.p, AX.ld, d_perm, tmp, N));
-        CHK(ew_copy(b, N, M, tmp, N, AX.p, AX.ld));
+        Mat Xs = Yb[cur ^ 1].cols_from(0, M), AXs = AYb[cur ^ 1].cols_from(0, M);
+        CHK(ew_gather_cols(b, N, M, X.p, X.ld, d_perm, Xs.p, Xs.ld));
+        CHK(ew_gather_cols(b, N, M, AX.p, AX.ld, d_perm, AXs.p, AXs.ld));
+        cur ^= 1;
+        X = Xs;
+        AX = AXs;
         CHK(stream_sync(b));
     }
+    kb->last_AX = real_mode ? nullptr : AX.p;
     if (real_mode)
         CHK(gamma_lobpcg_store(kb, M, X.p, X.ld, Xp, ldX));
     else
diff --git a/include/dftk_mi355x.h b/include/dftk_mi355x.h
--- a/include/dftk_mi355x.h
+++ b/include/dftk_mi355x.h
@@ -196,6 +196,8 @@
                          int64_t ldx);
 int dftk_mi_gamma_apply_H(dftk_mi_kblock* kb, int which, int n_bands, const dftk_mi_cplx* psih_d, int64_t ld_psi,
                           dftk_mi_cplx* Hpsih_d, int64_t ld_Hpsi);
+int dftk_mi_gamma_apply_H_add(dftk_mi_kblock* kb, int which, int n_bands, const dftk_mi_cplx* psih_d, int64_t ld_psi,
+                              dftk_mi_cplx* Hpsih_d, int64_t ld_Hpsi);
 int dftk_mi_density_accumulate_real(dftk_mi_kblock* kb, int n_bands, const dftk_mi_cplx* psi_d, int64_t ld_psi,
                                     const double* weight_h, double* rho_d);
 
```
